# ctSkennerton/crass

Measured on AMD Instinct MI355X. Metric: reads/sec through DR search+recruit, 150bp synthetic, 1/2/4/8 MI355X, higher is better.
Workload: dtype u8; 1 GPU; 100000000 synthetic 150 bp reads, 50 seeded DRs, 1 % CRISPR reads (BASELINE.json configs[2]); pass1 + merge + pass2; total_reads=100000000, reads_per_gpu=100000000, read_len=150, n_dr=50, parallelism=read-shards x1, launcher=single context, pass1_found=563794, pass2_found=436000, patterns=13320, ac_states=0, filter_survivors=1705594, fast_filter=1, lds_automaton=2, merge_fallbacks=0

## Files before the change

### crass_amd/csrc/dev_common.h

```cpp
#pragma once
#include "engine_internal.h"

namespace crass {

#define WAVE 64

static __device__ __forceinline__ void wave_sync()
{
    __builtin_amdgcn_fence(__ATOMIC_RELEASE, "wavefront");
    __builtin_amdgcn_wave_barrier();
    __builtin_amdgcn_fence(__ATOMIC_ACQUIRE, "wavefront");
}

static __device__ __forceinline__ uint32_t uni(uint32_t x) { return (uint32_t)__builtin_amdgcn_readfirstlane((int)x); }
static __device__ __forceinline__ int uni(int x) { return __builtin_amdgcn_readfirstlane(x); }
static __device__ __forceinline__ uint64_t uni64(uint64_t x) { return ((uint64_t)uni((uint32_t)(x >> 32)) << 32) | (uint64_t)uni((uint32_t)x); }

static __device__ __forceinline__ uint64_t rd_word_off(const DevReads &R, uint64_t r)
{
    return R.stride_words ? r * (uint64_t)R.stride_words : R.word_off[r];
}
static __device__ __forceinline__ uint32_t rd_len(const DevReads &R, uint64_t r)
{
    return R.uniform_len ? R.uniform_len : R.lengths[r];
}
static __device__ __forceinline__ bool rd_is_exc(const DevReads &R, uint64_t r)
{
    return (R.exc_mask[r >> 5] >> (r & 31)) & 1u;
}
static __device__ __forceinline__ uint64_t rd_hint_off(const DevReads &R, uint64_t r)
{
    return R.uniform_len ? r * (uint64_t)((R.uniform_len + 63u) >> 6) : R.pos_hint_off[r];
}
static __device__ __forceinline__ uint64_t rd_header_id(const DevReads &R, uint64_t r)
{
    return R.header_id ? R.header_id[r] : r;
}

typedef unsigned short u16x2 __attribute__((ext_vector_type(2)));
static __device__ __forceinline__ uint32_t pk_min_u16(uint32_t a, uint32_t b)
{
    u16x2 r = __builtin_elementwise_min(__builtin_bit_cast(u16x2, a), __builtin_bit_cast(u16x2, b));
    return __builtin_bit_cast(uint32_t, r);
}

}
```

### crass_amd/csrc/engine.cpp

```cpp
#include "engine_ctx.h"

#include <cstdio>
#include <new>
#include <string>

void crass_hip_ctx::widen_p1() const
{
    P1Dense &D = dense;
    if (D.wide_ready) return;
    (void)wait_bulk();
    const uint64_t n = D.n;
    const uint32_t ss_cap = D.pack_ss_cap, stride = dr_stride;
    const uint8_t *hb = D.h_blob.p;
    const uint16_t *b_replen = (const uint16_t *)(hb + D.lay.replen), *b_ss = (const uint16_t *)(hb + D.lay.ss);
    const uint8_t *b_nss = hb + D.lay.nss, *b_ss8 = hb + D.lay.ss;
    D.w_replen.resize(n); D.w_nss.resize(n); D.w_ss_off.resize(n); D.w_ss.resize(n * (size_t)ss_cap);
    D.w_dr_len.resize(n); D.w_dr.resize(n * (size_t)stride);
    if (D.dr_fallback) (void)hipStreamSynchronize(copy_stream);
    else (void)wait_dx();
    const size_t per_task = 16384;
    host_parallel_for((size_t)((n + per_task - 1) / per_task), 16, [&](size_t t) {
        const uint64_t k0 = t * per_task, k1 = std::min<uint64_t>(n, k0 + per_task);
        for (uint64_t k = k0; k < k1; k++) { D.w_replen[k] = b_replen[k]; D.w_nss[k] = b_nss[k]; D.w_ss_off[k] = k * (uint64_t)ss_cap; }
        if (D.lay.ss_elem == 1) for (uint64_t i = k0 * ss_cap; i < k1 * (uint64_t)ss_cap; i++) D.w_ss[i] = b_ss8[i];
// ... 152 lines not shown
{
    if (!c || level < 0 || level > 2) return CRASS_ERR_INVALID_ARG;
    c->timing_level = level;
    return CRASS_OK;
}

int crass_hip_set_host_view(crass_hip_ctx *c, int light)
{
    if (!c || light < 0 || light > 1) return CRASS_ERR_INVALID_ARG;
    quiesce_worker(c);
    c->host_view_light = light != 0;
    if (c->host_view_light) c->dm.M.x_on = 0;
    return CRASS_OK;
}

int crass_hip_set_timing_focus(crass_hip_ctx *c, unsigned kernels)
{
    if (!c || kernels > 7u) return CRASS_ERR_INVALID_ARG;
    c->timing_focus = kernels;
    return CRASS_OK;
}

void crass_hip_destroy(crass_hip_ctx *c)
{
    if (!c) return;
    (void)hipSetDevice(c->device);
    quiesce_worker(c);
    c->worker.stop();
    if (c->stream) (void)hipStreamSynchronize(c->stream);
    if (c->copy_stream) (void)hipStreamSynchronize(c->copy_stream);
    if (c->hint_stream) (void)hipStreamSynchronize(c->hint_stream);
    (void)sdma_wait(c->dma);
    (void)c->wait_dx();
    ingest_free_all(c);
    if (getenv("CRASS_POLL_REPORT")) fprintf(stderr, "[crass_hip] stage-flag polls that ran out of their budget: %u (of %u flags)\n", c->n_poll_timeouts.load(), c->flag_seq);
    c->lb_status.release(); c->lb_ticket.release(); c->h_lb_fail.release(); c->h_flags.release();
    if (c->xchg.ev_counts) (void)hipEventDestroy(c->xchg.ev_counts);
    c->dm.release(); c->h_qblob.release(); c->xchg.send.release(); c->xchg.xinfo.release(); c->xchg.h_xinfo.release();
    c->dd_map.release(); c->dd_dx_chars.release(); c->dd_dx_len.release(); c->dd_dx_hash.release();
    c->h_dmap.release(); c->h_dx_chars.release(); c->h_dx_len.release(); c->h_dx_hash.release();
    if (c->ev_gathered) (void)hipEventDestroy(c->ev_gathered);
    if (c->ev_sink_copies) (void)hipEventDestroy(c->ev_sink_copies);
    for (int q = 0; q < crass_hip_ctx::kHintParts; q++) if (c->ev_hint[q]) (void)hipEventDestroy(c->ev_hint[q]);
    if (c->ev_hint_go) (void)hipEventDestroy(c->ev_hint_go);
    if (c->hint_stream) (void)hipStreamDestroy(c->hint_stream);
    sdma_destroy(c->dma); c->dma = nullptr;
    for (auto &d : c->dma_sink) { sdma_destroy(d); d = nullptr; }
    for (auto &d : c->dma_dx) { sdma_destroy(d); d = nullptr; }
    if (c->ev_premerge) (void)hipEventDestroy(c->ev_premerge);
    if (c->copy_stream) (void)hipStreamDestroy(c->copy_stream);
    c->r_packed.release(); c->r_word_off.release(); c->r_lengths.release(); c->r_header_id.release();
    c->r_exc_mask.release(); c->r_exc_read.release(); c->r_exc_off.release(); c->r_exc_bytes.release();
    c->d_mask.release(); c->d_word_prefix.release(); c->d_block_sums.release(); c->d_idx.release(); c->d_count.release();
    c->d_found.release(); c->d_hit_info.release(); c->d_surv.release(); c->d_dr.release(); c->d_ss_pool.release();
    c->d_ss_used.release(); c->d_rec.release(); c->d_exc_hit.release(); c->d_extra.release(); c->d_extra_bad.release(); c->h_extra_bad.release();
    c->g_surv.release(); c->g_dr.release(); c->g_ss.release(); c->g_fidx.release(); c->h_count.release(); c->h_surv.release(); c->h_dr.release(); c->h_ss.release(); c->h_idx.release(); c->h_rec.release();
    c->a_go4w.release(); c->a_go16.release(); c->a_go32.release(); c->a_out.release(); c->a_go4.release(); c->dense.release(); c->d_fidx.release(); c->d_pos_hint.release(); c->d_pos_hint_off.release(); c->d_pos_hint_blk.release(); c->d_punt.release(); c->d_redo.release(); c->dd_keys.release(); c->dd_first.release(); c->dd_slot.release(); c->dd_rep.release(); c->dd_hash.release(); c->h_rep.release(); c->h_hash.release(); c->a_anchor.release(); c->d_slot_info.release(); c->d_slot_pid.release(); c->a_out_pid.release(); c->a_pat_token.release();
    for (auto &e : c->ev) if (e) (void)hipEventDestroy(e);
    if (c->stream) (void)hipStreamDestroy(c->stream);
    delete c;
}

int validate_reads(const crass_reads *r)
{
    if (!r) return CRASS_ERR_INVALID_ARG;
    if (r->n_reads && !r->packed) return CRASS_ERR_INVALID_ARG;
    if (!r->stride_words && r->n_reads && !r->word_off) return CRASS_ERR_INVALID_ARG;
    if (!r->uniform_len && r->n_reads && !r->lengths) return CRASS_ERR_INVALID_ARG;
    if (r->n_exceptions && (!r->exc_read || !r->exc_off || !r->exc_bytes)) return CRASS_ERR_INVALID_ARG;
    if (r->uniform_len > CRASS_HIP_MAX_READ_LEN) return CRASS_ERR_UNSUPPORTED;
    return CRASS_OK;
}

int alloc_scratch(crass_hip_ctx *c)
{
    const uint64_t n = c->R.n_reads;
    const uint64_t n_words = std::max<uint64_t>((n + 63) / 64, 1024);
    HIPCHK(c, c->d_mask.ensure(n_words + 1));
    HIPCHK(c, c->d_word_prefix.ensure(n_words + 1));
    HIPCHK(c, c->d_block_sums.ensure((n_words + 255) / 256 + 2));
    HIPCHK(c, c->d_idx.ensure(n + 1));
    HIPCHK(c, c->d_count.ensure(8));
    HIPCHK(c, c->d_found.ensure(n + 1));
    HIPCHK(c, c->d_hit_info.ensure(n + 1));
    HIPCHK(c, c->d_ss_used.ensure(4));
    HIPCHK(c, c->h_count.ensure(32));
    HIPCHK(c, hipMemsetAsync(c->d_found.p, 0, n + 1, c->stream));
    return CRASS_OK;
}

static int setup_pos_hints(crass_hip_ctx *c, const uint32_t *lengths, uint32_t uniform_len, uint64_t n)
{
    c->n_pos_hint_words = 0;
    c->R.pos_hint = nullptr; c->R.pos_hint_off = nullptr; c->R.wave_walk = 0; c->R.hint_all = 0;
    const DevParams &P = c->dp;
    const bool lane_filter = c->R.stride_words >= 4 && c->R.stride_words <= 16;
    c->hint_filter = c->max_len <= c->env.long_min && !lane_filter && !c->env.no_hint_filter;
    c->hint_filter_any = false;
    const bool shifts_ok = P.lowDR + P.lowSp >= 17 && P.highDR + P.highSp <= 127 && P.highDR + P.highSp >= P.lowDR + P.lowSp;
    const bool lattice_hints = P.window == 8 && P.skips == 8 && shifts_ok;
    const bool any_filter = c->hint_filter && !lattice_hints && shifts_ok && P.window >= 6 && P.window <= 9 && P.skips >= 1;
    if ((c->max_len <= c->env.long_min && !c->hint_filter) || n == 0 || !(lattice_hints || any_filter)) return CRASS_OK;
    if (c->env.no_pos_hints) return CRASS_OK;
    std::vector<uint64_t> off(n + 1);
    uint64_t at = 0;
    for (uint64_t i = 0; i < n; i++) { off[i] = at; at += ((uint64_t)(lengths ? lengths[i] : uniform_len) + 63) / 64; }
    off[n] = at;
    HIPCHK(c, c->d_pos_hint_off.ensure(n + 1)); HIPCHK(c, c->d_pos_hint.ensure(at + 1));
    HIPCHK(c, hipMemcpy(c->d_pos_hint_off.p, off.data(), (n + 1) * 8, hipMemcpyHostToDevice));
    c->n_pos_hint_words = at;
    c->hint_filter_any = any_filter;
    c->R.pos_hint = c->d_pos_hint.p; c->R.pos_hint_off = c->d_pos_hint_off.p;
    c->R.hint_all = any_filter ? 1u : 0u;
    c->R.wave_walk = c->max_len > std::min<uint32_t>(c->env.long_min, c->env.wave_walk_min) ? 1u : 0u;
    c->pos_hint_blk = false;
    { const char *hp = getenv("CRASS_HINT_PARTS");
      const int want = hp ? atoi(hp) : 2;
      const bool big = hp ? (n >= 64 && at >= 2048) : (n >= 4096 && at >= (1u << 20));
      c->hint_parts = (big && !c->hint_filter) ? std::min(std::max(want, 1), (int)crass_hip_ctx::kHintParts) : 1; }
    if (c->hint_parts > 1 && !c->hint_stream) {
        int prio_lo = 0, prio_hi = 0;
        (void)hipDeviceGetStreamPriorityRange(&prio_lo, &prio_hi);
        HIPCHK(c, hipStreamCreateWithPriority(&c->hint_stream, hipStreamNonBlocking, getenv("CRASS_HINT_SAME_PRIORITY") ? 0 : prio_lo));
        for (int q = 0; q < crass_hip_ctx::kHintParts; q++) HIPCHK(c, hipEventCreateWithFlags(&c->ev_hint[q], hipEventDisableTiming));
        HIPCHK(c, hipEventCreateWithFlags(&c->ev_hint_go, hipEventDisableTiming));
    }
    for (int q = 0; q <= c->hint_parts; q++) {
        const uint64_t r = q == c->hint_parts ? n : n * (uint64_t)q / (uint64_t)c->hint_parts;
        c->hint_read_split[q] = r;
        c->hint_word_split[q] = q == c->hint_parts ? at : ((off[r] + 255) & ~255ull);
    }
    if (lengths && n <= 0xFFFFFFFFull) {
        std::vector<uint32_t> blk((at + 255) / 256 + 1, 0);
        uint64_t r = 0;
        for (uint64_t b = 0; b * 256 < at; b++) {
            while (r + 1 < n && off[r + 1] <= b * 256) r++;
            blk[b] = (uint32_t)r;
// ... 201 lines not shown
```

### crass_amd/csrc/engine_ctx.h

```cpp
#pragma once
#include "../../include/crass_hip.h"
#include "engine_internal.h"
#include "merge.h"
#include "fastx_launch.h"

#include <algorithm>
#include <atomic>
#include <chrono>
#include <condition_variable>
#include <cstdint>
#include <cstdlib>
#include <cstring>
#include <functional>
#include <memory>
#include <mutex>
#include <thread>
#include <utility>
#include <vector>

#pragma GCC visibility push(hidden)
namespace crass {

inline double now_ms()
{
// ... 164 lines not shown
    std::vector<uint8_t> f_flags;
    DevBuf<unsigned long long> n_table; DevBuf<uint64_t> n_rec_pos, n_ids, n_ctl; DevBuf<uint32_t> n_long;
    PinBuf<uint64_t> n_h_ctl;
    StageTimer<3> tm_names;
    float last_hid_ms[3] = {0, 0, 0};
    DevBuf<unsigned long long> nt_table; DevBuf<uint64_t> nt_rec_pos;
    bool have_names = false, nt_on_arena = false;
    const uint8_t *nt_bytes = nullptr; uint64_t nt_n_bytes = 0, nt_n_reads = 0, nt_mask = 0;
    DevBuf<uint8_t> nq_names; DevBuf<uint64_t> nq_off, nq_out; DevBuf<uint32_t> nq_long;
    DevBuf<uint32_t> nq_ctl, no_len, no_flag; DevBuf<uint64_t> no_tiles, no_idx, no_off;
    PinBuf<uint64_t> nq_h_ctl, no_h;
    uint64_t last_find_found = 0;
    StageTimer<2> tm_find;
    float last_names_ms[2] = {0, 0};
    LineFetch hl, ql;
    DevBuf<uint8_t> fa_arena; uint64_t fa_bytes = 0; bool have_arena = false;
    PinBuf<uint64_t> fa_h_base; PinBuf<int32_t> fa_h_format;
    struct ShardStaged { uint32_t file; uint64_t a, b, off; };
    DevBuf<uint8_t> sh_stage, sh_tail; DevBuf<FxProbe> sh_part; PinBuf<FxProbe> sh_h_part;
    std::vector<ShardStaged> sh_staged;
    std::vector<uint64_t> sh_base;
    uint64_t sh_n_reads = 0; bool sh_scanned = false, sh_loaded = false;
    StageTimer<2> tm_probe;
    float last_probe_ms = 0;
};

}
#pragma GCC visibility pop

using namespace crass;

struct EnvSwitches {
    bool no_lookback = false, no_pos_hints = false, merge_profile = false, no_lane_kernel = false;
    bool host_merge = false, no_speculation = false, exc_separate = false, dm_inject_fail = false, dm_init_late = false;
    bool no_presize = false;
    bool dd_full_table = false;
    bool no_device_view = false;
    bool force_device_view = false;
    bool no_dense_light = false;
    bool no_warm_launch = false;
    uint32_t view_group_cap = 32768;
    uint32_t view_sort_max = 2048;
    uint64_t test_bounds[4] = {0, 0, 0, 0};
    uint32_t row_cap = 256, dm_group_cap = 16384, surv_debug = 0;
    int stage_timing = -1;
    uint64_t pool_cap_bytes = 0;
    bool no_hint_filter = false;
    uint32_t wave_walk_min = 800;
    uint32_t long_min = 2048;
    uint64_t text_chunk_bytes = 64ull << 20;
    bool inflate_hbm_window = true;
    uint32_t hid_hash_bits = 64;
    bool lane_find_serial = false;
    uint32_t probe_blocks = 0;
    void read()
    {
        auto on = [](const char *n) { return getenv(n) != nullptr; };
        no_lookback = on("CRASS_NO_LOOKBACK"); no_pos_hints = on("CRASS_NO_POS_HINTS");
        merge_profile = on("CRASS_MERGE_PROFILE"); no_lane_kernel = on("CRASS_NO_LANE_KERNEL"); host_merge = on("CRASS_HOST_MERGE");
        no_speculation = on("CRASS_NO_SPECULATION"); exc_separate = on("CRASS_EXC_SEPARATE"); dm_init_late = on("CRASS_DM_INIT_LATE");
        dm_inject_fail = on("CRASS_DM_INJECT_FAIL"); no_presize = on("CRASS_NO_PRESIZE"); no_device_view = on("CRASS_NO_DEVICE_VIEW"); dd_full_table = on("CRASS_DD_FULL_TABLE"); force_device_view = on("CRASS_DEVICE_VIEW");
        view_group_cap = 32768; if (const char *e = getenv("CRASS_VIEW_GROUP_CAP")) view_group_cap = (uint32_t)std::max(1, atoi(e));
        view_sort_max = 2048; if (const char *e = getenv("CRASS_VIEW_SORT_MAX")) view_sort_max = (uint32_t)std::min(2048, std::max(64, atoi(e)));
        row_cap = 256; if (const char *e = getenv("CRASS_ROW_CAP")) row_cap = (uint32_t)std::max(1, atoi(e));
        dm_group_cap = 16384; if (const char *e = getenv("CRASS_DM_GROUP_CAP")) dm_group_cap = (uint32_t)std::max(1, atoi(e));
        surv_debug = 0; if (const char *e = getenv("CRASS_SURV_DEBUG")) surv_debug = (uint32_t)atoi(e);
        stage_timing = -1; if (const char *e = getenv("CRASS_STAGE_TIMING")) stage_timing = std::min(2, std::max(0, atoi(e)));
        for (auto &b : test_bounds) b = 0;
        if (const char *e = getenv("CRASS_TEST_BOUNDS")) { int k = 0; for (const char *q = e; *q && k < 4; k++) { test_bounds[k] = (uint64_t)atoll(q); while (*q && *q != ',') q++; if (*q == ',') q++; } }
        no_hint_filter = on("CRASS_NO_HINT_FILTER");
        wave_walk_min = 800; if (const char *e = getenv("CRASS_WAVE_WALK_MIN")) wave_walk_min = (uint32_t)std::max(0, atoi(e));
        long_min = 2048; if (const char *e = getenv("CRASS_LONG_MIN")) long_min = (uint32_t)std::max(0, atoi(e));
        no_warm_launch = getenv("CRASS_NO_WARM_LAUNCH") != nullptr;
        no_dense_light = getenv("CRASS_NO_DENSE_LIGHT") != nullptr;
        text_chunk_bytes = 64ull << 20; if (const char *e = getenv("CRASS_TEXT_CHUNK_BYTES")) text_chunk_bytes = (uint64_t)std::max(1ll, atoll(e));
        inflate_hbm_window = true; if (const char *e = getenv("CRASS_INFLATE_WINDOW")) inflate_hbm_window = strcmp(e, "lds") != 0;
        hid_hash_bits = 64; if (const char *e = getenv("CRASS_HID_TEST_HASH_BITS")) hid_hash_bits = (uint32_t)std::min(64, std::max(0, atoi(e)));
        lane_find_serial = false; if (const char *e = getenv("CRASS_LANE_FIND_SERIAL")) lane_find_serial = atoi(e) != 0;
        probe_blocks = 0; if (const char *e = getenv("CRASS_PROBE_BLOCKS")) probe_blocks = (uint32_t)std::max(0, atoi(e));
        pool_cap_bytes = 0; if (const char *e = getenv("CRASS_POOL_CAP_MB")) pool_cap_bytes = (uint64_t)std::max(1ll, atoll(e)) << 20;
    }
};

struct crass_hip_ctx {
    crass_params prm{};
    EnvSwitches env;
    DevParams dp{};
    int device = 0;
    hipStream_t stream = nullptr;
    mutable int last_hip = 0;

    DevReads R{};
    bool have_reads = false;
    uint64_t read_base = 0;
    uint32_t max_len = 0;
    bool uniform = false;
    DevBuf<uint32_t> r_packed; DevBuf<uint64_t> r_word_off; DevBuf<uint32_t> r_lengths; DevBuf<uint64_t> r_header_id;
    DevBuf<uint32_t> r_exc_mask; DevBuf<uint64_t> r_exc_read; DevBuf<uint64_t> r_exc_off; DevBuf<uint8_t> r_exc_bytes;
    std::vector<uint64_t> h_exc_read;
    std::vector<uint32_t> h_lengths;
    Ingest in;

    DevBuf<uint64_t> d_mask; DevBuf<uint32_t> d_word_prefix; DevBuf<uint32_t> d_block_sums;
    DevBuf<uint64_t> d_idx; DevBuf<uint32_t> d_count; DevBuf<uint8_t> d_found; DevBuf<uint32_t> d_hit_info;
    bool hints_valid = false;
    DevBuf<SurvOut> d_surv; DevBuf<char> d_dr; DevBuf<uint32_t> d_ss_pool; DevBuf<uint32_t> d_ss_used;
    DevBuf<RecruitOut> d_rec; DevBuf<uint32_t> d_exc_hit; DevBuf<uint64_t> d_extra;
    DevBuf<uint32_t> d_extra_bad; PinBuf<uint32_t> h_extra_bad;
    PinBuf<uint32_t> h_count; PinBuf<SurvOut> h_surv; PinBuf<char> h_dr; PinBuf<uint32_t> h_ss; PinBuf<uint64_t> h_idx;
    DevBuf<SurvOut> g_surv; DevBuf<char> g_dr; DevBuf<uint32_t> g_ss;
    PinBuf<RecruitOut> h_rec;
    DevBuf<uint16_t> a_go16; DevBuf<uint32_t> a_go32; DevBuf<uint16_t> a_out; DevBuf<uint16_t> a_go4;
    DevAutomaton A{};
    HostAutomaton H;
    bool full_automaton_uploaded = false;
    DevBuf<uint32_t> a_go4w;
    DevBuf<uint32_t> a_anchor; DevBuf<uint32_t> d_slot_info; DevBuf<uint32_t> d_slot_pid; DevBuf<uint32_t> a_out_pid; DevBuf<uint32_t> a_pat_token;
    bool have_pat_token = false;
    DevAnchors K{};
    bool have_anchors = false;
    bool have_patterns = false;
    uint32_t n_installed_patterns = 0;

    bool have_pass1 = false;
    struct P1List {
        std::vector<uint64_t> read; std::vector<uint8_t> low; std::vector<uint32_t> replen, nss;
        std::vector<uint64_t> ss_off; std::vector<uint32_t, NoInitAlloc<uint32_t>> ss; std::vector<uint16_t> dr_len; std::vector<char, NoInitAlloc<char>> dr;
        void clear() { read.clear(); low.clear(); replen.clear(); nss.clear(); ss_off.clear(); ss.clear(); dr_len.clear(); dr.clear(); }
        void reserve(size_t n, uint32_t stride) { read.reserve(n); low.reserve(n); replen.reserve(n); nss.reserve(n); ss_off.reserve(n); ss.reserve(n * 6); dr_len.reserve(n); dr.reserve(n * stride); }
        size_t size() const { return read.size(); }
    } cand;
    mutable struct P1Dense {
        DevBuf<uint16_t> d_dr_len; DevBuf<char> d_dr;
        uint64_t n = 0;
        bool active = false;
        PinBuf<uint8_t> h_blob; DevBuf<uint8_t> d_blob;
        P1Blob lay{};
        uint32_t pack_ss_cap = 0;
        bool wide_ready = false;
        std::vector<uint32_t> w_replen, w_nss; std::vector<uint32_t, NoInitAlloc<uint32_t>> w_ss; std::vector<uint64_t> w_ss_off; std::vector<uint16_t> w_dr_len;
        std::vector<char, NoInitAlloc<char>> w_dr;
        PinBuf<char> h_dr_fb; PinBuf<uint16_t> h_dr_len_fb; bool dr_fallback = false;
        void release()
        {
            h_blob.release(); d_blob.release(); h_dr_fb.release(); h_dr_len_fb.release(); d_dr_len.release(); d_dr.release();
        }
    } dense;
    DevBuf<uint64_t> d_fidx;
    DevBuf<uint64_t> g_fidx;
    DevBuf<uint64_t> d_pos_hint, d_pos_hint_off; uint64_t n_pos_hint_words = 0;
    DevBuf<uint32_t> d_punt;
    DevBuf<uint32_t> d_redo;
    SdmaCopy *dma_sink[4] = {nullptr, nullptr, nullptr, nullptr};
    DevBuf<uint32_t> d_pos_hint_blk; bool pos_hint_blk = false;
    DevBuf<unsigned long long> dd_keys; DevBuf<uint32_t> dd_first, dd_slot, dd_rep; DevBuf<uint64_t> dd_hash;
    PinBuf<uint32_t> h_rep; PinBuf<uint64_t> h_hash;
    bool have_rep = false;
    DevBuf<uint32_t> dd_map; DevBuf<char> dd_dx_chars; DevBuf<uint16_t> dd_dx_len; DevBuf<uint64_t> dd_dx_hash;
// ... 282 lines not shown
```

### crass_amd/csrc/engine_internal.h

```cpp
#pragma once
#include <stdint.h>
#include <stddef.h>
#include <hip/hip_runtime.h>
#include "devmem.h"
#include "merge.h"

namespace crass {

struct DevReads {
    const uint32_t *packed;
    const uint64_t *word_off;
    const uint32_t *lengths;
    const uint64_t *header_id;
    const uint32_t *exc_mask;
    uint64_t n_reads;
    uint32_t stride_words;
    uint32_t uniform_len;
    const uint64_t *exc_read;
    const uint64_t *exc_off;
    const uint8_t  *exc_bytes;
    uint64_t n_exc;
    const uint64_t *pos_hint;
    const uint64_t *pos_hint_off;
    uint32_t wave_walk;
    uint32_t hint_all;
};

struct DevParams {
    uint32_t lowDR, highDR, lowSp, highSp, window, minRepeats;
    uint32_t skips;
    uint32_t debug_stop;
    uint32_t exc_survive;
    uint32_t find_serial;
    unsigned long long *prof;
};

struct SurvOut {
    uint32_t found;
    uint32_t n_ss;
    uint32_t repeat_len;
    uint32_t ss_off;
    uint16_t dr_len;
    uint8_t  low_lexi;
    uint8_t  err;
};

struct RecruitOut {
    uint32_t start, end;
    uint32_t token;
    uint16_t dr_len;
    uint8_t  low_lexi;
    uint8_t  pad;
};

struct DevAutomaton {
    const uint16_t *go16;
    const uint32_t *go32;
    const uint16_t *out_len;
    const uint32_t *out_pid;
    const uint16_t *go4;
    const uint32_t *go4w;
    uint32_t n_states;
    uint32_t n_sym1;
    uint8_t  sym[256];
    uint32_t acgt_ok;
    uint32_t max_pat_len;
};

static __host__ __device__ __forceinline__ uint32_t ak_bloom_word(uint32_t h) { return h >> 17; }
static __host__ __device__ __forceinline__ uint32_t ak_bloom_bits(uint32_t h) { return (1u << ((h >> 12) & 31u)) | (1u << ((h >> 7) & 31u)); }

struct DevAnchors {
    const uint32_t *table;
    uint32_t log_size;
    uint32_t mode;
    uint32_t m1, m2;
    uint32_t n_keys;
    uint32_t with_exc;
};

struct DevMergeState {
    uint32_t n_survivors;
    uint32_t n_patterns;
    uint32_t n_keys;
    uint32_t log_size;
    uint32_t fail;
    uint32_t k0;
    uint32_t all_t;
    uint32_t unused_a, unused_b;
    uint32_t tab_mode;
    uint32_t n_badk;
    uint32_t pad[5];
};

static constexpr uint32_t kDmHotStripes = 16, kDmHotCounters = 5, kDmHotWords = kDmHotCounters * kDmHotStripes * 32;
enum { kHotSurvivors = 0, kHotKeys = 1, kHotK0 = 2, kHotEntCursor = 3, kHotRdCursor = 4 };
__host__ __device__ inline uint32_t dm_hot(uint32_t counter, uint32_t block) { return (counter * kDmHotStripes + (block & (kDmHotStripes - 1u))) * 32u; }

// ... 102 lines not shown
    if (tid < kDmHotStripes) {
        M.hot[dm_hot(kHotSurvivors, (uint32_t)tid)] = 0u; M.hot[dm_hot(kHotKeys, (uint32_t)tid)] = 0u; M.hot[dm_hot(kHotK0, (uint32_t)tid)] = 0xFFFFFFFFu;
        M.hot[dm_hot(kHotEntCursor, (uint32_t)tid)] = 0u; M.hot[dm_hot(kHotRdCursor, (uint32_t)tid)] = 0u;
    }
    if (tid == 0) {
        DevMergeState s{};
        s.k0 = 0xFFFFFFFFu;
        s.fail = M.inject_fail ? 16u : 0u;
        *M.st = s;
    }
}

static __device__ __forceinline__ void stage_flag_store(uint32_t *flag, uint32_t val)
{
    __hip_atomic_store(flag, val, __ATOMIC_RELEASE, __HIP_MEMORY_SCOPE_SYSTEM);
}
hipError_t launch_xg_fill(const char *dx_chars, const uint16_t *dx_len, const uint32_t *d_nd, uint32_t stride, uint64_t cap_rows,
                          uint32_t slot_bytes, uint8_t *send, hipStream_t st, const uint32_t *p1_counts = nullptr, uint64_t surv_bound = 0,
                          uint32_t *h_flag = nullptr, uint32_t flag_val = 0);
hipError_t launch_xg_unpack(const uint8_t *recv, uint32_t world, uint32_t rank, uint32_t stride, uint64_t cap_rows, uint32_t slot_bytes,
                            char *g_chars, uint16_t *g_len, uint32_t *xinfo, hipStream_t st, uint32_t *h_xinfo = nullptr,
                            uint32_t *zero2 = nullptr,
                            unsigned long long *dd_keys = nullptr, uint32_t *dd_first = nullptr, uint32_t dd_size = 0);
hipError_t launch_device_merge(const DevMerge &M, hipStream_t st, bool init_done = false, hipStream_t view_st = nullptr,
                               hipEvent_t ev_fork = nullptr, hipEvent_t ev_view = nullptr,
                               hipEvent_t ev_apply = nullptr);
hipError_t launch_anchor_filter_dev(const DevReads &R, const DevMerge &M, const uint8_t *found_flag, uint64_t *hitmask, hipStream_t st, uint32_t max_blocks = 0);
hipError_t launch_dm_verify(const DevReads &R, const DevMerge &M, const uint64_t *idx, const uint32_t *d_n, uint64_t n_max,
                            uint32_t *info_by_slot, uint32_t *pid_by_slot, hipStream_t st);
hipError_t warm_dmerge_module();

struct SurvLds {
    uint32_t seq_bytes;
    uint32_t ss_cap;
    uint32_t row_elems;
    uint32_t words_cap;
    uint32_t hint_words;
    uint32_t total_bytes;
    uint32_t seq_window;
    uint32_t ss_slot;
};

hipError_t launch_filter_general(const DevReads &R, const DevParams &P, uint64_t *hitmask,
                                 uint32_t max_len, hipStream_t st);
hipError_t launch_hint_positions(const DevReads &R, const DevParams &P, const uint64_t *hint_off, const uint32_t *blk_read, uint64_t n_words,
                                 uint64_t *hint_bits, hipStream_t st,
                                 uint64_t w_begin = 0, uint64_t w_end = ~0ull,
                                 uint64_t *hitmask = nullptr);
hipError_t launch_hint_filter_any(const DevReads &R, const DevParams &P, const uint64_t *hint_off, const uint32_t *blk_read, uint64_t n_words,
                                  uint64_t *hitmask, uint64_t *hint_bits, hipStream_t st);
hipError_t launch_long_light(const DevReads &R, const DevParams &P, const uint32_t *d_n, uint64_t n_max, SurvOut *out, uint64_t slot_base,
                             uint32_t max_len, hipStream_t st, uint32_t *punt_list, uint32_t *d_punt_n, const uint64_t *surv_idx = nullptr);
hipError_t launch_filter_fast(const DevReads &R, const DevParams &P, uint64_t *hitmask, uint32_t *seed_hint, hipStream_t st,
                              uint8_t *clear_found = nullptr, bool *cleared = nullptr);
#define CRASS_VGPR_FLOOR(N) asm volatile("" ::: "v" #N)

#ifdef __HIPCC__
template <int THREADS>
static __device__ __forceinline__ uint32_t block_reserve(uint32_t v, uint32_t *counter)
{
    __shared__ uint32_t br_tot[THREADS / 64];
    __shared__ uint32_t br_base;
    const int lane = threadIdx.x & 63, w = threadIdx.x >> 6;
    uint32_t incl = v;
#pragma unroll
    for (int off = 1; off < 64; off <<= 1) {
        const uint32_t u = (uint32_t)__shfl_up((int)incl, off);
        if (lane >= off) incl += u;
    }
    if (lane == 63) br_tot[w] = incl;
    __syncthreads();
    if (threadIdx.x == 0) {
        uint32_t tot = 0;
        for (int i = 0; i < THREADS / 64; i++) { const uint32_t x = br_tot[i]; br_tot[i] = tot; tot += x; }
        br_base = tot ? atomicAdd(counter, tot) : 0u;
    }
    __syncthreads();
    return br_base + br_tot[w] + incl - v;
}
#endif

struct Lookback {
    unsigned long long *status;
    uint32_t *ticket;
    uint32_t epoch;
    uint32_t *fail;
};
static inline uint32_t lookback_tile_words(uint64_t n_words) { return n_words >= 16384 ? 4096u : 256u; }

hipError_t launch_compact(const uint64_t *mask, uint64_t n_words, uint64_t n_bits, uint32_t *word_prefix,
                          uint32_t *block_sums, uint64_t *out_idx, uint64_t out_cap, uint32_t *d_count,
                          hipStream_t st, uint32_t *zero_a = nullptr, uint32_t n_a = 0, uint32_t *zero_b = nullptr, uint32_t n_b = 0,
                          const Lookback *lb = nullptr);
hipError_t launch_survivor(const DevReads &R, const DevParams &P, bool exceptions,
                           const uint64_t *surv_idx, const uint32_t *d_n_surv, uint64_t n_surv_max,
                           SurvOut *out, char *dr_chars, uint32_t dr_stride,
                           uint32_t *ss_pool, uint32_t ss_pool_cap, uint32_t *d_ss_used,
                           uint8_t *found_flag, const uint32_t *seed_hint, const SurvLds &lds, int grid, hipStream_t st,
                           int punt_only = 0,
                           uint64_t slot_base = 0, uint64_t slot_total = 0,
                           const uint32_t *punt_list = nullptr, const uint32_t *d_punt_n = nullptr,
                           uint32_t *redo_list = nullptr);
hipError_t launch_survivor_lanes(const DevReads &R, const DevParams &P, const uint64_t *surv_idx, const uint32_t *d_n_surv,
                                 uint64_t n_surv_max, SurvOut *out, char *dr_chars, uint32_t dr_stride, uint32_t *ss_pool,
                                 uint32_t ss_cap, uint8_t *found_flag, const uint32_t *seed_hint, hipStream_t st,
                                 const DevMerge *init_merge = nullptr, uint32_t max_len = 0, uint32_t *punt_cnt = nullptr);
hipError_t launch_recruit_general(const DevReads &R, const DevAutomaton &A, const uint8_t *found_flag,
                                  uint64_t *hitmask, uint32_t *hit_info, hipStream_t st);
hipError_t launch_recruit_lds(const DevReads &R, const DevAutomaton &A, const uint8_t *found_flag,
                              uint64_t *hitmask, uint32_t *hit_info, hipStream_t st);
hipError_t launch_anchor_filter(const DevReads &R, const DevAnchors &K, const uint8_t *found_flag,
                                uint64_t *hitmask, hipStream_t st, uint32_t max_blocks = 0);
hipError_t launch_recruit_list(const DevReads &R, const DevAutomaton &A, const uint64_t *idx, const uint32_t *d_n,
                               uint64_t n_max, uint32_t *info_by_slot, uint32_t *pid_by_slot, hipStream_t st);
hipError_t launch_recruit_exceptions(const DevReads &R, const DevAutomaton &A, const uint8_t *found_flag,
                                     uint32_t *exc_hit_info , hipStream_t st);
hipError_t launch_recruit_finish(const DevReads &R, const uint64_t *hit_idx, const uint32_t *d_n_hits,
                                 uint64_t n_hits_max, const uint32_t *hit_info, bool info_by_slot, bool exceptions,
                                 const uint32_t *pid_by_slot, const uint32_t *pat_token,
                                 RecruitOut *out, char *dr_chars, uint32_t dr_stride, hipStream_t st,
                                 const uint64_t *pat_mask = nullptr);
hipError_t launch_levenshtein_batch(const uint8_t *chars, const uint64_t *a_off, const uint32_t *a_len,
                                    const uint64_t *b_off, const uint32_t *b_len, uint64_t n_pairs,
                                    int32_t *dist, float *sim, uint32_t max_len, hipStream_t st);
hipError_t launch_mark_found(const uint64_t *idx, uint64_t n, const uint64_t *header_id, uint8_t *found_flag, hipStream_t st);
hipError_t launch_mark_found_skip(const uint64_t *idx, uint64_t n, uint64_t n_reads, const uint64_t *header_id, uint8_t *found_flag, uint32_t *bad,
                                  hipStream_t st);
hipError_t launch_copy_to_host(const void *d_src, void *h_dst, uint64_t bytes, hipStream_t st);
struct SdmaCopy;
SdmaCopy *sdma_create();
void sdma_destroy(SdmaCopy *s);
bool sdma_start(SdmaCopy *s, const void *d_src, void *h_dst, size_t bytes);
int sdma_wait(SdmaCopy *s);
bool sdma_pending(const SdmaCopy *s);
hipError_t launch_build_exc_mask(const uint64_t *exc_read, uint64_t n_exc, uint32_t *exc_mask, hipStream_t st);

hipError_t launch_found_compact(const SurvOut *out, const uint32_t *d_n, uint64_t n_max, uint32_t *d_err, unsigned long long *dd_keys,
                                uint32_t *dd_first, uint32_t dd_size, uint64_t *fidx, uint32_t *d_nf, const Lookback &lb, hipStream_t st);
hipError_t launch_select_found(const SurvOut *out, uint64_t n, uint64_t *mask, uint32_t *d_err, hipStream_t st);
hipError_t launch_gather_sparse(const uint64_t *fidx, const uint32_t *d_nf, uint64_t n_max, const SurvOut *out, const char *dr_chars, uint32_t dr_stride,
                                const uint32_t *ss_pool, SurvOut *g_out, uint64_t *g_slot, char *g_dr, uint32_t *g_ss, uint32_t g_ss_cap,
                                uint32_t *d_ss_total, hipStream_t st, uint16_t *g_dr_len = nullptr,
                                int ss16 = 0);
hipError_t launch_found_mask(const SurvOut *out, const uint32_t *d_n, uint64_t n, uint64_t *mask, uint32_t *d_err, hipStream_t st,
                             unsigned long long *dd_keys = nullptr, uint32_t *dd_first = nullptr, uint32_t dd_size = 0);
hipError_t launch_gather_found(const uint64_t *fidx, const uint32_t *d_nf, uint64_t n_max, const SurvOut *out,
                               const uint64_t *surv_idx, uint64_t read_base, const char *dr_chars, uint32_t dr_stride,
                               const uint32_t *ss_pool, uint32_t ss_cap, uint32_t ss_elem, uint8_t *blob,
                               uint16_t *g_dr_len, char *g_dr, hipStream_t st,
                               unsigned long long *dd_keys = nullptr, uint32_t *dd_first = nullptr, uint32_t dd_size = 0,
                               uint64_t *dd_hash = nullptr, uint32_t *dd_slot = nullptr, uint32_t *d_mismatch = nullptr);
static constexpr uint32_t kDdMaxProbes = 256;
struct P1Blob { uint64_t read, replen, nss, low, ss, total; uint32_t ss_elem; };
__host__ __device__ inline P1Blob p1_blob_layout(uint64_t nf, uint32_t ss_cap, uint32_t ss_elem = 2)
{
    P1Blob b;
    uint64_t at = 0;
    auto sec = [&](uint64_t bytes) { const uint64_t o = at; at += (bytes + 15u) & ~15ull; return o; };
// ... 37 lines not shown
```

### crass_amd/csrc/engine_pass1.cpp

```cpp
#include "engine_ctx.h"

#include <cstdio>

extern "C" {

static int hint_wait_all(crass_hip_ctx *c)
{
    if (!c->hint_pending) return CRASS_OK;
    HIPCHK(c, hipStreamWaitEvent(c->stream, c->ev_hint[c->hint_parts - 1], 0));
    c->hint_pending = false;
    return CRASS_OK;
}

static bool getenv_once_hl_host() { static const bool v = getenv("CRASS_HL_HOST_DEDUPE") != nullptr; return v; }
static bool getenv_once_copy_early() { static const bool on = getenv("CRASS_COPY_EARLY") != nullptr; return on; }

static void dump_surv_prof(crass_hip_ctx *c)
{
    if (!c->dp.prof) return;
    unsigned long long v[192];
    if (hipMemcpy(v, c->dp.prof, sizeof v, hipMemcpyDeviceToHost) != hipSuccess) return;
    (void)hipMemset(c->dp.prof, 0, sizeof v);
    { const unsigned long long big = ~0ull; (void)hipMemcpy(c->dp.prof + 188, &big, 8, hipMemcpyHostToDevice); }
    if (v[191]) fprintf(stderr, "[surv_prof] %llu waves; first start .. last start %.1f us, first start .. last end %.1f us\n", v[186], (double)(v[187] - v[188]) / 100.0, (double)(v[189] - v[188]) / 100.0);
// ... 36 lines not shown
                         const uint64_t *surv_idx_host)
{
    if (n_total == 0) return hint_wait_all(c);
    const SurvLds lds_full = survivor_lds_last_resort(c->max_len, c->dp);
    if (lds_full.total_bytes > 160 * 1024) return CRASS_ERR_UNSUPPORTED;
    const bool rows_bounded = lds_full.row_elems < survivor_lds_layout(c->max_len, c->dp).row_elems;
    const uint32_t row_cap = rows_bounded ? std::min(c->env.row_cap, std::max(c->dp.highDR, c->dp.highSp)) : c->env.row_cap;
    const bool long_full = getenv("CRASS_LONG_FULL_LAYOUT") != nullptr;
    const uint32_t win_env = getenv("CRASS_SEQ_WINDOW") ? (uint32_t)atoi(getenv("CRASS_SEQ_WINDOW")) : 0u;
    const bool windowed = !exc && (win_env || (c->max_len > c->env.long_min && !long_full));
    const SurvLds lds = windowed ? survivor_lds_layout(c->max_len, c->dp, row_cap, win_env ? win_env : 4608u, 256u)
                                 : survivor_lds_layout(c->max_len, c->dp, row_cap);
    const bool capped = lds.row_elems != lds_full.row_elems || lds.seq_window != 0 || lds.ss_cap != lds_full.ss_cap;
    const uint64_t chunk_cap = std::min<uint64_t>(n_total, 1u << 20);
    const uint64_t ss_per = std::min<uint64_t>(lds_full.ss_cap, 64);
    const uint64_t pool_cap = std::min<uint64_t>(std::max<uint64_t>(chunk_cap * ss_per, 1u << 16), 1ull << 28);
    HIPCHK(c, c->d_surv.ensure(chunk_cap));
    HIPCHK(c, c->d_dr.ensure(chunk_cap * c->dr_stride));
    HIPCHK(c, c->d_ss_pool.ensure(pool_cap));
    HIPCHK(c, c->h_surv.ensure(chunk_cap));
    HIPCHK(c, c->h_dr.ensure(chunk_cap * c->dr_stride));
    const bool ident_list = !exc && !surv_idx_host && c->R.n_exc == 0 && n_total <= chunk_cap;
    const uint32_t sh0 = c->dp.lowDR + c->dp.lowSp, sh1 = c->dp.highDR + c->dp.highSp;
    const bool light_any = !c->R.pos_hint && c->max_len > c->env.long_min && !(c->dp.window == 8 && c->dp.skips == 8) && c->dp.window >= 6 && c->dp.window <= 9 &&
                           sh0 >= 17 && sh1 <= 127 && sh1 >= sh0 && !c->env.no_pos_hints;
    const bool use_light = ident_list && ((c->R.pos_hint && c->dp.skips == 8 && c->dp.window == 8) || light_any) && c->dp.debug_stop == 0 && !getenv("CRASS_NO_LIGHT");
    const int grid = 256 * 64;
    const uint32_t stride = c->dr_stride;
    L.reserve(L.size() + n_total / 2 + 16, stride);
    for (uint64_t off = 0; off < n_total; off += chunk_cap) {
        const uint64_t nchunk = std::min(chunk_cap, n_total - off);
        HIPCHK(c, hipMemsetAsync(c->d_ss_used.p, 0, 4, c->stream));
        DevReads R = c->R;
        if (exc) {
            R.exc_read = c->R.exc_read + off; R.exc_off = c->R.exc_off + off; R.n_exc = nchunk;
        }
        if (use_light) {
            HIPCHK(c, c->d_punt.ensure(nchunk + 1)); HIPCHK(c, hipMemsetAsync(c->d_punt.p, 0, 4, c->stream));
            HIPCHK(c, c->d_redo.ensure(nchunk + 1)); HIPCHK(c, hipMemsetAsync(c->d_redo.p, 0, 4, c->stream));
        }
        if (!exc && off == 0) HIPCHK(c, c->stamp(8, 1));
        if (!exc && c->hint_pending && off == 0 && nchunk == n_total) {
            uint64_t s0 = 0;
            for (int q = 0; q < c->hint_parts; q++) {
                const uint64_t r1 = c->hint_read_split[q + 1];
                uint64_t s1 = q + 1 == c->hint_parts ? nchunk
                            : (surv_idx_host ? (uint64_t)(std::lower_bound(surv_idx_host, surv_idx_host + nchunk, r1) - surv_idx_host) : std::min<uint64_t>(r1, nchunk));
                if (q > 0) HIPCHK(c, hipStreamWaitEvent(c->stream, c->ev_hint[q], 0));
                if (s1 > s0 && use_light)
                    HIPCHK(c, launch_long_light(R, c->dp, c->d_count.p + 1, s1 - s0, c->d_surv.p + s0, s0, c->max_len, c->stream, c->d_punt.p + 1, c->d_punt.p));
                else if (s1 > s0)
                    HIPCHK(c, launch_survivor(R, c->dp, false, ident_list ? nullptr : c->d_idx.p + s0, c->d_count.p + 1, s1 - s0,
                                              c->d_surv.p + s0, c->d_dr.p + s0 * (size_t)stride, stride, c->d_ss_pool.p, (uint32_t)pool_cap, c->d_ss_used.p,
                                              c->d_found.p, c->hints_valid ? c->d_hit_info.p : nullptr, lds,
                                              (int)std::min<uint64_t>(grid, s1 - s0), c->stream, 0, s0, nchunk));
                s0 = s1;
            }
            c->hint_pending = false;
        } else if (use_light) {
            { const int hw = hint_wait_all(c); if (hw) return hw; }
            HIPCHK(c, launch_long_light(R, c->dp, c->d_count.p + 1, nchunk, c->d_surv.p, 0, c->max_len, c->stream, c->d_punt.p + 1, c->d_punt.p));
        } else {
            { const int hw = hint_wait_all(c); if (hw) return hw; }
            HIPCHK(c, launch_survivor(R, c->dp, exc, (exc || ident_list) ? nullptr : c->d_idx.p + off, c->d_count.p + (exc ? 0 : 1), nchunk,
                                      c->d_surv.p, c->d_dr.p, stride, c->d_ss_pool.p, (uint32_t)pool_cap, c->d_ss_used.p,
                                      c->d_found.p, (!exc && c->hints_valid) ? c->d_hit_info.p : nullptr, lds,
                                      (int)std::min<uint64_t>(grid, nchunk), c->stream));
        }
        if (use_light)
            HIPCHK(c, launch_survivor(R, c->dp, false, nullptr, c->d_count.p + 1, nchunk,
                                      c->d_surv.p, c->d_dr.p, stride, c->d_ss_pool.p, (uint32_t)pool_cap, c->d_ss_used.p,
                                      c->d_found.p, nullptr, lds, (int)std::min<uint64_t>(256 * 12, nchunk), c->stream, 7, 0, nchunk, c->d_punt.p + 1, c->d_punt.p,
                                      capped ? c->d_redo.p : nullptr));
        if (use_light && c->dp.prof) { HIPCHK(c, hipStreamSynchronize(c->stream)); dump_surv_prof(c); }
        if (capped && use_light)
            HIPCHK(c, launch_survivor(R, c->dp, false, nullptr, c->d_count.p + 1, nchunk,
                                      c->d_surv.p, c->d_dr.p, stride, c->d_ss_pool.p, (uint32_t)pool_cap, c->d_ss_used.p,
                                      c->d_found.p, nullptr, lds_full, (int)std::min<uint64_t>(256 * 2, nchunk), c->stream, 6, 0, nchunk, c->d_redo.p + 1, c->d_redo.p));
        else if (capped)
            HIPCHK(c, launch_survivor(R, c->dp, exc, (exc || ident_list) ? nullptr : c->d_idx.p + off, c->d_count.p + (exc ? 0 : 1), nchunk,
                                      c->d_surv.p, c->d_dr.p, stride, c->d_ss_pool.p, (uint32_t)pool_cap, c->d_ss_used.p,
                                      c->d_found.p, (!exc && c->hints_valid) ? c->d_hit_info.p : nullptr, lds_full,
                                      (int)std::min<uint64_t>(grid, nchunk), c->stream, 6));
        if (!exc && off == 0) HIPCHK(c, c->stamp(9, 1));
        const uint64_t n_words = (nchunk + 63) / 64;
        HIPCHK(c, c->d_fidx.ensure(nchunk)); HIPCHK(c, c->g_surv.ensure(nchunk)); HIPCHK(c, c->g_dr.ensure(nchunk * (size_t)stride + 16));
        HIPCHK(c, c->g_ss.ensure(pool_cap)); HIPCHK(c, c->g_fidx.ensure(nchunk));
        HIPCHK(c, c->d_mask.ensure(n_words + 1)); HIPCHK(c, c->d_word_prefix.ensure(n_words + 1)); HIPCHK(c, c->d_block_sums.ensure((n_words + 255) / 256 + 2));
        HIPCHK(c, hipMemsetAsync(c->d_count.p + 2, 0, 8, c->stream));
        HIPCHK(c, hipMemsetAsync(c->d_ss_used.p, 0, 4, c->stream));
        HIPCHK(c, launch_select_found(c->d_surv.p, nchunk, c->d_mask.p, c->d_count.p + 3, c->stream));
        HIPCHK(c, launch_compact(c->d_mask.p, n_words, nchunk, c->d_word_prefix.p, c->d_block_sums.p, c->d_fidx.p, nchunk, c->d_count.p + 2, c->stream));
        const bool ss16 = c->max_len < 65536;
        const bool hl_dedupe = !exc && off == 0 && nchunk == n_total && c->R.n_exc == 0 && !c->xchg.active && !c->env.host_merge &&
                               c->prm.lowDRsize >= (int)kDevMinDR && stride <= 64 && (stride & 15u) == 0 && nchunk < (1u << 24) && !getenv_once_hl_host();
        if (hl_dedupe) HIPCHK(c, c->g_dr_len.ensure(nchunk));
        HIPCHK(c, launch_gather_sparse(c->d_fidx.p, c->d_count.p + 2, nchunk, c->d_surv.p, c->d_dr.p, stride, c->d_ss_pool.p, c->g_surv.p,
                                       c->g_fidx.p, c->g_dr.p, c->g_ss.p, (uint32_t)pool_cap, c->d_ss_used.p, c->stream,
                                       hl_dedupe ? c->g_dr_len.p : nullptr, ss16 ? 1 : 0));
        HIPCHK(c, hipMemcpyAsync(c->h_count.p + 2, c->d_count.p + 2, 8, hipMemcpyDeviceToHost, c->stream));
        HIPCHK(c, hipMemcpyAsync(c->h_count.p + 6, c->d_ss_used.p, 4, hipMemcpyDeviceToHost, c->stream));
        const double tq0 = now_ms();
        HIPCHK(c, hipStreamSynchronize(c->stream));
        const double tq1 = now_ms();
        dump_surv_prof(c);
        if (c->h_count.p[3] == 2) return CRASS_ERR_SEARCH_FATAL;
        if (c->h_count.p[3]) return CRASS_ERR_OVERFLOW;
        const uint64_t nf = c->h_count.p[2];
        const uint32_t used = c->h_count.p[6];
        if (nf > nchunk || used > pool_cap) return CRASS_ERR_OVERFLOW;
        HIPCHK(c, c->h_ss.ensure(used + 1)); HIPCHK(c, c->h_idx.ensure(nf + 1));
        static const bool sink_eager = getenv("CRASS_SINK_EAGER") != nullptr;
        const bool lazy = !sink_eager && !exc && off == 0 && nchunk == n_total && c->R.n_exc == 0 && !surv_idx_host && &L == &c->cand && L.read.empty();
        if (nf) {
            hipStream_t cs = lazy ? c->copy_stream : c->stream;
            const void *srcs[4] = {c->g_surv.p, c->g_dr.p, c->g_fidx.p, c->g_ss.p};
            void *dsts[4] = {c->h_surv.p, c->h_dr.p, c->h_idx.p, c->h_ss.p};
            const size_t nbs[4] = {nf * sizeof(SurvOut), nf * (size_t)stride, nf * 8, used ? (size_t)used * (ss16 ? 2 : 4) : 0};
            static const bool sink_blit = getenv("CRASS_COPY_BLIT") != nullptr;
            for (int q = 0; q < 4; q++) {
                if (!nbs[q]) continue;
                if (lazy && !sink_blit) {
                    if (!c->dma_sink[q]) c->dma_sink[q] = sdma_create();
                    if (sdma_start(c->dma_sink[q], srcs[q], dsts[q], nbs[q])) continue;
                }
                HIPCHK(c, hipMemcpyAsync(dsts[q], srcs[q], nbs[q], hipMemcpyDeviceToHost, cs));
            }
            if (lazy) {
                if (!c->ev_sink_copies) HIPCHK(c, hipEventCreateWithFlags(&c->ev_sink_copies, hipEventDisableTiming));
                HIPCHK(c, hipEventRecord(c->ev_sink_copies, c->copy_stream));
                c->bulk_pending = true;
            }
            else HIPCHK(c, hipStreamSynchronize(c->stream));
        }
        bool hl_queued = false, hl_premerge = false;
// ... 197 lines not shown
                D.dr_fallback = true;
                HIPCHK(c, hipMemcpyAsync(c->h_rep.p, c->dd_rep.p, nf * 4, hipMemcpyDeviceToHost, c->copy_stream));
                HIPCHK(c, hipMemcpyAsync(c->h_hash.p, c->dd_hash.p, nf * 8, hipMemcpyDeviceToHost, c->copy_stream));
                c->bulk_pending = true;
                c->have_rep = true;
            }
        }
    } else D.lay.total = 0;
    D.n = nf;
    D.active = true;
    return CRASS_OK;
}

static int run_survivors_dense(crass_hip_ctx *c, uint64_t n_surv, const uint32_t *d_nsurv, bool *overflow, bool defer = false)
{
    *overflow = false;
    { const int hw = hint_wait_all(c); if (hw) return hw; }
    const SurvLds lds = survivor_lds_layout(c->max_len, c->dp);
    if (lds.total_bytes > 160 * 1024) return CRASS_ERR_UNSUPPORTED;
    const uint32_t stride = c->dr_stride;
    const uint64_t pool_cap = std::max<uint64_t>(n_surv * (uint64_t)lds.ss_cap, 1u << 16);
    if (n_surv == 0 || n_surv > kDenseMaxSurvivors || pool_cap >= (1ull << 31) || lds.ss_cap > 128 || (stride & 15)) return CRASS_ERR_STATE;
    crass_hip_ctx::P1Dense &D = c->dense;
    const bool speculative = (d_nsurv == c->d_count.p);
    const uint64_t n_alloc = speculative ? n_surv : std::max<uint64_t>(n_surv, survivor_bound(n_surv));
    const uint32_t ss_elem = c->max_len <= 256 ? 1u : 2u;
    const bool dedupe = n_surv < (1u << 24);
    const bool defer_ok = defer && dedupe && speculative && c->xchg.active;
    { const int as = ensure_dense_buffers(c, n_alloc, pool_cap, lds, dedupe); if (as) return as; }
    if (!speculative) {
        HIPCHK(c, hipMemsetAsync(c->d_count.p + 2, 0, 20, c->stream));
        HIPCHK(c, hipMemsetAsync(c->d_ss_used.p, 0, 4, c->stream));
    }
    c->dm_prepared_n = 0; c->dm_prepared_src = nullptr;
    const DevMerge *init_merge = nullptr;
    if (speculative && dedupe && c->prm.lowDRsize >= (int)kDevMinDR && stride <= 64 && !c->env.host_merge && !c->env.no_speculation && !c->env.dm_init_late) {
        const char *src = nullptr; const uint16_t *src_len = nullptr; uint64_t bound = 0;
        if (!c->xchg.active && c->dm_prev_local && c->dx_cap_hint) {
            HIPCHK(c, c->dd_dx_chars.ensure(n_alloc * stride + 16)); HIPCHK(c, c->dd_dx_len.ensure(n_alloc));
            src = c->dd_dx_chars.p; src_len = c->dd_dx_len.p; bound = c->dx_cap_hint;
        } else if (c->xchg.active && c->xchg.gx_cap_hint && c->xchg.gx_cap_hint <= c->xchg.world * c->xchg.cap) {
            const uint64_t n_max = c->xchg.world * c->xchg.cap;
            HIPCHK(c, c->dm.gx_chars.ensure((size_t)n_max * stride + 16)); HIPCHK(c, c->dm.gx_len.ensure(n_max));
            src = c->dm.gx_chars.p; src_len = c->dm.gx_len.p; bound = c->xchg.gx_cap_hint;
        }
        if (src) {
            const int ps = device_merge_prepare(c, src, src_len, bound, c->d_count.p + 4);
            if (ps) return ps;
            init_merge = &c->dm.M;
        }
    }
    HIPCHK(c, c->stamp(8, 1));
    static const bool no_hints_dbg = getenv("CRASS_SURV_NO_HINTS") != nullptr;
    const uint32_t *hints = (c->hints_valid && !no_hints_dbg) ? c->d_hit_info.p : nullptr;
    const bool no_lanes = c->env.no_lane_kernel;
    hipError_t le = no_lanes ? hipErrorNotSupported
                             : launch_survivor_lanes(c->R, c->dp, c->d_idx.p, d_nsurv, n_surv, c->d_surv.p, c->d_dr.p, stride,
                                                     c->d_ss_pool.p, lds.ss_cap, c->d_found.p, hints, c->stream, init_merge, c->max_len, c->d_count.p + 6);
    if (le != hipSuccess && le != hipErrorNotSupported) { c->last_hip = (int)le; return CRASS_ERR_HIP; }
    if (le == hipSuccess && init_merge) { c->dm_prepared_n = init_merge->n_tok; c->dm_prepared_src = init_merge->dx_chars; }
    bool light_done = false;
    if (le == hipErrorNotSupported && !no_lanes && c->dp.debug_stop == 0 && !c->env.no_dense_light && c->max_len <= 12288 && c->dp.window >= 6 && c->dp.window <= 9) {
        DevReads RL = c->R;
        const bool lattice = c->R.pos_hint && !c->R.hint_all && c->dp.skips == 8 && c->dp.window == 8;
        if (!lattice && !c->R.hint_all) RL.pos_hint = nullptr;
        HIPCHK(c, c->d_punt.ensure(n_surv + 1)); HIPCHK(c, hipMemsetAsync(c->d_punt.p, 0, 4, c->stream));
        const hipError_t ll = launch_long_light(RL, c->dp, d_nsurv, n_surv, c->d_surv.p, 0, c->max_len, c->stream, c->d_punt.p + 1, c->d_punt.p, c->d_idx.p);
        if (ll == hipSuccess) {
            light_done = true;
            HIPCHK(c, launch_survivor(c->R, c->dp, false, c->d_idx.p, d_nsurv, n_surv, c->d_surv.p, c->d_dr.p, stride,
                                      c->d_ss_pool.p, (uint32_t)pool_cap, c->d_ss_used.p, c->d_found.p, hints, lds,
                                      (int)std::min<uint64_t>(256 * 12, n_surv), c->stream, 7, 0, 0, c->d_punt.p + 1, c->d_punt.p));
        } else if (ll != hipErrorNotSupported) { c->last_hip = (int)ll; return CRASS_ERR_HIP; }
    }
    if (!light_done)
    HIPCHK(c, launch_survivor(c->R, c->dp, false, c->d_idx.p, d_nsurv, n_surv, c->d_surv.p, c->d_dr.p, stride,
                              c->d_ss_pool.p, (uint32_t)pool_cap, c->d_ss_used.p, c->d_found.p, hints, lds,
                              (int)std::min<uint64_t>(256 * 32, n_surv), c->stream, le == hipSuccess ? 4 : 0, 0, 0, nullptr,
                              le == hipSuccess ? c->d_count.p + 6 : nullptr));
    if (c->R.n_exc)
        HIPCHK(c, launch_survivor(c->R, c->dp, true, c->d_idx.p, d_nsurv, n_surv, c->d_surv.p, c->d_dr.p, stride,
                                  c->d_ss_pool.p, (uint32_t)pool_cap, c->d_ss_used.p, c->d_found.p, nullptr, lds,
                                  (int)std::min<uint64_t>(256 * 32, n_surv), c->stream, 5));
    HIPCHK(c, c->stamp(9, 1));
    const uint64_t n_words = (n_surv + 63) / 64;
    uint32_t tsize = 1024;
    if (dedupe) while (tsize < n_surv * 2) tsize <<= 1;
    if (dedupe && speculative && c->dx_cap_hint && !c->dd_full_table && !c->env.dd_full_table) {
        uint32_t small = c->env.test_bounds[1] ? 64u : 4096u;
        while (small < c->dx_cap_hint * 4ull && small < tsize) small <<= 1;
        tsize = std::min(tsize, small);
    }
    Lookback lbf;
    if (const Lookback *lb = c->next_lookback_elems(n_surv, &lbf)) {
        HIPCHK(c, launch_found_compact(c->d_surv.p, d_nsurv, n_surv, c->d_count.p + 3, dedupe ? c->dd_keys.p : nullptr,
                                       dedupe ? c->dd_first.p : nullptr, tsize, c->d_fidx.p, c->d_count.p + 2, *lb, c->stream));
    } else {
        HIPCHK(c, launch_found_mask(c->d_surv.p, d_nsurv, n_surv, c->d_mask.p, c->d_count.p + 3, c->stream,
                                    dedupe ? c->dd_keys.p : nullptr, dedupe ? c->dd_first.p : nullptr, tsize));
        HIPCHK(c, launch_compact(c->d_mask.p, n_words, n_surv, c->d_word_prefix.p, c->d_block_sums.p, c->d_fidx.p, n_surv, c->d_count.p + 2, c->stream));
    }
    HIPCHK(c, launch_gather_found(c->d_fidx.p, c->d_count.p + 2, n_surv, c->d_surv.p, c->d_idx.p, c->read_base, c->d_dr.p, stride,
                                  c->d_ss_pool.p, lds.ss_cap, ss_elem, D.d_blob.p, D.d_dr_len.p, D.d_dr.p, c->stream,
                                  dedupe ? c->dd_keys.p : nullptr, dedupe ? c->dd_first.p : nullptr, tsize, c->dd_hash.p, c->dd_slot.p,
                                  c->d_count.p + 5));
    c->have_rep = false;
    c->have_dev_tokens = false;
    if (dedupe) {
        Lookback lbd;
        const bool dxd = c->dx_via_dma;
        HIPCHK(c, launch_dx_tokens(D.d_dr.p, D.d_dr_len.p, c->dd_hash.p, stride, c->d_count.p + 2, (uint32_t)n_surv, c->dd_rep.p, c->dd_slot.p, c->dd_first.p, c->d_mask.p,
                                   c->d_word_prefix.p, c->d_block_sums.p, c->d_fidx.p, c->d_count.p + 4, c->d_count.p + 5, dxd ? c->dd_map.p : c->h_dmap.p,
                                   dxd ? nullptr : c->h_dx_chars.p, dxd ? nullptr : c->h_dx_len.p, dxd ? nullptr : c->h_dx_hash.p, c->dd_dx_chars.p, c->dd_dx_len.p, c->stream,
                                   c->d_count.p, defer_ok ? c->h_count.p + 16 : c->h_count.p, 8,
                                   c->next_lookback_tiles((n_surv + 1023) / 1024, &lbd)));
        if (c->xchg.active)
            HIPCHK(c, launch_xg_fill(c->dd_dx_chars.p, c->dd_dx_len.p, c->d_count.p + 4, stride, c->xchg.cap, c->xchg.slot, c->xchg.send.p, c->stream,
                                     defer_ok ? c->d_count.p : nullptr, n_surv,
                                     (defer_ok && c->poll_on) ? c->h_flags.p : nullptr, (defer_ok && c->poll_on) ? (c->want_p1 = ++c->flag_seq) : 0u));
    }
    if (!dedupe) HIPCHK(c, hipMemcpyAsync(c->h_count.p, c->d_count.p, 32, hipMemcpyDeviceToHost, c->stream));
    bool premerge_queued = false;
    c->premerge = 0;
    D.wide_ready = false; D.dr_fallback = false;
    D.pack_ss_cap = lds.ss_cap;
    const bool will_premerge = speculative && dedupe && !c->xchg.active && c->dm_prev_local && c->dx_cap_hint && c->prm.lowDRsize >= (int)kDevMinDR && stride <= 64 &&
                               !c->env.host_merge && !c->env.no_speculation;
    if (!c->poll_on && (will_premerge || defer_ok)) HIPCHK(c, hipEventRecord(c->ev_gathered, c->stream));
    if (will_premerge) {
        const bool prepared = c->dm_prepared_n == c->dx_cap_hint && c->dm_prepared_src == c->dd_dx_chars.p;
        const int ps = device_merge_enqueue(c, c->dd_dx_chars.p, c->dd_dx_len.p, c->dx_cap_hint, c->d_count.p + 4, prepared);
        if (ps) return ps;
        premerge_queued = true;
        if (!c->poll_on || !c->dma) HIPCHK(c, hipEventRecord(c->ev_premerge, c->stream));
    }
// ... 30 lines not shown
static int first_call_bounds_impl(crass_hip_ctx *c)
{
    c->surv_cap_hint = 0; c->hit_cap_hint = 0; c->dx_cap_hint = 0; c->dm_prev_local = false; c->premerge = 0;
    c->recruit_exact = false;
    const uint64_t n = c->R.n_reads;
    if (c->env.no_presize || c->env.no_speculation || n == 0 || c->max_len > c->env.long_min) return CRASS_OK;
    if (c->R.n_exc && c->env.exc_separate) return CRASS_OK;
    const DevParams &P = c->dp;
    const SurvLds lds = survivor_lds_layout(c->max_len, P);
    if (lds.total_bytes > 160 * 1024 || lds.ss_cap > 128 || (c->dr_stride & 15)) return CRASS_OK;
    const uint32_t min_len = P.lowDR + P.lowSp + P.window + 1;
    const double seeds = c->max_len > min_len ? (double)(c->max_len - min_len) / P.skips + 1.0 : 1.0;
    const double cand = (double)(P.highDR + P.highSp - P.lowDR - P.lowSp + 1);
    double rate = seeds * cand / (double)(1ull << (2 * P.window)) + 0.02;
    if (rate > 1.0) rate = 1.0;
    uint64_t surv = survivor_bound((uint64_t)((double)n * rate));
    if (surv > n + 65536) surv = survivor_bound(n * 2 / 3);
    if (c->env.test_bounds[0]) surv = std::max<uint64_t>(64, c->env.test_bounds[0]);
    const uint64_t pool_cap = std::max<uint64_t>(surv * (uint64_t)lds.ss_cap, 1u << 16);
    if (surv > kDenseMaxSurvivors || pool_cap >= (1ull << 31)) return CRASS_OK;
    size_t free_b = 0, total_b = 0;
    if (hipMemGetInfo(&free_b, &total_b) != hipSuccess) return CRASS_OK;
    const uint64_t per = 140ull + 3ull * c->dr_stride + 6ull * lds.ss_cap;
    if (surv * per > free_b / 4) return CRASS_OK;
    const bool dedupe = surv < (1u << 24);
    int s = ensure_dense_buffers(c, surv, pool_cap, lds, dedupe);
    if (s) return s;
    c->surv_cap_hint = surv;
    { const uint64_t nw = (n + 63) / 64; c->prealloc_lookback(std::max<uint64_t>((nw + lookback_tile_words(nw) - 1) / lookback_tile_words(nw), (surv + 1023) / 1024)); }
    if (dedupe && c->prm.lowDRsize >= (int)kDevMinDR && c->dr_stride <= 64 && !c->env.host_merge) {
        uint64_t dx = crass_hip_exchange_rows_for(n);
        if (c->env.test_bounds[1]) dx = std::max<uint64_t>(16, c->env.test_bounds[1]);
        s = device_merge_prepare(c, c->dd_dx_chars.p, c->dd_dx_len.p, dx, c->d_count.p + 4);
        if (s) return s;
        c->dx_cap_hint = (uint32_t)dx;
        c->dm_prev_local = true;
        try {
            auto touch = [](auto &v, size_t k) { v.resize(k); v.clear(); };
            MergeResult &m = c->merge;
            touch(m.cand_token, (size_t)(n / 128 + 4096));
            touch(m.tokens.strings.chars, (size_t)dx * 48); touch(m.tokens.strings.off, (size_t)dx + 2); m.tokens.strings.clear();
            touch(m.patterns.chars, (size_t)dx * 24); touch(m.patterns.off, (size_t)dx + 2); m.patterns.clear();
            touch(m.pat_group, (size_t)dx); touch(m.pat_token, (size_t)dx); touch(m.grp_tokens, (size_t)dx); touch(m.grp_off, (size_t)dx / 4 + 16);
        } catch (const std::bad_alloc &) { }
    }
    uint64_t hits = hit_bound(n / 64);
    if (c->env.test_bounds[2]) hits = std::max<uint64_t>(16, c->env.test_bounds[2]);
    s = ensure_recruit_buffers(c, hits, 0, true, true);
    if (s) return s;
    c->hit_cap_hint = hits;
    if (!c->env.no_warm_launch) {
        HIPCHK(c, hipMemsetAsync(c->d_count.p, 0, 32, c->stream));
        HIPCHK(c, launch_survivor(c->R, c->dp, false, c->d_idx.p, c->d_count.p + 1, surv, c->d_surv.p, c->d_dr.p, c->dr_stride,
                                  c->d_ss_pool.p, (uint32_t)pool_cap, c->d_ss_used.p, c->d_found.p, nullptr, lds,
                                  (int)std::min<uint64_t>(256 * 32, surv), c->stream, 4));
    }
    host_pool_warm();
    return CRASS_OK;
}

int first_call_bounds(crass_hip_ctx *c)
{
    const int s = first_call_bounds_impl(c);
    if (s == CRASS_ERR_OOM) {
        c->surv_cap_hint = 0; c->hit_cap_hint = 0; c->dx_cap_hint = 0; c->dm_prev_local = false; c->premerge = 0;
        c->last_hip = 0;
        c->dm.release();
        c->dm_prepared_n = 0; c->dm_prepared_src = nullptr;
        return CRASS_OK;
    }
    return s;
}

struct FilterRoute { bool fast = false, hint_filtered = false, found_cleared = false; };

static int launch_filter(crass_hip_ctx *c, uint64_t n_words, FilterRoute &fr)
{
    hipError_t fe = hipErrorNotSupported;
    static const bool found_memset = getenv("CRASS_FOUND_MEMSET") != nullptr;
    if (c->R.stride_words >= 4 && c->R.stride_words <= 16)
        fe = launch_filter_fast(c->R, c->dp, c->d_mask.p, c->d_hit_info.p, c->stream, found_memset ? nullptr : c->d_found.p, &fr.found_cleared);
    if (fe != hipSuccess) fr.found_cleared = false;
    const bool lattice_hints = c->hint_filter && c->R.pos_hint && !c->hint_filter_any;
    if (fe == hipSuccess) fr.fast = true;
    else if (fe == hipErrorNotSupported && (lattice_hints || (c->hint_filter_any && c->n_pos_hint_words))) {
        HIPCHK(c, hipMemsetAsync(c->d_mask.p, 0, n_words * 8, c->stream));
        const uint32_t *blk = c->pos_hint_blk ? c->d_pos_hint_blk.p : nullptr;
        const hipError_t he = lattice_hints ? launch_hint_positions(c->R, c->dp, c->d_pos_hint_off.p, blk, c->n_pos_hint_words, c->d_pos_hint.p, c->stream, 0, c->n_pos_hint_words, c->d_mask.p)
                                            : launch_hint_filter_any(c->R, c->dp, c->d_pos_hint_off.p, blk, c->n_pos_hint_words, c->d_mask.p, c->d_pos_hint.p, c->stream);
        c->hint_pending = false;
        if (he != hipSuccess) { c->last_hip = (int)he; return CRASS_ERR_HIP; }
        fr.hint_filtered = true;
    }
    else if (fe == hipErrorNotSupported) { HIPCHK(c, launch_filter_general(c->R, c->dp, c->d_mask.p, c->max_len, c->stream)); }
    else { c->last_hip = (int)fe; return CRASS_ERR_HIP; }
    return CRASS_OK;
}

static int launch_unfiltered(crass_hip_ctx *c, uint64_t n_words)
{
    HIPCHK(c, hipMemsetAsync(c->d_mask.p, 0xFF, n_words * 8, c->stream));
    if (!c->R.pos_hint) return CRASS_OK;
    const uint32_t *blk = c->pos_hint_blk ? c->d_pos_hint_blk.p : nullptr;
    if (c->hint_parts > 1) { HIPCHK(c, hipEventRecord(c->ev_hint_go, c->stream)); HIPCHK(c, hipStreamWaitEvent(c->hint_stream, c->ev_hint_go, 0)); }
    for (int q = 0; q < c->hint_parts; q++) {
        hipStream_t hs = q == 0 ? c->stream : c->hint_stream;
        hipError_t he = launch_hint_positions(c->R, c->dp, c->d_pos_hint_off.p, blk, c->n_pos_hint_words, c->d_pos_hint.p, hs,
                                              c->hint_word_split[q], c->hint_word_split[q + 1]);
        if (he != hipSuccess) { c->last_hip = (int)he; return CRASS_ERR_HIP; }
        if (q > 0) HIPCHK(c, hipEventRecord(c->ev_hint[q], c->hint_stream));
    }
    c->hint_pending = c->hint_parts > 1;
    return CRASS_OK;
}

int read_count(crass_hip_ctx *c)
{
    HIPCHK(c, hipMemcpyAsync(c->h_count.p, c->d_count.p, 4, hipMemcpyDeviceToHost, c->stream));
    HIPCHK(c, hipStreamSynchronize(c->stream));
    return CRASS_OK;
}

static int host_survivor_list(crass_hip_ctx *c, bool use_filter, uint64_t &n_surv, std::vector<uint64_t> &surv_idx)
{
    surv_idx.resize(n_surv);
    if (n_surv && use_filter) {
        HIPCHK(c, c->h_idx.ensure(n_surv));
        HIPCHK(c, hipMemcpyAsync(c->h_idx.p, c->d_idx.p, n_surv * 8, hipMemcpyDeviceToHost, c->stream));
        HIPCHK(c, hipStreamSynchronize(c->stream));
        memcpy(surv_idx.data(), c->h_idx.p, n_surv * 8);
    } else if (n_surv) {
        const uint64_t n = c->R.n_reads;
        size_t e = 0, w = 0;
        for (uint64_t r = 0; r < n; r++) {
            while (e < c->h_exc_read.size() && c->h_exc_read[e] < r) e++;
// ... 25 lines not shown
    return m;
}

static int fill_send_from_host(crass_hip_ctx *c)
{
    ensure_distinct(c);
    const uint64_t nd = c->dx_len.size();
    std::vector<uint8_t> buf(c->xchg.send_bytes(), 0);
    reinterpret_cast<uint64_t *>(buf.data())[0] = nd;
    reinterpret_cast<uint32_t *>(buf.data())[2] = c->dr_stride;
    reinterpret_cast<uint32_t *>(buf.data())[3] = (uint32_t)c->xchg.cap;
    for (uint64_t j = 0; j < nd && j < c->xchg.cap; j++) {
        uint8_t *row = buf.data() + (j + 1) * (size_t)c->xchg.slot;
        memcpy(row, c->dx_chars.data() + j * (size_t)c->dr_stride, c->dr_stride);
        const uint32_t l = c->dx_len[j];
        memcpy(row + c->dr_stride, &l, 4);
    }
    HIPCHK(c, hipMemcpy(c->xchg.send.p, buf.data(), buf.size(), hipMemcpyHostToDevice));
    return CRASS_OK;
}

static void publish_p1_counters(crass_hip_ctx *c, uint64_t n_surv, bool fast, bool hint_filtered, float ms_sink_host)
{
    c->cnt.ms_sink_host = ms_sink_host;
    c->cnt.n_filter_survivors = n_surv + (c->dp.exc_survive ? 0 : c->R.n_exc);
    c->cnt.n_pass1_found = c->n_cand();
    c->cnt.used_fast_filter = fast ? 1 : (hint_filtered ? 2 : 0);
    c->spans_p1 = true; c->span_survivors = n_surv != 0;
}

int crass_hip_seed_scan(crass_hip_ctx *c)
{
    if (!c) return CRASS_ERR_INVALID_ARG;
    if (!c->have_reads) return CRASS_ERR_STATE;
    (void)hipSetDevice(c->device);
    (void)c->wait_bulk();
    (void)c->wait_dx();
    c->bulk_status = CRASS_OK; c->dx_status = CRASS_OK;
    quiesce_worker(c);
    c->have_pass1 = c->have_merge = c->have_pass2 = false;
    c->dm.active = false;
    c->premerge_inflight = false;
    c->p1d.active = false;
    const bool defer_p1 = c->p1d.enabled && !c->p1d.force_sync && c->xchg.active;
    c->p1d.force_sync = false;
    if (c->dm.view_launched) { HIPCHK(c, hipStreamWaitEvent(c->stream, c->dm.ev_view, 0)); c->dm.view_launched = false; }
    const uint64_t n = c->R.n_reads;
    const uint64_t n_words = (n + 63) / 64;
    HIPCHK(c, c->stamp(0, 1));
    FilterRoute fr;
    const bool use_filter = c->max_len <= c->env.long_min;
    c->dp.exc_survive = (use_filter && c->R.n_exc > 0 && !c->env.exc_separate) ? 1u : 0u;
    if (const int fs = use_filter ? launch_filter(c, n_words, fr) : launch_unfiltered(c, n_words)) return fs;
    c->hints_valid = fr.fast;
    if (!fr.found_cleared) HIPCHK(c, hipMemsetAsync(c->d_found.p, 0, n + 1, c->stream));
    HIPCHK(c, c->stamp(1, 1));
    Lookback lbs;
    HIPCHK(c, launch_compact(c->d_mask.p, n_words, n, c->d_word_prefix.p, c->d_block_sums.p, c->d_idx.p, n, c->d_count.p, c->stream,
                             c->d_count.p + 2, 5, c->d_ss_used.p, 1, c->next_lookback(n_words, &lbs)));
    HIPCHK(c, c->stamp(2, 2));
    c->dense.active = false; c->have_rep = false; c->have_distinct = false;
    c->have_dev_tokens = false; c->hl_tokens = false;
    c->cand_fill = nullptr; c->cand_pending_n = 0;
    c->cand.clear();
    const double t_sink0 = now_ms();
    uint64_t n_surv = 0;
    int s = CRASS_ERR_STATE;
    const bool exc_ok = c->R.n_exc == 0 || c->dp.exc_survive;
    if (use_filter && exc_ok && c->surv_cap_hint && !c->env.no_speculation) {
        bool overflow = false;
        HIPCHK(c, c->stamp(3, 2));
        s = run_survivors_dense(c, c->surv_cap_hint, c->d_count.p, &overflow, defer_p1);
        if (s != CRASS_OK && s != CRASS_ERR_STATE) return s;
        if (s == CRASS_OK && c->p1d.active) {
            c->p1d.fast = fr.fast; c->p1d.hint_filtered = fr.hint_filtered;
            HIPCHK(c, c->stamp(4, 2));
            return CRASS_OK;
        }
        if (s == CRASS_OK) {
            n_surv = c->h_count.p[0];
            if (overflow) c->n_bound_overflows[0]++;
            if (overflow || n_surv == 0) {
                c->dense.active = false;
                s = CRASS_ERR_STATE;
                HIPCHK(c, hipMemsetAsync(c->d_found.p, 0, n + 1, c->stream));
            }
        } else {
            if (const int rs = read_count(c)) return rs;
            n_surv = c->h_count.p[0];
        }
    } else if (!use_filter && c->R.n_exc == 0) {
        n_surv = n;
    } else {
        if (const int rs = read_count(c)) return rs;
        n_surv = c->h_count.p[0];
    }
    const bool spec_done = (s == CRASS_OK);
    const bool try_dense = !spec_done && use_filter && exc_ok && n_surv > 0 && n_surv <= kDenseMaxSurvivors;
    if (!spec_done) {
        c->h_count.p[1] = 0xFFFFFFFFu;
        HIPCHK(c, hipMemcpyAsync(c->d_count.p + 1, c->h_count.p + 1, 4, hipMemcpyHostToDevice, c->stream));
        HIPCHK(c, c->stamp(3, 2));
        bool overflow = false;
        s = try_dense ? run_survivors_dense(c, n_surv, c->d_count.p + 1, &overflow) : CRASS_ERR_STATE;
        if (s != CRASS_OK && s != CRASS_ERR_STATE) return s;
    }
    if (use_filter && exc_ok) c->surv_cap_hint = survivor_bound(n_surv);
    if (s == CRASS_ERR_STATE) {
        const bool identity = !use_filter && c->R.n_exc == 0;
        std::vector<uint64_t> surv_idx;
        if (!identity) { const int ls = host_survivor_list(c, use_filter, n_surv, surv_idx); if (ls) return ls; }
        s = run_survivors(c, false, n_surv, c->cand, identity ? nullptr : surv_idx.data());
// ... 58 lines not shown
```

### crass_amd/csrc/kernels.hip

```cpp
#include "dev_common.h"
#include "comp_table.h"
#include "lane_find.h"
#include <type_traits>
#include <algorithm>

namespace crass {

static __constant__ CompTable c_comp = make_comp_table();

#define FG_WAVES 4

static __device__ __forceinline__ uint32_t lds_code(const uint32_t *w, uint32_t p, uint32_t mask)
{
    uint32_t wi = p >> 4, sh = (p & 15u) * 2u;
    uint64_t v = ((uint64_t)w[wi + 1] << 32) | w[wi];
    return (uint32_t)(v >> sh) & mask;
}

__global__ __launch_bounds__(FG_WAVES * WAVE) void k_filter_general(DevReads R, DevParams P, uint64_t *hitmask,
                                                                      uint32_t lds_words_per_wave)
{
    extern __shared__ __attribute__((aligned(16))) uint32_t fg_lds[];
    const int lane = threadIdx.x & 63;
    const int wave = threadIdx.x >> 6;
// ... 128 lines not shown
    }
    uint32_t miss = (t0 | (t0 >> 15)) & 0xFFFFu;
    if (SW > 8) miss |= (t1 | (t1 >> 15)) << 16;
    return ~miss & (n_seed >= 32 ? 0xFFFFFFFFu : ((1u << n_seed) - 1u));
}

template <int W, int D0, int D1, int LCT, int RPL>
__global__ __launch_bounds__(256) void k_filter_fast_impl(DevReads R, DevParams P, uint64_t *hitmask, uint32_t *seed_hint, uint8_t *clear_found)
{
    const uint64_t r_first = blockIdx.x * (uint64_t)(256 * RPL) + threadIdx.x;
    if (clear_found && r_first == 0) clear_found[R.n_reads] = 0;
    constexpr int WX = W + (D1 >> 4) + 2;
    const uint64_t r_last = R.n_reads - 1;
    uint32_t nxt[W];
    uint64_t nxt_exc;
    if constexpr (RPL > 1) ff_request_row<W>(R, P, r_first, r_last, nxt, nxt_exc);
    else ff_load_row<W>(R, P, r_first, nxt, nxt_exc);
#pragma unroll
    for (int it = 0; it < RPL; it++) {
    const uint64_t r = r_first + (uint64_t)it * 256u;
    const bool active = r < R.n_reads;
    if constexpr (RPL == 1) { if (clear_found && active) clear_found[r] = 0; }
    uint32_t w[WX];
#pragma unroll
    for (int i = 0; i < WX; i++) w[i] = i < W ? nxt[i] : 0u;
    const bool exc = (nxt_exc >> (r & 63)) & 1u;
    if (it + 1 < RPL) {
        ff_request_row<W>(R, P, r + 256u, r_last, nxt, nxt_exc);
        __builtin_amdgcn_sched_barrier(0);
    }
    const uint32_t L = active ? rd_len(R, r) : 0u;
    constexpr int SW = ((16 * W - 58) / 8 + 2) / 2;
    uint32_t acc[SW];
    ff_exact_scan<D0, D1, LCT>(w, acc, [&]() { if constexpr (RPL > 1) { if (clear_found) clear_found[active ? r : R.n_reads] = 0; } });
    bool hit = false;
    const int searchEnd = LCT > 0 ? (LCT - D0 - 8 - 1) : (int)(L - P.lowDR - P.lowSp - 8 - 1);
    if (active && !exc && searchEnd >= 0) {
        const uint32_t hint = ff_exact_hint<LCT>(acc, searchEnd / 8 + 1);
        hit = hint != 0;
        if (hit) seed_hint[r] = hint;
    }
    uint64_t m = __ballot(hit);
    if ((threadIdx.x & 63) == 0 && active) hitmask[r >> 6] = m;
    }
}

static __device__ __forceinline__ uint32_t pk_minimum3_f16(uint32_t a, uint32_t b, uint32_t c)
{
    uint32_t r;
    asm("v_pk_minimum3_f16 %0, %1, %2, %3" : "=v"(r) : "v"(a), "v"(b), "v"(c));
    return r;
}
template <int W, int D0, int D1, int LCT, int RPL>
__global__ __launch_bounds__(256) void k_filter_fast_pairs(DevReads R, DevParams P, uint64_t *hitmask, uint32_t *seed_hint, uint8_t *clear_found)
{
    static_assert(LCT > 0 && LCT - D0 - 9 >= 0 && RPL * 256 <= 65536, "uniform length with at least one seed");
    __shared__ uint32_t q_n;
    __shared__ uint16_t q[256 * RPL];
    __shared__ uint32_t tile_mask[2 * 4 * RPL];
    const uint64_t r_block = blockIdx.x * (uint64_t)(256 * RPL);
    const uint64_t r_first = r_block + threadIdx.x;
    const uint32_t lane = threadIdx.x & 63u;
    if (clear_found && r_first == 0) clear_found[R.n_reads] = 0;
    constexpr int WX = W + (D1 >> 4) + 2;
    constexpr int SW = ((16 * W - 58) / 8 + 2) / 2;
    constexpr int n_seed = (LCT - D0 - 9) / 8 + 1;
    constexpr uint32_t M14 = 0x3FFF3FFFu;
    const uint64_t r_last = R.n_reads - 1;
    uint32_t nxt[W];
    uint64_t nxt_exc;
    ff_request_row<W>(R, P, r_first, r_last, nxt, nxt_exc);
    if (threadIdx.x < 2 * 4 * RPL) tile_mask[threadIdx.x] = 0;
    if (threadIdx.x == 0) q_n = 0;
    __syncthreads();
#pragma unroll
    for (int it = 0; it < RPL; it++) {
        const uint64_t r = r_first + (uint64_t)it * 256u;
        const bool active = r < R.n_reads;
        uint32_t w[WX];
#pragma unroll
        for (int i = 0; i < WX; i++) w[i] = i < W ? nxt[i] : 0u;
        const bool exc = (nxt_exc >> (r & 63)) & 1u;
        if (it + 1 < RPL) {
            ff_request_row<W>(R, P, r + 256u, r_last, nxt, nxt_exc);
            __builtin_amdgcn_sched_barrier(0);
        }
        uint32_t acc[SW];
#pragma unroll
        for (int i = 0; i < SW; i++) acc[i] = 0x3C003C00u;
#pragma unroll
        for (int d = D0; d <= D1; d += 2) {
            if (d == D0 + 2 && clear_found) clear_found[active ? r : R.n_reads] = 0;
#pragma unroll
            for (int k = 0; k < SW; k++) {
                if (d > LCT - 9 - 16 * k) continue;
                const int q0 = d >> 4, sh0 = (d & 15) * 2;
                const uint32_t s0 = sh0 ? __builtin_amdgcn_alignbit(w[k + q0 + 1], w[k + q0], sh0) : w[k + q0];
                const uint32_t a = (s0 ^ w[k]) & M14;
                uint32_t b = a;
                if (d + 1 <= D1 && d + 1 <= LCT - 9 - 16 * k) {
                    const int q1 = (d + 1) >> 4, sh1 = ((d + 1) & 15) * 2;
                    const uint32_t s1 = sh1 ? __builtin_amdgcn_alignbit(w[k + q1 + 1], w[k + q1], sh1) : w[k + q1];
                    b = (s1 ^ w[k]) & M14;
                }
                acc[k] = pk_minimum3_f16(acc[k], a, b);
            }
        }
        uint32_t m = 0x3C003C00u;
#pragma unroll
        for (int k = 0; 2 * k < n_seed; k += 2) m = pk_minimum3_f16(m, acc[k], 2 * (k + 1) < n_seed ? acc[k + 1] : acc[k]);
        const bool pos = active && !exc && pk_nonzero_u16(m) != 0x00010001u;
        const uint64_t pm = __ballot(pos);
        if (pm) {
            uint32_t base = 0;
            if (lane == 0) base = atomicAdd(&q_n, (uint32_t)__popcll(pm));
            base = __builtin_amdgcn_readfirstlane(base);
            const uint32_t before = __builtin_amdgcn_mbcnt_hi((uint32_t)(pm >> 32), __builtin_amdgcn_mbcnt_lo((uint32_t)pm, 0u));
            if (pos) q[base + before] = (uint16_t)(it * 256 + threadIdx.x);
        }
    }
    __syncthreads();
    const uint32_t qn = q_n;
    for (uint32_t b0 = threadIdx.x & ~63u; b0 < qn; b0 += 256u) {
        const bool have = b0 + lane < qn;
        const uint32_t loc = have ? q[b0 + lane] : 0u;
        uint32_t w[WX];
#pragma unroll
        for (int i = 0; i < WX; i++) w[i] = 0u;
        if (have) ff_load_words<W>(R, r_block + loc, w);
        uint32_t acc[SW];
        ff_exact_scan<D0, D1, LCT>(w, acc);
        const uint32_t hint = ff_exact_hint<LCT>(acc, n_seed);
        if (have && hint != 0) {
            seed_hint[r_block + loc] = hint;
            atomicOr(&tile_mask[loc >> 5], 1u << (loc & 31u));
        }
    }
    __syncthreads();
    if (threadIdx.x < 4 * RPL) {
        const uint64_t r0 = r_block + threadIdx.x * 64u;
        if (r0 < R.n_reads) hitmask[r0 >> 6] = (uint64_t)tile_mask[2 * threadIdx.x] | ((uint64_t)tile_mask[2 * threadIdx.x + 1] << 32);
    }
}

template <int W>
__global__ __launch_bounds__(256) void k_filter_fast_range(DevReads R, DevParams P, uint64_t *hitmask, uint32_t *seed_hint)
{
    const uint64_t r = blockIdx.x * (uint64_t)256 + threadIdx.x;
    constexpr int WX = 2 * W + 2;
    uint32_t row[W];
    uint64_t exc_word;
    ff_load_row<W>(R, P, r, row, exc_word);
    const bool active = r < R.n_reads;
    uint32_t w[WX];
#pragma unroll
    for (int i = 0; i < WX; i++) w[i] = i < W ? row[i] : 0u;
    const bool exc = (exc_word >> (r & 63)) & 1u;
    const uint32_t L = active ? rd_len(R, r) : 0u;
    constexpr int SW = ((16 * W - 26) / 8 + 2) / 2;
    const int D0 = (int)(P.lowDR + P.lowSp), D1 = min((int)(P.highDR + P.highSp), 16 * W + 15);
    uint32_t acc[SW];
#pragma unroll
    for (int i = 0; i < SW; i++) acc[i] = 0xFFFFFFFFu;
    const int n_seed_max = (16 * W - D0 - 9) / 8 + 1;
#pragma unroll
    for (int q = 0; q <= W; q++) {
        if (16 * q + 15 < D0 || 16 * q > D1) continue;
        const int sb_lo = max(0, D0 - 16 * q), sb_hi = min(15, D1 - 16 * q);
        for (int sb = sb_lo; sb <= sb_hi; sb++) {
            const uint32_t sh = (uint32_t)(2 * sb);
#pragma unroll
            for (int k = 0; k < SW; k++) {
                if (2 * k >= n_seed_max) continue;
                const uint32_t lo = w[k + q], hi = w[k + q + 1];
                acc[k] = pk_min_u16(acc[k], __builtin_amdgcn_alignbit(hi, lo, sh) ^ w[k]);
            }
        }
    }
    bool hit = false;
    const int searchEnd = (int)(L - P.lowDR - P.lowSp - 8 - 1);
    if (active && !exc && searchEnd >= 0) {
        const int n_seed = searchEnd / 8 + 1;
        uint32_t t0 = 0, t1 = 0;
#pragma unroll
        for (int k = 0; k < SW; k++) {
            const uint32_t f = pk_nonzero_u16(acc[k]);
            if (k < 8) t0 |= f << (2 * k); else t1 |= f << (2 * (k - 8));
        }
        uint32_t miss = (t0 | (t0 >> 15)) & 0xFFFFu;
        if (SW > 8) miss |= (t1 | (t1 >> 15)) << 16;
        const uint32_t hint = ~miss & (n_seed >= 32 ? 0xFFFFFFFFu : ((1u << n_seed) - 1u));
        hit = hint != 0;
        if (hit) seed_hint[r] = hint;
    }
// ... 24 lines not shown
#pragma unroll
    for (int q = 0; q <= W; q++) {
        if (16 * q + 15 < D0 || 16 * q > D1) continue;
        const int sb_lo = max(0, D0 - 16 * q), sb_hi = min(15, D1 - 16 * q);
        for (int sb = sb_lo; sb <= sb_hi; sb++) {
            const uint32_t sh = (uint32_t)(2 * sb);
            uint32_t z[W + 1];
#pragma unroll
            for (int k = 0; k <= W; k++) {
                const uint32_t x = __builtin_amdgcn_alignbit(w[k + q + 1], w[k + q], sh) ^ w[k];
                z[k] = x | (x >> 1);
            }
#pragma unroll
            for (int k = 0; k < W; k++) z[k] |= __builtin_amdgcn_alignbit(z[k + 1], z[k], (uint32_t)(2 * s1));
            if (s2 > 0) {
                z[W] |= z[W] >> (2 * s1);
#pragma unroll
                for (int k = 0; k < W; k++) z[k] |= __builtin_amdgcn_alignbit(z[k + 1], z[k], (uint32_t)(2 * s2));
            }
            if (s3 > 0) {
                z[W] |= z[W] >> (2 * s2);
#pragma unroll
                for (int k = 0; k < W; k++) z[k] |= __builtin_amdgcn_alignbit(z[k + 1], z[k], (uint32_t)(2 * s3));
            }
            if (s4 > 0) {
                z[W] |= z[W] >> (2 * s3);
#pragma unroll
                for (int k = 0; k < W; k++) z[k] |= __builtin_amdgcn_alignbit(z[k + 1], z[k], (uint32_t)(2 * s4));
            }
#pragma unroll
            for (int k = 0; k < W; k++) nz[k] &= z[k];
        }
    }
    bool hit = false;
    const int searchEnd = (int)(L - P.lowDR - P.lowSp - P.window - 1);
    if (active && !exc && searchEnd >= 0) {
        const uint32_t skips = P.skips;
        uint32_t hint = 0, more = 0;
        uint32_t j = 0;
        for (uint32_t i = 0; j <= (uint32_t)searchEnd; i++, j += skips) {
            uint32_t word = 0;
#pragma unroll
            for (int k = 0; k < W; k++) word = (j >> 4) == (uint32_t)k ? nz[k] : word;
            const uint32_t m = ((word >> (2u * (j & 15u))) & 1u) ^ 1u;
            if (i < 32u) hint |= m << i; else more |= m;
        }
        hit = (hint | more) != 0;
        if (hit) seed_hint[r] = more ? 0xFFFFFFFFu : hint;
    }
    const uint64_t m = __ballot(hit);
    if ((threadIdx.x & 63) == 0 && active) hitmask[r >> 6] = m;
}

hipError_t launch_filter_fast(const DevReads &R, const DevParams &P, uint64_t *hitmask, uint32_t *seed_hint, hipStream_t st, uint8_t *clear_found, bool *cleared)
{
    if (cleared) *cleared = false;
    if (!R.stride_words || R.n_reads == 0) return hipErrorNotSupported;
    if (P.window != 8 || P.skips != 8) {
        if (P.window < 6 || P.window > 9 || P.skips < 1 || P.lowDR + P.lowSp < 17 || P.highDR + P.highSp < P.lowDR + P.lowSp) return hipErrorNotSupported;
        const uint64_t nb = (R.n_reads + 255) / 256;
        if (nb > 0x7FFFFFFFull) return hipErrorNotSupported;
        switch (R.stride_words) {
#define FA_CASE(WW) case WW: CRASS_LAUNCH((k_filter_fast_any<WW>), dim3((unsigned)nb), dim3(256), 0, st, R, P, hitmask, seed_hint); break;
            FA_CASE(4) FA_CASE(5) FA_CASE(6) FA_CASE(7) FA_CASE(8) FA_CASE(9) FA_CASE(10)
            FA_CASE(11) FA_CASE(12) FA_CASE(13) FA_CASE(14) FA_CASE(15) FA_CASE(16)
#undef FA_CASE
            default: return hipErrorNotSupported;
        }
        return hipGetLastError();
    }
    if (P.lowDR + P.lowSp != 49 || P.highDR + P.highSp != 97) {
        if (P.lowDR + P.lowSp < 17 || P.highDR + P.highSp < P.lowDR + P.lowSp) return hipErrorNotSupported;
        const uint64_t nb = (R.n_reads + 255) / 256;
        if (nb > 0x7FFFFFFFull) return hipErrorNotSupported;
        switch (R.stride_words) {
#define FR_CASE(WW) case WW: CRASS_LAUNCH((k_filter_fast_range<WW>), dim3((unsigned)nb), dim3(256), 0, st, R, P, hitmask, seed_hint); break;
            FR_CASE(4) FR_CASE(5) FR_CASE(6) FR_CASE(7) FR_CASE(8) FR_CASE(9) FR_CASE(10)
            FR_CASE(11) FR_CASE(12) FR_CASE(13) FR_CASE(14) FR_CASE(15) FR_CASE(16)
#undef FR_CASE
            default: return hipErrorNotSupported;
        }
        return hipGetLastError();
    }
    uint64_t blocks = (R.n_reads + 255) / 256;
    if (blocks > 0x7FFFFFFFull) return hipErrorNotSupported;
    static const int rpl_env = getenv("CRASS_FF_RPL") ? atoi(getenv("CRASS_FF_RPL")) : 0;
    const int rpl = rpl_env ? rpl_env : (R.n_reads >= (1u << 22) ? 4 : 1);
    dim3 g((unsigned)blocks), b(256), g4((unsigned)((blocks + 3) / 4));
    static const bool ff_exact = getenv("CRASS_FF_EXACT") && atoi(getenv("CRASS_FF_EXACT")) != 0;
    if (cleared && clear_found) *cleared = true;
#define FF_LEN(LL, WW) if (R.uniform_len == LL && R.stride_words == WW) { \
        if (rpl >= 4 && !ff_exact) CRASS_LAUNCH((k_filter_fast_pairs<WW, 49, 97, LL, 4>), g4, b, 0, st, R, P, hitmask, seed_hint, clear_found); \
        else if (rpl >= 4) CRASS_LAUNCH((k_filter_fast_impl<WW, 49, 97, LL, 4>), g4, b, 0, st, R, P, hitmask, seed_hint, clear_found); \
        else CRASS_LAUNCH((k_filter_fast_impl<WW, 49, 97, LL, 1>), g, b, 0, st, R, P, hitmask, seed_hint, clear_found); \
        return hipGetLastError(); }
    FF_LEN(100, 7) FF_LEN(101, 7) FF_LEN(125, 8) FF_LEN(126, 8) FF_LEN(150, 10) FF_LEN(151, 10) FF_LEN(250, 16) FF_LEN(251, 16)
#undef FF_LEN
    switch (R.stride_words) {
#define FF_CASE(WW) case WW: CRASS_LAUNCH((k_filter_fast_impl<WW, 49, 97, 0, 1>), g, b, 0, st, R, P, hitmask, seed_hint, clear_found); break;
        FF_CASE(4) FF_CASE(5) FF_CASE(6) FF_CASE(7) FF_CASE(8) FF_CASE(9) FF_CASE(10)
        FF_CASE(11) FF_CASE(12) FF_CASE(13) FF_CASE(14) FF_CASE(15) FF_CASE(16)
#undef FF_CASE
        default: if (cleared) *cleared = false; return hipErrorNotSupported;
    }
    return hipGetLastError();
}

static __device__ __forceinline__ uint64_t hint_bits_class(const uint32_t (&w)[13], uint32_t rho)
{
    uint32_t v[12];
    const uint32_t rs = 2u * rho;
#pragma unroll
    for (int i = 0; i < 12; i++) v[i] = rs ? ((w[i] >> rs) | (w[i + 1] << (32u - rs))) : w[i];
    uint32_t acc[4] = {0xFFFFFFFFu, 0xFFFFFFFFu, 0xFFFFFFFFu, 0xFFFFFFFFu};
#pragma unroll
    for (int d = 49; d <= 97; d++) {
        const int q = d >> 4, sh = (d & 15) * 2;
#pragma unroll
        for (int k = 0; k < 4; k++) {
            const uint32_t lo = v[k + q], hi = v[k + q + 1];
            const uint32_t x = (sh ? ((lo >> sh) | (hi << (32 - sh))) : lo) ^ v[k];
            acc[k] = pk_min_u16(acc[k], x);
        }
    }
    const uint32_t m0 = pk_nonzero_u16(acc[0]), m1 = pk_nonzero_u16(acc[1]), m2 = pk_nonzero_u16(acc[2]), m3 = pk_nonzero_u16(acc[3]);
    const uint32_t lo = __builtin_amdgcn_perm(m1, m0, 0x06040200u) ^ 0x01010101u;
    const uint32_t hi = __builtin_amdgcn_perm(m3, m2, 0x06040200u) ^ 0x01010101u;
    return ((uint64_t)(hi << rho) << 32) | (uint64_t)(lo << rho);
}

static __device__ __forceinline__ uint64_t hint_bits_class_range(const uint32_t (&w)[13], uint32_t rho, int D0, int D1)
{
    uint32_t v[12];
    const uint32_t rs = 2u * rho;
#pragma unroll
    for (int i = 0; i < 12; i++) v[i] = rs ? ((w[i] >> rs) | (w[i + 1] << (32u - rs))) : w[i];
    uint32_t acc[4] = {0xFFFFFFFFu, 0xFFFFFFFFu, 0xFFFFFFFFu, 0xFFFFFFFFu};
#pragma unroll
    for (int q = 0; q < 8; q++) {
        if (16 * q + 15 < D0 || 16 * q > D1) continue;
        const int sb_lo = max(0, D0 - 16 * q), sb_hi = min(15, D1 - 16 * q);
        for (int sb = sb_lo; sb <= sb_hi; sb++) {
            const uint32_t sh = (uint32_t)(2 * sb);
#pragma unroll
            for (int k = 0; k < 4; k++) acc[k] = pk_min_u16(acc[k], __builtin_amdgcn_alignbit(v[k + q + 1], v[k + q], sh) ^ v[k]);
// ... 1116 lines not shown
        for (int i = 0; i < SV_PREFETCH_HINTS; i++) {
            const int wi = lane + i * WAVE;
            if (wi < nh) l_hint[wi] = pf.hw[i];
        }
        first = lane + SV_PREFETCH_HINTS * WAVE;
        if (nh <= SV_PREFETCH_HINTS * WAVE) return;
    }
    const uint64_t *ph = R.pos_hint + rd_hint_off(R, r);
    for (int wi = first; wi < nh; wi += WAVE) l_hint[wi] = ph[wi];
}

static __device__ void load_read_to_lds(const DevReads &R, uint64_t r, uint8_t *seq, uint32_t *words, int L, int lane,
                                        const ReadPrefetch *pf = nullptr)
{
    const uint32_t *g = R.packed + rd_word_off(R, r);
    const int nw = (L + 15) >> 4;
    const int ng = (nw + 4) >> 2;
    const bool have = pf && pf->r == r;
    uint4 *w4 = reinterpret_cast<uint4 *>(words);
    int first = lane;
    if (have) {
#pragma unroll
        for (int i = 0; i < SV_PREFETCH_VEC; i++) {
            const int gi = lane + i * WAVE;
            if (gi < ng) w4[gi] = pf->v[i];
        }
        first = lane + SV_PREFETCH_VEC * WAVE;
    }
    for (int gi = first; gi < ng; gi += WAVE) w4[gi] = sv_load_group(g, gi, nw);
    (void)seq;
}

#define PROF_READ_DONE(cat_, tot_) do { \
            wave_sync(); \
            if (lane == 0) { h.lprof[PF_TOTAL] = (tot_); h.lprof[PF_READS] = 1ull; } \
            wave_sync(); \
            unsigned long long *ws_ = h.lprof + PF_SLOTS + (cat_) * PF_SLOTS; \
            if (lane < PF_SLOTS && lane != PF_MAX) ws_[lane] += h.lprof[lane]; \
            if (lane == PF_MAX && (tot_) > ws_[PF_MAX]) ws_[PF_MAX] = (tot_); \
            if (lane == 0) { int b_ = 63 - __clzll((long long)((tot_) | 1ull)) - 8; b_ = b_ < 0 ? 0 : (b_ >= PF_BINS ? PF_BINS - 1 : b_); h.lprof[5 * PF_SLOTS + (cat_) * PF_BINS + b_] += 1ull; } \
            wave_sync(); } while (0)
#define PROF_WAVE_FLUSH() do { if (h.lprof) { wave_sync(); \
            if (lane == 0) { atomicAdd(P.prof + 190, (unsigned long long)__builtin_readcyclecounter() - wave_c0); atomicAdd(P.prof + 191, (unsigned long long)__builtin_amdgcn_s_memrealtime() - wave_r0); \
                             atomicMax(P.prof + 189, (unsigned long long)__builtin_amdgcn_s_memrealtime()); atomicAdd(P.prof + 186, 1ull); \
                             if (blockIdx.x < 16384) P.prof[193 + 2 * blockIdx.x] = (unsigned long long)__builtin_amdgcn_s_memrealtime(); } \
            for (int q_ = lane; q_ < 4 * PF_SLOTS + 4 * PF_BINS; q_ += WAVE) { \
                const unsigned long long v_ = h.lprof[PF_SLOTS + q_]; \
                if (v_) { if (q_ < 4 * PF_SLOTS && (q_ % PF_SLOTS) == PF_MAX) atomicMax(P.prof + q_, v_); else atomicAdd(P.prof + q_, v_); } } } } while (0)
template <bool EXC>
__global__ __launch_bounds__(WAVE) __attribute__((amdgpu_waves_per_eu(3, 3))) void k_survivor(DevReads R, DevParams P, const uint64_t *surv_idx,
                                                   const uint32_t *d_n_surv, uint64_t n_max, SurvOut *out,
                                                   char *dr_chars, uint32_t dr_stride, uint32_t *ss_pool,
                                                   uint32_t ss_pool_cap, uint32_t *d_ss_used,
                                                   uint8_t *found_flag, const uint32_t *seed_hint, SurvLds lds, int punt_only, uint64_t slot_base, uint64_t slot_total,
                                                   const uint32_t *punt_list, const uint32_t *d_punt_n, uint32_t *redo_list)
{
    extern __shared__ __attribute__((aligned(16))) uint8_t sv_lds[];
    const int lane = threadIdx.x;
    RH h;
    h.seq = sv_lds;
    h.seq_buf = sv_lds; h.seq_win = EXC ? 0 : (int)lds.seq_window;
    h.ss = reinterpret_cast<uint32_t *>(sv_lds + lds.seq_bytes);
    h.cap = (int)lds.ss_cap;
    h.rowA = reinterpret_cast<uint16_t *>(h.ss + lds.ss_cap);
    h.rowB = h.rowA + lds.row_elems;
    h.row_cap = (int)lds.row_elems;
    uint32_t *l_words = reinterpret_cast<uint32_t *>(h.rowB + lds.row_elems);
    h.words = EXC ? nullptr : l_words;
    h.sims = reinterpret_cast<float *>(l_words + lds.words_cap);
    uint64_t *l_hint = reinterpret_cast<uint64_t *>(h.sims + lds.ss_cap);
    h.cmask = (1u << (2 * P.window)) - 1u;
    h.lprof = P.prof ? reinterpret_cast<unsigned long long *>(sv_lds + ((lds.total_bytes + 7u) & ~7u)) : nullptr;
    if (h.lprof) { for (int q = lane; q < PF_LDS_WORDS; q += WAVE) h.lprof[q] = 0ull; wave_sync(); }
    const unsigned long long wave_c0 = h.lprof ? (unsigned long long)__builtin_readcyclecounter() : 0ull;
    const unsigned long long wave_r0 = h.lprof ? (unsigned long long)__builtin_amdgcn_s_memrealtime() : 0ull;
    if (h.lprof && lane == 0) { atomicMin(P.prof + 188, wave_r0); atomicMax(P.prof + 187, wave_r0); }
    if (h.lprof && lane == 0 && blockIdx.x < 16384) P.prof[192 + 2 * blockIdx.x] = wave_r0;
    uint64_t n_surv = (EXC && punt_only != 5) ? R.n_exc : (uint64_t)(*d_n_surv);
    if (n_surv > n_max) n_surv = n_max;
    if (!EXC && punt_only == 4 && !punt_list && d_punt_n && *d_punt_n == 0u) { PROF_WAVE_FLUSH(); return; }
    uint64_t punt_base = (uint64_t)blockIdx.x * WAVE, punt_mask = 0;
    uint64_t lp = blockIdx.x;
    const uint64_t n_list = punt_list ? (uint64_t)(*d_punt_n) : 0;
    ReadPrefetch pf;
    pf.r = ~0ull;
    uint64_t next_s = ~0ull, next_r = 0;
    for (uint64_t s = blockIdx.x;; ) {
        if (punt_only && punt_list) {
            if (lp >= n_list) { PROF_WAVE_FLUSH(); return; }
            s = uni(punt_list[lp]);
            lp += gridDim.x;
        } else if (punt_only) {
            while (punt_mask == 0) {
                if (punt_base >= n_surv) { PROF_WAVE_FLUSH(); return; }
                const uint64_t q = punt_base + lane;
                punt_mask = __ballot(q < n_surv && out[q].err == (uint8_t)punt_only);
                if (punt_mask == 0) punt_base += (uint64_t)gridDim.x * WAVE;
            }
            const int b = __ffsll((unsigned long long)punt_mask) - 1;
            punt_mask &= punt_mask - 1;
            s = punt_base + b;
            if (punt_mask == 0) punt_base += (uint64_t)gridDim.x * WAVE;
        } else if (s >= n_surv) { PROF_WAVE_FLUSH(); return; }
        uint64_t r;
        int L;
        wave_sync();
        const unsigned long long prof_t0 = h.lprof ? (unsigned long long)__builtin_readcyclecounter() : 0ull;
// ... 8 lines not shown
                e = lo;
            } else r = uni64(R.exc_read[s]);
            uint64_t o0 = uni64(R.exc_off[e]);
            L = (int)uni((uint32_t)(R.exc_off[e + 1] - o0));
            for (int i = lane; i < L; i += WAVE) h.seq[i] = R.exc_bytes[o0 + i];
        } else {
            r = (next_s == s) ? next_r : (surv_idx ? uni64(surv_idx[s]) : s + slot_base);
            if (!punt_only && R.n_exc && rd_is_exc(R, r)) {
                if (lane == 0) { SurvOut x; x.found = 0; x.n_ss = 0; x.repeat_len = 0; x.ss_off = 0; x.dr_len = 0; x.low_lexi = 0; x.err = 5; out[s] = x; }
                s += gridDim.x;
                continue;
            }
            L = (int)uni(rd_len(R, r));
            bool no_seed = false;
            if (R.pos_hint && !punt_only) {
                const int nh = (L + 63) >> 6;
                bool any = false;
                if (pf.r == r) {
#pragma unroll
                    for (int i = 0; i < SV_PREFETCH_HINTS; i++) any |= (lane + i * WAVE < nh) && pf.hw[i] != 0ull;
                    if (nh > SV_PREFETCH_HINTS * WAVE) any = true;
                } else {
                    const uint64_t *gh = R.pos_hint + rd_hint_off(R, r);
                    for (int wi = lane; wi < nh; wi += WAVE) any |= gh[wi] != 0ull;
                }
                no_seed = __ballot(any) == 0ull;
            }
            if (!no_seed) {
                load_read_to_lds(R, r, h.seq, l_words, L, lane, &pf);
                if (R.pos_hint) load_hints_to_lds(R, r, L, l_hint, lane, pf);
            }
            pf.r = ~0ull;
            if (!punt_only && s + gridDim.x < n_surv) {
                const uint64_t r2 = surv_idx ? uni64(surv_idx[s + gridDim.x]) : s + gridDim.x + slot_base;
                next_s = s + gridDim.x; next_r = r2;
                if (!R.n_exc || !rd_is_exc(R, r2)) prefetch_read(R, r2, lane, pf);
            } else if (punt_only && punt_list && lp < n_list) {
                const uint64_t s2 = uni(punt_list[lp]);
                const uint64_t r2 = surv_idx ? uni64(surv_idx[s2]) : s2 + slot_base;
                next_s = s2; next_r = r2;
                prefetch_read(R, r2, lane, pf);
            }
            if (no_seed) {
                if (lane == 0) { SurvOut x; x.found = 0; x.n_ss = 0; x.repeat_len = 0; x.ss_off = 0; x.dr_len = 0; x.low_lexi = 0; x.err = 0; out[s] = x; }
                if (h.lprof) { const unsigned long long tot = (unsigned long long)__builtin_readcyclecounter() - prof_t0; PROF_READ_DONE(0, tot); }
                s += gridDim.x;
                continue;
            }
        }
        wave_sync();
        if (h.lprof && lane == 0) h.lprof[PF_STAGE] = (unsigned long long)__builtin_readcyclecounter() - prof_t0;
        h.L = L; h.nss = 0; h.replen = 0; h.err = 0;
        h.asc_lo = 0; h.asc_hi = 0; h.asc_pad = (int)(P.highDR + P.highSp) + 32; h.seq = h.seq_buf;
        const uint32_t hint = (!EXC && seed_hint) ? seed_hint[r] : 0xFFFFFFFFu;
        uint64_t *ph = (!EXC && R.pos_hint) ? l_hint : nullptr;
        uint32_t *cls_from = reinterpret_cast<uint32_t *>(l_hint + lds.hint_words - 4);
        if (ph && lane < 8) cls_from[lane] = (lane == 0 || R.hint_all) ? 0u : 0xFFFFFFFFu;
        wave_sync();
        const uint32_t j_start = (!EXC && punt_only == 7) ? uni(out[s].repeat_len) : 0u;
        int f = (P.debug_stop == 1) ? 0 : search_core(h, P, hint, lane, ph, ph ? cls_from : nullptr, j_start);
        const unsigned long long prof_t1 = h.lprof ? (unsigned long long)__builtin_readcyclecounter() : 0ull;
        SurvOut o;
        o.found = 0; o.n_ss = 0; o.repeat_len = 0; o.ss_off = 0; o.dr_len = 0; o.low_lexi = 0; o.err = 0;
        if (f == -3 || (f == -2 && lds.ss_cap < lds.ss_slot)) o.err = 6;
        else if (f < 0) o.err = (f == -2) ? 2 : 1;
        if (f == 1 && P.debug_stop != 4) {
            int low = 0;
            int dlen = dr_low_lexi(h, dr_chars + s * (uint64_t)dr_stride, (int)dr_stride, low, lane);
            if (dlen < 0 || dlen > (int)dr_stride) o.err = 1;
            else {
                uint32_t off = 0;
                if ((slot_total ? slot_total : n_surv) * lds.ss_slot <= ss_pool_cap) off = (uint32_t)(s + slot_base) * lds.ss_slot;
                else {
                    if (lane == 0) off = atomicAdd(d_ss_used, (uint32_t)h.nss);
                    off = (uint32_t)__shfl((int)off, 0);
                }
                if ((uint64_t)off + (uint64_t)h.nss > ss_pool_cap) o.err = 3;
                else {
                    for (int k = lane; k < h.nss; k += WAVE) ss_pool[off + k] = h.ss[k];
                    o.found = 1; o.n_ss = (uint32_t)h.nss; o.repeat_len = (uint32_t)h.replen;
                    o.ss_off = off; o.dr_len = (uint16_t)dlen; o.low_lexi = (uint8_t)low;
                    if (lane == 0) found_flag[rd_header_id(R, r)] = 1;
                }
            }
        }
        if (lane == 0) out[s] = o;
        if (redo_list && o.err == 6 && lane == 0) redo_list[1u + atomicAdd(redo_list, 1u)] = (uint32_t)s;
        if (h.lprof && lane == 0) h.lprof[PF_OUT] = (unsigned long long)__builtin_readcyclecounter() - prof_t1;
        if (h.lprof) {
            const unsigned long long tot = (unsigned long long)__builtin_readcyclecounter() - prof_t0;
            const int cat = o.err ? 3 : (o.found ? 2 : 1);
            PROF_READ_DONE(cat, tot);
            if (lane == 0) atomicMax(P.prof + 185, (tot << 24) | (unsigned long long)((s + slot_base) & 0xFFFFFFull));
        }
        if (!punt_only) s += gridDim.x;
    }
}

#define LL_HW 3
#define LL_VEC 3
struct LightPrefetch { uint4 v[LL_VEC]; uint64_t hw[LL_HW]; };

static __device__ __forceinline__ void ll_prefetch(const DevReads &R, uint64_t r, int lane, LightPrefetch &pf)
{
    const uint32_t *g = R.packed + rd_word_off(R, r);
    const int L = (int)uni(rd_len(R, r));
    const int nw = (L + 15) >> 4, nh = (L + 63) >> 6;
// ... 873 lines not shown
            uint32_t endSearch = j + o.highDR + o.highSp + o.window;
            if (endSearch >= seq_length) endSearch = seq_length - 1;
            if (endSearch < beginSearch) endSearch = beginSearch;
            if (beginSearch > seq_length) { error = true; continue; }
            int pos = ln_find(h, (int)beginSearch, (int)endSearch, (int)j, (int)o.window, o.find_serial);
            if (o.debug_stop == 2) pos = -1;
            if (pos >= 0) {
                ln_add(h, j, j + o.window - 1);
                ln_add(h, (uint32_t)pos, (uint32_t)pos + o.window - 1);
                if (!h.punt) ln_scan_right(h, (int)j, o.window, o.lowSp, 24, o.find_serial);
                if (h.punt) { finished = true; result = 0; continue; }
            }
            if ((uint32_t)(h.nss / 2) >= o.minRepeats) {
                uint32_t actual_repeat_length = ln_extend(h, (int)o.window, (int)o.lowSp);
                if (o.debug_stop != 3 && (actual_repeat_length >= o.lowDR) && (actual_repeat_length <= o.highDR)) { ready = true; continue; }
                j = ln_ss(h, h.nss - 1) - 1;
                on_lattice = false;
            }
            h.nss = 0;
            j = j + skips;
        }
        if (!finished && error) { finished = true; result = -1; }
        if (!finished && out_of_seeds) { finished = true; result = 0; }
        if (!__syncthreads_or((int)(!finished))) break;
        QcPending pd;
        pd.kind = 0;
        int qc = 0;
        if (!finished) qc = qc_pool_begin(h, (int)o.lowSp, (int)o.highSp, o.debug_stop, pool, pd);
        __syncthreads();
        {
            const uint32_t n32 = pool.cnt[0], n64 = pool.cnt[1];
            for (uint32_t t = threadIdx.x; t < n32; t += blockDim.x) qc_run_task<uint32_t>(pool, t);
            for (uint32_t t = blockDim.x - 1u - threadIdx.x; t < n64; t += blockDim.x) qc_run_task<uint64_t>(pool, pool.cap - 1u - t);
        }
        __syncthreads();
        if (threadIdx.x == 0) { pool.cnt[0] = 0u; pool.cnt[1] = 0u; }
        if (!finished) {
            if (qc == 2) qc = qc_pool_end(pool, pd);
            if (h.punt) { finished = true; result = 0; }
            else if (qc < 0) { finished = true; result = -1; }
            else if (qc) { finished = true; result = 1; }
            else {
                j = ln_ss(h, h.nss - 1) - 1;
                on_lattice = false;
                h.nss = 0;
                j = j + skips;
            }
        }
    }
    return result;
}

#define SL_WAVES 4
static __device__ __forceinline__ uint64_t ln_hint64(const DevReads &R, const uint32_t *seed_hint, uint64_t r, int L, uint32_t skips)
{
    if (seed_hint) return 0xFFFFFFFF00000000ull | (uint64_t)seed_hint[r];
    if (!R.pos_hint) return ~0ull;
    const uint64_t *ph = R.pos_hint + rd_hint_off(R, r);
    const int nh = (L + 63) >> 6;
    if (R.hint_all) {
        uint64_t hint = 0;
        for (uint32_t i = 0, p = 0; i < 64u && (int)p < L; i++, p += skips) hint |= ((ph[p >> 6] >> (p & 63u)) & 1ull) << i;
        return hint;
    }
    uint64_t hint = 0;
    for (int k = 0; k < 8 && k < nh; k++)
        hint |= (((ph[k] & 0x0101010101010101ull) * 0x0102040810204080ull) >> 56) << (8 * k);
    return hint;
}
__global__ __launch_bounds__(WAVE * SL_WAVES) void k_survivor_lanes(DevReads R, DevParams P, const uint64_t *surv_idx, const uint32_t *d_n_surv,
                                                         uint64_t n_max, SurvOut *out, char *dr_chars, uint32_t dr_stride,
                                                         uint32_t *ss_pool, uint32_t ss_cap, uint8_t *found_flag,
                                                         const uint32_t *seed_hint, uint32_t words_per_read, DevMerge IM, int do_init, int regroup,
                                                         uint32_t *punt_cnt)
{
    extern __shared__ __attribute__((aligned(16))) uint32_t sl_lds[];
    __shared__ uint16_t sl_perm[WAVE * SL_WAVES];
    __shared__ uint32_t sl_cnt[SL_WAVES];
    __shared__ uint32_t sl_hint[WAVE * SL_WAVES];
    const int lane = threadIdx.x & (WAVE - 1), wv = threadIdx.x >> 6;
    if (do_init) dm_init_slice(IM, blockIdx.x * (uint64_t)blockDim.x + threadIdx.x, (uint64_t)gridDim.x * blockDim.x);
    uint64_t n_surv = *d_n_surv;
    if (n_surv > n_max) n_surv = n_max;
    uint64_t s = blockIdx.x * (uint64_t)blockDim.x + threadIdx.x;
    if (regroup) {
        bool heavy = false;
        if (s < n_surv) {
            const uint64_t r0 = surv_idx[s];
            const uint32_t h0 = seed_hint ? seed_hint[r0] : 0u;
            sl_hint[threadIdx.x] = h0;
            heavy = !rd_is_exc(R, r0) && (seed_hint ? __popc(h0) : __popcll(ln_hint64(R, nullptr, r0, (int)rd_len(R, r0), P.skips))) >= 2;
        }
        const uint64_t hb = __ballot(heavy);
        if (lane == 0) sl_cnt[wv] = (uint32_t)__popcll(hb);
        __syncthreads();
        uint32_t heavy_before = 0, heavy_total = 0;
#pragma unroll
        for (int k = 0; k < SL_WAVES; k++) { const uint32_t c = sl_cnt[k]; heavy_total += c; if (k < wv) heavy_before += c; }
        const uint32_t below = (uint32_t)__popcll(hb & ((1ull << lane) - 1ull));
        const uint32_t pos = heavy ? heavy_before + below
                                   : heavy_total + ((uint32_t)wv * WAVE - heavy_before) + ((uint32_t)lane - below);
        sl_perm[pos] = (uint16_t)threadIdx.x;
        __syncthreads();
        s = blockIdx.x * (uint64_t)blockDim.x + sl_perm[threadIdx.x];
    }
    const bool hint_in_lds = regroup && seed_hint;
    const size_t wave_words = (size_t)(words_per_read + 5) * WAVE + ((size_t)ss_cap * WAVE + 1) / 2;
    uint32_t *wbase = sl_lds + (size_t)wv * wave_words;
    uint32_t *lw = wbase + lane;
    uint16_t *lss = reinterpret_cast<uint16_t *>(wbase + (size_t)(words_per_read + 5) * WAVE) + lane;
    static_assert(WAVE * SL_WAVES <= 256, "QcTask keeps the owner's thread index in 8 bits");
    __shared__ QcTask sl_task[2 * WAVE * SL_WAVES];
    __shared__ uint8_t sl_res[2 * WAVE * SL_WAVES];
    __shared__ uint32_t sl_qcnt[2];
    if (threadIdx.x < 2) sl_qcnt[threadIdx.x] = 0u;
    QcPool pool;
    pool.task = sl_task; pool.res = sl_res; pool.cnt = sl_qcnt; pool.rows = sl_lds; pool.wave_words = (uint32_t)wave_words; pool.cap = 2 * WAVE * SL_WAVES;
    bool active = s < n_surv;
    const uint64_t r = active ? surv_idx[s] : 0;
    if (active && rd_is_exc(R, r)) {
        SurvOut o;
        o.found = 0; o.n_ss = 0; o.repeat_len = 0; o.ss_off = 0; o.dr_len = 0; o.low_lexi = 0; o.err = 5;
        out[s] = o;
        active = false;
    }
    const int L = active ? (int)rd_len(R, r) : 0;
    const uint32_t *g = R.packed + (active ? rd_word_off(R, r) : 0);
    const int nw = (L + 15) >> 4;
    {
        int i = 0;
        for (; i + 4 <= nw; i += 4) {
            const ff_u32x4 v = *reinterpret_cast<const ff_u32x4 *>(g + i);
            lw[i * WAVE] = v.x; lw[(i + 1) * WAVE] = v.y; lw[(i + 2) * WAVE] = v.z; lw[(i + 3) * WAVE] = v.w;
        }
        for (; i < nw; i++) lw[i * WAVE] = g[i];
        for (; i < (int)words_per_read + 5; i++) lw[i * WAVE] = 0u;
    }
    LaneRead h;
    h.w = lw; h.ss = lss; h.L = L; h.nss = 0; h.cap = (int)ss_cap; h.replen = 0; h.punt = 0;
    h.cmask = (1u << (2 * P.window)) - 1u;
    const uint64_t hint = !active ? 0ull : hint_in_lds ? (0xFFFFFFFF00000000ull | (uint64_t)sl_hint[(uint32_t)(s - blockIdx.x * (uint64_t)blockDim.x)]) : ln_hint64(R, seed_hint, r, L, P.skips);
    int f = (P.debug_stop == 1) ? 0 : ln_search_core(h, P, hint, active, pool);
    if (!active) return;
    if (P.debug_stop == 4 && f == 1) f = 0;
    SurvOut o;
    o.found = 0; o.n_ss = 0; o.repeat_len = 0; o.ss_off = 0; o.dr_len = 0; o.low_lexi = 0; o.err = 0;
    if (h.punt) { o.err = 4; if (punt_cnt) atomicAdd(punt_cnt, 1u); }
    else if (f < 0) o.err = 1;
    else if (f == 1) {
        const int num_repeats = h.nss / 2;
        int pick;
        if (num_repeats == 1) pick = 0;
        else if (num_repeats == 2) {
            if (ln_ss(h, 0) == 0) pick = 2;
            else if (ln_ss(h, h.nss - 1) == (uint32_t)L) pick = 0;
            else pick = ((int)(ln_ss(h, 1) - ln_ss(h, 0)) > (int)(ln_ss(h, 3) - ln_ss(h, 2))) ? 0 : 2;
        } else pick = 2;
        uint32_t dlen = 0;
        const uint32_t st = ln_ss(h, pick);
        if (!substr_len(L, st, ln_ss(h, pick + 1) - st + 1, dlen) || dlen > dr_stride) o.err = 1;
        else {
            int less = 0;
            char *dr = dr_chars + s * (uint64_t)dr_stride;
            const uint32_t off = (uint32_t)s * ss_cap;
            if (dlen <= 64 && (dr_stride & 15u) == 0) {
                uint64_t v0, v1;
                ln_load128(h, (int)st, v0, v1);
                const uint64_t m0 = dlen >= 32 ? ~0ull : ((1ull << (2 * dlen)) - 1ull);
                const uint64_t m1 = dlen >= 64 ? ~0ull : (dlen > 32 ? ((1ull << (2 * (dlen - 32))) - 1ull) : 0ull);
                v0 &= m0; v1 &= m1;
                auto rev2 = [](uint64_t t) -> uint64_t { t = __brevll(t); return ((t >> 1) & 0x5555555555555555ull) | ((t & 0x5555555555555555ull) << 1); };
                const uint64_t c0 = rev2(~v1), c1 = rev2(~v0);
                const uint32_t drop = 128u - 2u * dlen;
                uint64_t r0, r1;
                if (drop == 0) { r0 = c0; r1 = c1; }
                else if (drop < 64) { r0 = (c0 >> drop) | (c1 << (64 - drop)); r1 = c1 >> drop; }
                else { r0 = c1 >> (drop - 64); r1 = 0; }
                r0 &= m0; r1 &= m1;
                const uint64_t d0 = v0 ^ r0, d1 = v1 ^ r1;
                if (d0 | d1) {
                    const uint64_t dv = d0 ? d0 : d1, av = d0 ? v0 : v1, bv = d0 ? r0 : r1;
                    const int p = (__ffsll((unsigned long long)dv) - 1) & ~1;
                    less = ((av >> p) & 3ull) < ((bv >> p) & 3ull);
                }
                const uint64_t s0 = less ? v0 : r0, s1 = less ? v1 : r1;
                uint4 *d4 = reinterpret_cast<uint4 *>(dr);
                for (uint32_t q = 0; q < dr_stride / 16; q++) {
                    const uint32_t bits = q < 2 ? (uint32_t)(s0 >> (32 * q)) : (q < 4 ? (uint32_t)(s1 >> (32 * (q - 2))) : 0u);
                    uint32_t wv[4];
#pragma unroll
                    for (int k = 0; k < 4; k++) {
                        const uint32_t b8 = (bits >> (8 * k)) & 0xFFu;
                        const uint32_t Ls = ((b8 & 0x55u) * 0x00041041u) & 0x01010101u, Hs = (((b8 >> 1) & 0x55u) * 0x00041041u) & 0x01010101u;
                        uint32_t asc = 0x41414141u + (Ls << 1) + Hs * 6u + (Ls & Hs) * 0x0Bu;
                        const int rem = (int)dlen - (int)(q * 16 + k * 4);
                        if (rem <= 0) asc = 0u; else if (rem < 4) asc &= (1u << (8 * rem)) - 1u;
                        wv[k] = asc;
                    }
                    uint4 o4; o4.x = wv[0]; o4.y = wv[1]; o4.z = wv[2]; o4.w = wv[3];
                    d4[q] = o4;
                }
                if (less) for (int k = 0; k < h.nss; k++) ss_pool[off + k] = ln_ss(h, k);
                else for (int k = 0; k < h.nss; k++) ss_pool[off + k] = (uint32_t)L - 1 - ln_ss(h, h.nss - 1 - k);
            } else {
            for (uint32_t i = 0; i < dlen; i++) {
                const uint32_t a = ln_base(h, (int)(st + i)), b = 3u - ln_base(h, (int)(st + dlen - 1 - i));
                if (a != b) { less = a < b; break; }
            }
            if (less) {
                for (uint32_t i = 0; i < dr_stride; i++) dr[i] = (i < dlen) ? "ACGT"[ln_base(h, (int)(st + i))] : (char)0;
                for (int k = 0; k < h.nss; k++) ss_pool[off + k] = ln_ss(h, k);
            } else {
                for (uint32_t i = 0; i < dr_stride; i++) dr[i] = (i < dlen) ? "ACGT"[3u - ln_base(h, (int)(st + dlen - 1 - i))] : (char)0;
                for (int k = 0; k < h.nss; k++) ss_pool[off + k] = (uint32_t)L - 1 - ln_ss(h, h.nss - 1 - k);
            }
            }
            o.found = 1; o.n_ss = (uint32_t)h.nss; o.repeat_len = (uint32_t)h.replen; o.ss_off = off;
            o.dr_len = (uint16_t)dlen; o.low_lexi = (uint8_t)less;
            found_flag[rd_header_id(R, r)] = 1;
        }
    }
    out[s] = o;
}

hipError_t launch_survivor_lanes(const DevReads &R, const DevParams &P, const uint64_t *surv_idx, const uint32_t *d_n_surv,
                                 uint64_t n_surv_max, SurvOut *out, char *dr_chars, uint32_t dr_stride, uint32_t *ss_pool,
                                 uint32_t ss_cap, uint8_t *found_flag, const uint32_t *seed_hint, hipStream_t st, const DevMerge *init_merge,
                                 uint32_t max_len, uint32_t *punt_cnt)
{
    if (n_surv_max == 0) return init_merge ? hipErrorNotSupported : hipSuccess;
    const uint32_t wpr = R.stride_words ? R.stride_words : (max_len + 15) / 16;
    if (!wpr || wpr > 32 || ss_cap > 64) return hipErrorNotSupported;
    const size_t wave_words = (size_t)(wpr + 5) * WAVE + ((size_t)ss_cap * WAVE + 1) / 2;
    const size_t lds = wave_words * 4 * SL_WAVES;
    static const bool no_regroup = getenv("CRASS_SURV_NO_REGROUP") != nullptr;
    const unsigned bt = WAVE * SL_WAVES;
    if (lds > 64 * 1024) {
        const hipError_t e = hipFuncSetAttribute(reinterpret_cast<const void *>(&k_survivor_lanes), hipFuncAttributeMaxDynamicSharedMemorySize, (int)lds);
        if (e != hipSuccess) return e;
    }
    CRASS_LAUNCH(k_survivor_lanes, dim3((unsigned)((n_surv_max + bt - 1) / bt)), dim3(bt), lds, st, R, P, surv_idx, d_n_surv,
                       n_surv_max, out, dr_chars, dr_stride, ss_pool, ss_cap, found_flag, seed_hint, wpr, init_merge ? *init_merge : DevMerge{},
                       init_merge ? 1 : 0, ((seed_hint || R.pos_hint) && !no_regroup) ? 1 : 0, punt_cnt);
    return hipGetLastError();
}

SurvLds survivor_lds_layout(uint32_t max_len, const DevParams &P, uint32_t row_len_cap, uint32_t seq_window_bytes, uint32_t ss_entries_cap)
{
    SurvLds l;
    l.seq_bytes = ((max_len + 16 + 16) + 15u) & ~15u;
    l.seq_window = 0;
    if (seq_window_bytes && ((seq_window_bytes + 15u) & ~15u) + 32u < l.seq_bytes) { l.seq_bytes = ((seq_window_bytes + 15u) & ~15u) + 32u; l.seq_window = l.seq_bytes - 32u; }
    uint32_t reps = max_len / (P.window + P.lowSp) + 4;
    l.ss_cap = ((2 * reps) + 3u) & ~3u;
    l.ss_slot = l.ss_cap;
    if (ss_entries_cap && ((ss_entries_cap + 3u) & ~3u) < l.ss_cap) l.ss_cap = (ss_entries_cap + 3u) & ~3u;
    l.row_elems = ((std::min(max_len, row_len_cap) + 8) + 7u) & ~7u;
    l.words_cap = (((max_len + 15) / 16 + 2) + 3u) & ~3u;
    l.hint_words = (((max_len + 63) / 64 + 2 + 1u) & ~1u) + 4u;
    l.total_bytes = l.seq_bytes + l.ss_cap * 4 + 2 * l.row_elems * 2 + l.words_cap * 4 + l.ss_cap * 4 + l.hint_words * 8;
    return l;
}

SurvLds survivor_lds_last_resort(uint32_t max_len, const DevParams &P)
{
    const SurvLds l = survivor_lds_layout(max_len, P);
    if (l.total_bytes <= 160 * 1024) return l;
    return survivor_lds_layout(max_len, P, std::max(P.highDR, P.highSp));
}

hipError_t launch_survivor(const DevReads &R, const DevParams &P, bool exceptions, const uint64_t *surv_idx,
                           const uint32_t *d_n_surv, uint64_t n_surv_max, SurvOut *out, char *dr_chars,
                           uint32_t dr_stride, uint32_t *ss_pool, uint32_t ss_pool_cap, uint32_t *d_ss_used,
                           uint8_t *found_flag, const uint32_t *seed_hint, const SurvLds &lds, int grid, hipStream_t st,
                           int punt_only, uint64_t slot_base, uint64_t slot_total, const uint32_t *punt_list, const uint32_t *d_punt_n, uint32_t *redo_list)
{
    if (n_surv_max == 0) return hipSuccess;
    hipError_t e;
    const uint32_t lds_bytes = ((lds.total_bytes + 7u) & ~7u) + (P.prof ? PF_LDS_WORDS * 8u : 0u);
    if (exceptions) {
        e = hipFuncSetAttribute(reinterpret_cast<const void *>(&k_survivor<true>), hipFuncAttributeMaxDynamicSharedMemorySize, (int)lds_bytes);
        if (e != hipSuccess) return e;
        CRASS_LAUNCH(k_survivor<true>, dim3(grid), dim3(WAVE), lds_bytes, st, R, P, surv_idx, d_n_surv, n_surv_max,
                           out, dr_chars, dr_stride, ss_pool, ss_pool_cap, d_ss_used, found_flag, seed_hint, lds, punt_only, slot_base, slot_total, punt_list, d_punt_n, redo_list);
    } else {
        e = hipFuncSetAttribute(reinterpret_cast<const void *>(&k_survivor<false>), hipFuncAttributeMaxDynamicSharedMemorySize, (int)lds_bytes);
        if (e != hipSuccess) return e;
        static const bool occ_dbg = getenv("CRASS_OCC_DEBUG") != nullptr;
        if (occ_dbg) {
            int nb = -1;
            (void)hipOccupancyMaxActiveBlocksPerMultiprocessor(&nb, reinterpret_cast<const void *>(&k_survivor<false>), WAVE, lds_bytes);
            fprintf(stderr, "[occ] k_survivor<false>: %d blocks per CU with %u bytes of LDS, grid %d, punt %d\n", nb, lds_bytes, grid, punt_only);
        }
        CRASS_LAUNCH(k_survivor<false>, dim3(grid), dim3(WAVE), lds_bytes, st, R, P, surv_idx, d_n_surv, n_surv_max,
                           out, dr_chars, dr_stride, ss_pool, ss_pool_cap, d_ss_used, found_flag, seed_hint, lds, punt_only, slot_base, slot_total, punt_list, d_punt_n, redo_list);
    }
    return hipGetLastError();
}

__global__ __launch_bounds__(256) void k_lev_batch_lanes(const uint8_t *chars, const uint64_t *a_off, const uint32_t *a_len,
                                                          const uint64_t *b_off, const uint32_t *b_len, uint64_t n_pairs,
                                                          int32_t *dist, float *sim)
{
    uint64_t k = blockIdx.x * (uint64_t)blockDim.x + threadIdx.x;
    if (k >= n_pairs) return;
    const uint8_t *s = chars + a_off[k], *t = chars + b_off[k];
    const int n = (int)a_len[k], m = (int)b_len[k];
    int d = lane_lev_bp(s, n, t, m);
    dist[k] = d;
    if (sim && d >= 0) {
        float max_length = (float)(n > m ? n : m);
        sim[k] = (n < 3 || m < 3) ? 0.0f : (float)(1.0 - (double)((float)d / max_length));
    }
}

__global__ __launch_bounds__(WAVE) void k_lev_batch(const uint8_t *chars, const uint64_t *a_off, const uint32_t *a_len,
                                                     const uint64_t *b_off, const uint32_t *b_len, uint64_t n_pairs,
                                                     int32_t *dist, float *sim, uint32_t row_elems, uint32_t str_bytes)
{
    extern __shared__ __attribute__((aligned(16))) uint8_t lv_lds[];
    uint8_t *sa = lv_lds;
    uint8_t *sb = lv_lds + str_bytes;
    uint16_t *rowA = reinterpret_cast<uint16_t *>(lv_lds + 2 * (size_t)str_bytes);
    uint16_t *rowB = rowA + row_elems;
    const int lane = threadIdx.x;
    for (uint64_t k = blockIdx.x; k < n_pairs; k += gridDim.x) {
        int n = (int)a_len[k], m = (int)b_len[k];
        if (dist[k] != -1) continue;
        wave_sync();
        for (int i = lane; i < n; i += WAVE) sa[i] = chars[a_off[k] + i];
        for (int i = lane; i < m; i += WAVE) sb[i] = chars[b_off[k] + i];
        wave_sync();
        int d = wave_lev(sa, n, sb, m, rowA, rowB, lane);
        float s = 0.0f;
        if (sim) s = wave_similarity(sa, n, sb, m, rowA, rowB, lane);
        if (lane == 0) { dist[k] = d; if (sim) sim[k] = s; }
    }
}

hipError_t launch_levenshtein_batch(const uint8_t *chars, const uint64_t *a_off, const uint32_t *a_len,
                                    const uint64_t *b_off, const uint32_t *b_len, uint64_t n_pairs,
                                    int32_t *dist, float *sim, uint32_t max_len, hipStream_t st)
{
    if (n_pairs == 0) return hipSuccess;
    uint32_t str_bytes = (max_len + 16 + 15u) & ~15u;
    uint32_t row_elems = ((max_len + 8) + 7u) & ~7u;
    size_t lds = 2 * (size_t)str_bytes + 2 * (size_t)row_elems * 2;
    hipError_t e = hipFuncSetAttribute(reinterpret_cast<const void *>(&k_lev_batch), hipFuncAttributeMaxDynamicSharedMemorySize, (int)lds);
// ... 9 lines not shown
```

### crass_amd/csrc/sinks.hip

```cpp
#include "dev_common.h"
#include <algorithm>

namespace crass {

__global__ void k_build_exc_mask(const uint64_t *exc_read, uint64_t n_exc, uint32_t *exc_mask)
{
    uint64_t i = blockIdx.x * (uint64_t)blockDim.x + threadIdx.x;
    if (i < n_exc) {
        uint64_t r = exc_read[i];
        atomicOr(&exc_mask[r >> 5], 1u << (r & 31));
    }
}

__global__ void k_mark_found(const uint64_t *idx, uint64_t n, const uint64_t *header_id, uint8_t *found_flag)
{
    const uint64_t i = blockIdx.x * (uint64_t)blockDim.x + threadIdx.x;
    if (i < n) { const uint64_t r = idx[i]; found_flag[header_id ? header_id[r] : r] = 1; }
}
hipError_t launch_mark_found(const uint64_t *idx, uint64_t n, const uint64_t *header_id, uint8_t *found_flag, hipStream_t st)
{
    if (!n) return hipSuccess;
    CRASS_LAUNCH(k_mark_found, dim3((unsigned)((n + 255) / 256)), dim3(256), 0, st, idx, n, header_id, found_flag);
    return hipGetLastError();
}
// ... 46 lines not shown
{
    __shared__ uint32_t sh[256];
    uint64_t wi = blockIdx.x * 256ull + threadIdx.x;
    uint32_t c = 0;
    if (wi < n_words) {
        uint64_t m = mask[wi];
        uint64_t rem = n_bits - wi * 64;
        if (rem < 64) m &= (1ull << rem) - 1ull;
        c = (uint32_t)__popcll(m);
    }
    sh[threadIdx.x] = c;
    __syncthreads();
    for (int off = 1; off < 256; off <<= 1) {
        uint32_t v = (threadIdx.x >= (unsigned)off) ? sh[threadIdx.x - off] : 0;
        __syncthreads();
        sh[threadIdx.x] += v;
        __syncthreads();
    }
    if (wi < n_words) word_prefix[wi] = sh[threadIdx.x] - c;
    if (threadIdx.x == 255) block_sums[blockIdx.x] = sh[255];
}

__global__ __launch_bounds__(1024) void k_block_scan(uint32_t *block_sums, uint32_t n_blocks, uint32_t *d_count, uint32_t *zero_a, uint32_t n_a, uint32_t *zero_b, uint32_t n_b)
{
    if (threadIdx.x < n_a) zero_a[threadIdx.x] = 0u;
    if (threadIdx.x < n_b) zero_b[threadIdx.x] = 0u;

    __shared__ uint32_t sh[1024];
    __shared__ uint32_t carry;
    if (threadIdx.x == 0) carry = 0;
    __syncthreads();
    for (uint32_t base = 0; base < n_blocks; base += 1024) {
        uint32_t i = base + threadIdx.x;
        uint32_t c = (i < n_blocks) ? block_sums[i] : 0;
        sh[threadIdx.x] = c;
        __syncthreads();
        for (int off = 1; off < 1024; off <<= 1) {
            uint32_t v = (threadIdx.x >= (unsigned)off) ? sh[threadIdx.x - off] : 0;
            __syncthreads();
            sh[threadIdx.x] += v;
            __syncthreads();
        }
        uint32_t excl = sh[threadIdx.x] - c + carry;
        if (i < n_blocks) block_sums[i] = excl;
        __syncthreads();
        if (threadIdx.x == 1023) carry += sh[1023];
        __syncthreads();
    }
    if (threadIdx.x == 0) *d_count = carry;
}

__global__ __launch_bounds__(256) void k_mask_scatter(const uint64_t *mask, uint64_t n_words, uint64_t n_bits,
                                                       const uint32_t *word_prefix, const uint32_t *block_sums,
                                                       uint64_t *out_idx, uint64_t out_cap)
{
    uint64_t wi = blockIdx.x * 256ull + threadIdx.x;
    if (wi >= n_words) return;
    uint64_t m = mask[wi];
    uint64_t rem = n_bits - wi * 64;
    if (rem < 64) m &= (1ull << rem) - 1ull;
    uint64_t o = (uint64_t)block_sums[blockIdx.x] + word_prefix[wi];
    while (m) {
        int b = __ffsll((unsigned long long)m) - 1;
        m &= m - 1;
        if (o < out_cap) out_idx[o] = wi * 64 + b;
        o++;
    }
}

static __device__ __forceinline__ unsigned long long lb_pack(uint32_t epoch, uint32_t flag, uint32_t value)
{
    return ((unsigned long long)epoch << 34) | ((unsigned long long)flag << 32) | value;
}
static __device__ uint32_t lb_exclusive_prefix(const Lookback &lb, uint32_t tile, uint32_t total)
{
    __shared__ uint32_t excl_sh;
    if (threadIdx.x < 64) {
        const int lane = (int)threadIdx.x;
        if (lane == 0)
            __hip_atomic_store(&lb.status[tile], lb_pack(lb.epoch, tile == 0 ? 2u : 1u, total), __ATOMIC_RELAXED, __HIP_MEMORY_SCOPE_AGENT);
        uint32_t excl = 0;
        int t = (int)tile - 1;
        while (t >= 0) {
            const int idx = t - lane;
            uint32_t flag = 2u, val = 0u;
            if (idx >= 0) {
                flag = 0u;
                for (uint32_t spins = 0; spins < (1u << 24); spins++) {
                    const unsigned long long w = __hip_atomic_load(&lb.status[idx], __ATOMIC_RELAXED, __HIP_MEMORY_SCOPE_AGENT);
                    if ((uint32_t)(w >> 34) == lb.epoch && ((w >> 32) & 3ull) != 0ull) { flag = (uint32_t)(w >> 32) & 3u; val = (uint32_t)w; break; }
                    __builtin_amdgcn_s_sleep(1);
                }
                if (flag == 0u) { *lb.fail = 1u; flag = 2u; }
            }
            const unsigned long long pm = __ballot(flag == 2u);
            const int stop = pm ? __ffsll(pm) - 1 : 64;
            uint32_t v = lane <= stop ? val : 0u;
#pragma unroll
            for (int off = 32; off > 0; off >>= 1) v += (uint32_t)__shfl_xor((int)v, off);
            excl += v;
            if (pm) break;
            t -= 64;
        }
        if (lane == 0) {
            if (tile != 0) __hip_atomic_store(&lb.status[tile], lb_pack(lb.epoch, 2u, excl + total), __ATOMIC_RELAXED, __HIP_MEMORY_SCOPE_AGENT);
            excl_sh = excl;
        }
    }
    __syncthreads();
    return excl_sh;
}
static __device__ uint32_t lb_tile_id(const Lookback &lb, uint32_t n_act)
{
    __shared__ uint32_t tile_sh;
    if (threadIdx.x == 0) {
        const uint32_t t = atomicAdd(lb.ticket, 1u);
        if (t + 1u >= n_act) __hip_atomic_store(lb.ticket, 0u, __ATOMIC_RELAXED, __HIP_MEMORY_SCOPE_AGENT);
        tile_sh = t;
    }
    __syncthreads();
    return tile_sh;
}
template <int T>
static __device__ uint32_t block_scan_t(uint32_t v, uint32_t *total)
{
    __shared__ uint32_t wsum[T / 64];
    const int lane = threadIdx.x & 63, wv = threadIdx.x >> 6;
    uint32_t incl = v;
#pragma unroll
    for (int off = 1; off < 64; off <<= 1) {
        const uint32_t y = (uint32_t)__shfl_up((int)incl, off);
        if (lane >= off) incl += y;
    }
    if (lane == 63) wsum[wv] = incl;
    __syncthreads();
    uint32_t base = 0, all = 0;
#pragma unroll
    for (int k = 0; k < T / 64; k++) { const uint32_t s = wsum[k]; if (k < wv) base += s; all += s; }
    *total = all;
    return base + incl - v;
}

template <int T, int W>
__global__ __launch_bounds__(T) void k_mask_compact_lb(const uint64_t *mask, uint64_t n_words, uint64_t n_bits, uint32_t *word_prefix,
                                                        uint32_t *block_sums, uint64_t *out_idx, uint64_t out_cap, uint32_t *d_count,
                                                        uint32_t *zero_a, uint32_t n_a, uint32_t *zero_b, uint32_t n_b, Lookback lb,
                                                        uint32_t n_tiles)
{
    const uint32_t tile = lb_tile_id(lb, n_tiles);
    if (tile == 0) {
        if (threadIdx.x < n_a) zero_a[threadIdx.x] = 0u;
        if (threadIdx.x < n_b) zero_b[threadIdx.x] = 0u;
    }
    const uint64_t w0 = ((uint64_t)tile * T + threadIdx.x) * W;
    uint64_t m[W];
    uint32_t cnt = 0;
#pragma unroll
    for (int q = 0; q < W; q++) {
        const uint64_t wi = w0 + q;
        m[q] = 0;
        if (wi < n_words) {
            m[q] = mask[wi];
            const uint64_t rem = n_bits - wi * 64;
            if (rem < 64) m[q] &= (1ull << rem) - 1ull;
        }
        cnt += (uint32_t)__popcll(m[q]);
    }
    uint32_t total;
    const uint32_t in_tile = block_scan_t<T>(cnt, &total);
    const uint32_t excl = lb_exclusive_prefix(lb, tile, total);
    if (tile == n_tiles - 1 && threadIdx.x == 0) *d_count = excl + total;
    uint64_t o = (uint64_t)excl + in_tile;
#pragma unroll
    for (int q = 0; q < W; q++) {
        const uint64_t wi = w0 + q;
        if (wi >= n_words) break;
        if (word_prefix) {
            word_prefix[wi] = (uint32_t)o;
            if ((wi & 255u) == 0) block_sums[wi >> 8] = 0u;
        }
        uint64_t mm = m[q];
        while (mm) {
            const int b = __ffsll((unsigned long long)mm) - 1;
            mm &= mm - 1;
            if (o < out_cap) out_idx[o] = wi * 64 + b;
            o++;
        }
    }
}

static constexpr uint32_t kLbElemsPerTile = 4096;
static __device__ uint32_t lb_rank4(const Lookback &lb, uint32_t tile, uint32_t cnt, uint32_t *upto)
{
    uint32_t all;
    const uint32_t in_tile = block_scan_t<1024>(cnt, &all);
    const uint32_t excl = lb_exclusive_prefix(lb, tile, all);
    *upto = excl + all;
    return excl + in_tile;
}

hipError_t launch_compact(const uint64_t *mask, uint64_t n_words, uint64_t n_bits, uint32_t *word_prefix,
                          uint32_t *block_sums, uint64_t *out_idx, uint64_t out_cap, uint32_t *d_count, hipStream_t st,
                          uint32_t *zero_a, uint32_t n_a, uint32_t *zero_b, uint32_t n_b, const Lookback *lb)
{
    if (lb && n_words) {
        const uint32_t tw = lookback_tile_words(n_words);
        const uint32_t n_tiles = (uint32_t)((n_words + tw - 1) / tw);
        if (tw == 256)
            CRASS_LAUNCH((k_mask_compact_lb<256, 1>), dim3(n_tiles), dim3(256), 0, st, mask, n_words, n_bits, word_prefix, block_sums, out_idx, out_cap,
                               d_count, zero_a, n_a, zero_b, n_b, *lb, n_tiles);
        else
            CRASS_LAUNCH((k_mask_compact_lb<1024, 4>), dim3(n_tiles), dim3(1024), 0, st, mask, n_words, n_bits, word_prefix, block_sums, out_idx, out_cap,
                               d_count, zero_a, n_a, zero_b, n_b, *lb, n_tiles);
        return hipGetLastError();
    }
    if (n_words == 0) {
        if (n_a) (void)hipMemsetAsync(zero_a, 0, 4 * (size_t)n_a, st);
        if (n_b) (void)hipMemsetAsync(zero_b, 0, 4 * (size_t)n_b, st);
        return hipMemsetAsync(d_count, 0, 4, st);
    }
    unsigned nb = (unsigned)((n_words + 255) / 256);
    CRASS_LAUNCH(k_mask_count, dim3(nb), dim3(256), 0, st, mask, n_words, n_bits, word_prefix, block_sums);
    CRASS_LAUNCH(k_block_scan, dim3(1), dim3(1024), 0, st, block_sums, nb, d_count, zero_a, n_a, zero_b, n_b);
    CRASS_LAUNCH(k_mask_scatter, dim3(nb), dim3(256), 0, st, mask, n_words, n_bits, word_prefix, block_sums, out_idx, out_cap);
    return hipGetLastError();
}

__global__ __launch_bounds__(256) void k_found_mask(const SurvOut *out, const uint32_t *d_n, uint64_t n, uint64_t *mask, uint32_t *d_err,
                                                     unsigned long long *dd_keys, uint32_t *dd_first, uint32_t dd_size)
{
    const uint64_t s = blockIdx.x * (uint64_t)blockDim.x + threadIdx.x;
    for (uint64_t i = s; i < dd_size; i += (uint64_t)gridDim.x * blockDim.x) { dd_keys[i] = 0ull; dd_first[i] = 0xFFFFFFFFu; }
    bool f = false;
    if (s < n && s < (uint64_t)*d_n) {
        const SurvOut o = out[s];
        f = o.found != 0;
        if (o.err) atomicMax(d_err, (uint32_t)o.err);
    }
    const uint64_t m = __ballot(f);
    if ((threadIdx.x & 63) == 0 && s < n) mask[s >> 6] = m;
}

static __device__ uint64_t dr_hash64(const char *p, uint32_t n)
{
    uint64_t h = 0x9E3779B97F4A7C15ull ^ ((uint64_t)n * 0xD6E8FEB86659FD93ull);
    while (n >= 8) {
        uint64_t v = 0;
        for (int i = 0; i < 8; i++) v |= (uint64_t)(uint8_t)p[i] << (8 * i);
        h = (h ^ v) * 0xFF51AFD7ED558CCDull; h ^= h >> 32; p += 8; n -= 8;
    }
    if (n) {
        uint64_t v = 0;
        for (uint32_t i = 0; i < n; i++) v |= (uint64_t)(uint8_t)p[i] << (8 * i);
        h = (h ^ v) * 0xC4CEB9FE1A85EC53ull; h ^= h >> 29;
    }
    return h ^ (h >> 31);
}

#define GF_BLOCK 1024
#define GF_SLOTS 2048
__global__ __launch_bounds__(GF_BLOCK) void k_gather_found(const uint64_t *fidx, const uint32_t *d_nf, uint64_t n_max,
                                                            const SurvOut *out, const uint64_t *surv_idx, uint64_t read_base,
                                                            const char *dr_chars, uint32_t dr_stride, const uint32_t *ss_pool,
                                                            uint32_t ss_cap, uint32_t ss_elem, uint8_t *blob, uint16_t *g_dr_len, char *g_dr,
                                                            unsigned long long *dd_keys, uint32_t *dd_first, uint32_t dd_mask,
                                                            uint64_t *dd_hash, uint32_t *dd_slot, uint32_t *d_mismatch)
{
    __shared__ unsigned long long lkey[GF_SLOTS];
    __shared__ uint32_t lmin[GF_SLOTS], lslot[GF_SLOTS];
    const uint64_t k = blockIdx.x * (uint64_t)GF_BLOCK + threadIdx.x;
    uint64_t n = *d_nf;
    if (n > n_max) n = n_max;
    if (blockIdx.x * (uint64_t)GF_BLOCK >= n) return;
    if (dd_keys) {
        for (uint32_t i = threadIdx.x; i < GF_SLOTS; i += GF_BLOCK) { lkey[i] = 0ull; lmin[i] = 0xFFFFFFFFu; }
        __syncthreads();
    }
// ... 471 lines not shown
```

Baseline: 30.03 billion reads/s.

## Pack seed hints per filter block and compact them into survivor slot order

The fast filter now writes seed hints densely per block of survivors instead of scattering them by read index. The compaction kernels then copy each survivor's hint into a slot-indexed array, so the survivor kernels read hints contiguously by slot rather than gathering from a read-indexed table. This adds a hint buffer sized to the read count and extra work in compaction. It also ties the filter block size to the compaction's hint block size, which is enforced by static asserts.

After: 30.01 billion reads/s (median of 2 runs). No clear change (-0.1%).

```diff
diff --git a/crass_amd/csrc/dev_common.h b/crass_amd/csrc/dev_common.h
--- a/crass_amd/csrc/dev_common.h
+++ b/crass_amd/csrc/dev_common.h
@@ -28,6 +28,10 @@
 {
     return (R.exc_mask[r >> 5] >> (r & 31)) & 1u;
 }
+static __device__ __forceinline__ uint32_t seed_hint_of(const SeedHints &h, uint64_t r, uint64_t s)
+{
+    return h.by_slot ? h.by_slot[s] : (h.by_read ? h.by_read[r] : 0xFFFFFFFFu);
+}
 static __device__ __forceinline__ uint64_t rd_hint_off(const DevReads &R, uint64_t r)
 {
     return R.uniform_len ? r * (uint64_t)((R.uniform_len + 63u) >> 6) : R.pos_hint_off[r];
diff --git a/crass_amd/csrc/engine.cpp b/crass_amd/csrc/engine.cpp
--- a/crass_amd/csrc/engine.cpp
+++ b/crass_amd/csrc/engine.cpp
@@ -228,7 +228,7 @@
     c->r_packed.release(); c->r_word_off.release(); c->r_lengths.release(); c->r_header_id.release();
     c->r_exc_mask.release(); c->r_exc_read.release(); c->r_exc_off.release(); c->r_exc_bytes.release();
     c->d_mask.release(); c->d_word_prefix.release(); c->d_block_sums.release(); c->d_idx.release(); c->d_count.release();
-    c->d_found.release(); c->d_hit_info.release(); c->d_surv.release(); c->d_dr.release(); c->d_ss_pool.release();
+    c->d_found.release(); c->d_hit_info.release(); c->d_surv_hint.release(); c->d_surv.release(); c->d_dr.release(); c->d_ss_pool.release();
     c->d_ss_used.release(); c->d_rec.release(); c->d_exc_hit.release(); c->d_extra.release(); c->d_extra_bad.release(); c->h_extra_bad.release();
     c->g_surv.release(); c->g_dr.release(); c->g_ss.release(); c->g_fidx.release(); c->h_count.release(); c->h_surv.release(); c->h_dr.release(); c->h_ss.release(); c->h_idx.release(); c->h_rec.release();
     c->a_go4w.release(); c->a_go16.release(); c->a_go32.release(); c->a_out.release(); c->a_go4.release(); c->dense.release(); c->d_fidx.release(); c->d_pos_hint.release(); c->d_pos_hint_off.release(); c->d_pos_hint_blk.release(); c->d_punt.release(); c->d_redo.release(); c->dd_keys.release(); c->dd_first.release(); c->dd_slot.release(); c->dd_rep.release(); c->dd_hash.release(); c->h_rep.release(); c->h_hash.release(); c->a_anchor.release(); c->d_slot_info.release(); c->d_slot_pid.release(); c->a_out_pid.release(); c->a_pat_token.release();
@@ -259,6 +259,7 @@
     HIPCHK(c, c->d_count.ensure(8));
     HIPCHK(c, c->d_found.ensure(n + 1));
     HIPCHK(c, c->d_hit_info.ensure(n + 1));
+    if (c->hints_can_pack()) HIPCHK(c, c->d_surv_hint.ensure(n + 1));
     HIPCHK(c, c->d_ss_used.ensure(4));
     HIPCHK(c, c->h_count.ensure(32));
     HIPCHK(c, hipMemsetAsync(c->d_found.p, 0, n + 1, c->stream));
diff --git a/crass_amd/csrc/engine_ctx.h b/crass_amd/csrc/engine_ctx.h
--- a/crass_amd/csrc/engine_ctx.h
+++ b/crass_amd/csrc/engine_ctx.h
@@ -240,6 +240,7 @@
     bool inflate_hbm_window = true;
     uint32_t hid_hash_bits = 64;
     bool lane_find_serial = false;
+    bool hints_by_read = false;
     uint32_t probe_blocks = 0;
     void read()
     {
@@ -265,6 +266,7 @@
         inflate_hbm_window = true; if (const char *e = getenv("CRASS_INFLATE_WINDOW")) inflate_hbm_window = strcmp(e, "lds") != 0;
         hid_hash_bits = 64; if (const char *e = getenv("CRASS_HID_TEST_HASH_BITS")) hid_hash_bits = (uint32_t)std::min(64, std::max(0, atoi(e)));
         lane_find_serial = false; if (const char *e = getenv("CRASS_LANE_FIND_SERIAL")) lane_find_serial = atoi(e) != 0;
+        hints_by_read = false; if (const char *e = getenv("CRASS_HINTS_BY_READ")) hints_by_read = atoi(e) != 0;
         probe_blocks = 0; if (const char *e = getenv("CRASS_PROBE_BLOCKS")) probe_blocks = (uint32_t)std::max(0, atoi(e));
         pool_cap_bytes = 0; if (const char *e = getenv("CRASS_POOL_CAP_MB")) pool_cap_bytes = (uint64_t)std::max(1ll, atoll(e)) << 20;
     }
@@ -292,6 +294,16 @@
     DevBuf<uint64_t> d_mask; DevBuf<uint32_t> d_word_prefix; DevBuf<uint32_t> d_block_sums;
     DevBuf<uint64_t> d_idx; DevBuf<uint32_t> d_count; DevBuf<uint8_t> d_found; DevBuf<uint32_t> d_hit_info;
     bool hints_valid = false;
+    bool hints_packed = false;
+    DevBuf<uint32_t> d_surv_hint;
+    SeedHints pass1_hints(uint64_t off = 0) const
+    {
+        SeedHints h;
+        if (!hints_valid) return h;
+        if (hints_packed) h.by_slot = d_surv_hint.p + off; else h.by_read = d_hit_info.p;
+        return h;
+    }
+    bool hints_can_pack() const { return !env.hints_by_read && R.uniform_len && R.stride_words >= 4 && R.stride_words <= 16; }
     DevBuf<SurvOut> d_surv; DevBuf<char> d_dr; DevBuf<uint32_t> d_ss_pool; DevBuf<uint32_t> d_ss_used;
     DevBuf<RecruitOut> d_rec; DevBuf<uint32_t> d_exc_hit; DevBuf<uint64_t> d_extra;
     DevBuf<uint32_t> d_extra_bad; PinBuf<uint32_t> h_extra_bad;
diff --git a/crass_amd/csrc/engine_internal.h b/crass_amd/csrc/engine_internal.h
--- a/crass_amd/csrc/engine_internal.h
+++ b/crass_amd/csrc/engine_internal.h
@@ -44,6 +44,18 @@
     uint8_t  low_lexi;
     uint8_t  err;
 };
+
+struct SeedHints {
+    const uint32_t *by_read = nullptr;
+    const uint32_t *by_slot = nullptr;
+#if defined(__HIPCC__) || defined(__CUDACC__)
+    __host__ __device__
+#endif
+    bool any() const { return by_read || by_slot; }
+    SeedHints from_slot(uint64_t off) const { SeedHints h = *this; if (h.by_slot) h.by_slot += off; return h; }
+};
+static constexpr uint32_t kHintBlockReads = 1024;
+static constexpr uint32_t kHintBlockWords = kHintBlockReads / 64;
 
 struct RecruitOut {
     uint32_t start, end;
@@ -252,7 +264,7 @@
 hipError_t launch_long_light(const DevReads &R, const DevParams &P, const uint32_t *d_n, uint64_t n_max, SurvOut *out, uint64_t slot_base,
                              uint32_t max_len, hipStream_t st, uint32_t *punt_list, uint32_t *d_punt_n, const uint64_t *surv_idx = nullptr);
 hipError_t launch_filter_fast(const DevReads &R, const DevParams &P, uint64_t *hitmask, uint32_t *seed_hint, hipStream_t st,
-                              uint8_t *clear_found = nullptr, bool *cleared = nullptr);
+                              uint8_t *clear_found = nullptr, bool *cleared = nullptr, bool *packed = nullptr);
 #define CRASS_VGPR_FLOOR(N) asm volatile("" ::: "v" #N)
 
 #ifdef __HIPCC__
@@ -291,19 +303,20 @@
 hipError_t launch_compact(const uint64_t *mask, uint64_t n_words, uint64_t n_bits, uint32_t *word_prefix,
                           uint32_t *block_sums, uint64_t *out_idx, uint64_t out_cap, uint32_t *d_count,
                           hipStream_t st, uint32_t *zero_a = nullptr, uint32_t n_a = 0, uint32_t *zero_b = nullptr, uint32_t n_b = 0,
-                          const Lookback *lb = nullptr);
+                          const Lookback *lb = nullptr,
+                          const uint32_t *packed_hint = nullptr, uint32_t *slot_hint = nullptr);
 hipError_t launch_survivor(const DevReads &R, const DevParams &P, bool exceptions,
                            const uint64_t *surv_idx, const uint32_t *d_n_surv, uint64_t n_surv_max,
                            SurvOut *out, char *dr_chars, uint32_t dr_stride,
                            uint32_t *ss_pool, uint32_t ss_pool_cap, uint32_t *d_ss_used,
-                           uint8_t *found_flag, const uint32_t *seed_hint, const SurvLds &lds, int grid, hipStream_t st,
+                           uint8_t *found_flag, const SeedHints &hints, const SurvLds &lds, int grid, hipStream_t st,
                            int punt_only = 0,
                            uint64_t slot_base = 0, uint64_t slot_total = 0,
                            const uint32_t *punt_list = nullptr, const uint32_t *d_punt_n = nullptr,
                            uint32_t *redo_list = nullptr);
 hipError_t launch_survivor_lanes(const DevReads &R, const DevParams &P, const uint64_t *surv_idx, const uint32_t *d_n_surv,
                                  uint64_t n_surv_max, SurvOut *out, char *dr_chars, uint32_t dr_stride, uint32_t *ss_pool,
-                                 uint32_t ss_cap, uint8_t *found_flag, const uint32_t *seed_hint, hipStream_t st,
+                                 uint32_t ss_cap, uint8_t *found_flag, const SeedHints &hints, hipStream_t st,
                                  const DevMerge *init_merge = nullptr, uint32_t max_len = 0, uint32_t *punt_cnt = nullptr);
 hipError_t launch_recruit_general(const DevReads &R, const DevAutomaton &A, const uint8_t *found_flag,
                                   uint64_t *hitmask, uint32_t *hit_info, hipStream_t st);
diff --git a/crass_amd/csrc/engine_pass1.cpp b/crass_amd/csrc/engine_pass1.cpp
--- a/crass_amd/csrc/engine_pass1.cpp
+++ b/crass_amd/csrc/engine_pass1.cpp
@@ -112,7 +112,7 @@
                 else if (s1 > s0)
                     HIPCHK(c, launch_survivor(R, c->dp, false, ident_list ? nullptr : c->d_idx.p + s0, c->d_count.p + 1, s1 - s0,
                                               c->d_surv.p + s0, c->d_dr.p + s0 * (size_t)stride, stride, c->d_ss_pool.p, (uint32_t)pool_cap, c->d_ss_used.p,
-                                              c->d_found.p, c->hints_valid ? c->d_hit_info.p : nullptr, lds,
+                                              c->d_found.p, c->pass1_hints(s0), lds,
                                               (int)std::min<uint64_t>(grid, s1 - s0), c->stream, 0, s0, nchunk));
                 s0 = s1;
             }
@@ -124,23 +124,23 @@
             { const int hw = hint_wait_all(c); if (hw) return hw; }
             HIPCHK(c, launch_survivor(R, c->dp, exc, (exc || ident_list) ? nullptr : c->d_idx.p + off, c->d_count.p + (exc ? 0 : 1), nchunk,
                                       c->d_surv.p, c->d_dr.p, stride, c->d_ss_pool.p, (uint32_t)pool_cap, c->d_ss_used.p,
-                                      c->d_found.p, (!exc && c->hints_valid) ? c->d_hit_info.p : nullptr, lds,
+                                      c->d_found.p, (!exc && !ident_list) ? c->pass1_hints(off) : SeedHints{}, lds,
                                       (int)std::min<uint64_t>(grid, nchunk), c->stream));
         }
         if (use_light)
             HIPCHK(c, launch_survivor(R, c->dp, false, nullptr, c->d_count.p + 1, nchunk,
                                       c->d_surv.p, c->d_dr.p, stride, c->d_ss_pool.p, (uint32_t)pool_cap, c->d_ss_used.p,
-                                      c->d_found.p, nullptr, lds, (int)std::min<uint64_t>(256 * 12, nchunk), c->stream, 7, 0, nchunk, c->d_punt.p + 1, c->d_punt.p,
+                                      c->d_found.p, SeedHints{}, lds, (int)std::min<uint64_t>(256 * 12, nchunk), c->stream, 7, 0, nchunk, c->d_punt.p + 1, c->d_punt.p,
                                       capped ? c->d_redo.p : nullptr));
         if (use_light && c->dp.prof) { HIPCHK(c, hipStreamSynchronize(c->stream)); dump_surv_prof(c); }
         if (capped && use_light)
             HIPCHK(c, launch_survivor(R, c->dp, false, nullptr, c->d_count.p + 1, nchunk,
                                       c->d_surv.p, c->d_dr.p, stride, c->d_ss_pool.p, (uint32_t)pool_cap, c->d_ss_used.p,
-                                      c->d_found.p, nullptr, lds_full, (int)std::min<uint64_t>(256 * 2, nchunk), c->stream, 6, 0, nchunk, c->d_redo.p + 1, c->d_redo.p));
+                                      c->d_found.p, SeedHints{}, lds_full, (int)std::min<uint64_t>(256 * 2, nchunk), c->stream, 6, 0, nchunk, c->d_redo.p + 1, c->d_redo.p));
         else if (capped)
             HIPCHK(c, launch_survivor(R, c->dp, exc, (exc || ident_list) ? nullptr : c->d_idx.p + off, c->d_count.p + (exc ? 0 : 1), nchunk,
                                       c->d_surv.p, c->d_dr.p, stride, c->d_ss_pool.p, (uint32_t)pool_cap, c->d_ss_used.p,
-                                      c->d_found.p, (!exc && c->hints_valid) ? c->d_hit_info.p : nullptr, lds_full,
+                                      c->d_found.p, (!exc && !ident_list) ? c->pass1_hints(off) : SeedHints{}, lds_full,
                                       (int)std::min<uint64_t>(grid, nchunk), c->stream, 6));
         if (!exc && off == 0) HIPCHK(c, c->stamp(9, 1));
         const uint64_t n_words = (nchunk + 63) / 64;
@@ -444,7 +444,7 @@
     }
     HIPCHK(c, c->stamp(8, 1));
     static const bool no_hints_dbg = getenv("CRASS_SURV_NO_HINTS") != nullptr;
-    const uint32_t *hints = (c->hints_valid && !no_hints_dbg) ? c->d_hit_info.p : nullptr;
+    const SeedHints hints = no_hints_dbg ? SeedHints{} : c->pass1_hints();
     const bool no_lanes = c->env.no_lane_kernel;
     hipError_t le = no_lanes ? hipErrorNotSupported
                              : launch_survivor_lanes(c->R, c->dp, c->d_idx.p, d_nsurv, n_surv, c->d_surv.p, c->d_dr.p, stride,
@@ -472,7 +472,7 @@
                               le == hipSuccess ? c->d_count.p + 6 : nullptr));
     if (c->R.n_exc)
         HIPCHK(c, launch_survivor(c->R, c->dp, true, c->d_idx.p, d_nsurv, n_surv, c->d_surv.p, c->d_dr.p, stride,
-                                  c->d_ss_pool.p, (uint32_t)pool_cap, c->d_ss_used.p, c->d_found.p, nullptr, lds,
+                                  c->d_ss_pool.p, (uint32_t)pool_cap, c->d_ss_used.p, c->d_found.p, SeedHints{}, lds,
                                   (int)std::min<uint64_t>(256 * 32, n_surv), c->stream, 5));
     HIPCHK(c, c->stamp(9, 1));
     const uint64_t n_words = (n_surv + 63) / 64;
@@ -609,7 +609,7 @@
     if (!c->env.no_warm_launch) {
         HIPCHK(c, hipMemsetAsync(c->d_count.p, 0, 32, c->stream));
         HIPCHK(c, launch_survivor(c->R, c->dp, false, c->d_idx.p, c->d_count.p + 1, surv, c->d_surv.p, c->d_dr.p, c->dr_stride,
-                                  c->d_ss_pool.p, (uint32_t)pool_cap, c->d_ss_used.p, c->d_found.p, nullptr, lds,
+                                  c->d_ss_pool.p, (uint32_t)pool_cap, c->d_ss_used.p, c->d_found.p, SeedHints{}, lds,
                                   (int)std::min<uint64_t>(256 * 32, surv), c->stream, 4));
     }
     host_pool_warm();
@@ -629,15 +629,18 @@
     return s;
 }
 
-struct FilterRoute { bool fast = false, hint_filtered = false, found_cleared = false; };
+struct FilterRoute { bool fast = false, hint_filtered = false, found_cleared = false, packed = false; };
 
 static int launch_filter(crass_hip_ctx *c, uint64_t n_words, FilterRoute &fr)
 {
     hipError_t fe = hipErrorNotSupported;
     static const bool found_memset = getenv("CRASS_FOUND_MEMSET") != nullptr;
-    if (c->R.stride_words >= 4 && c->R.stride_words <= 16)
-        fe = launch_filter_fast(c->R, c->dp, c->d_mask.p, c->d_hit_info.p, c->stream, found_memset ? nullptr : c->d_found.p, &fr.found_cleared);
-    if (fe != hipSuccess) fr.found_cleared = false;
+    if (c->R.stride_words >= 4 && c->R.stride_words <= 16) {
+        fr.packed = c->hints_can_pack();
+        if (fr.packed) HIPCHK(c, c->d_surv_hint.ensure(c->R.n_reads + 1));
+        fe = launch_filter_fast(c->R, c->dp, c->d_mask.p, c->d_hit_info.p, c->stream, found_memset ? nullptr : c->d_found.p, &fr.found_cleared, &fr.packed);
+    }
+    if (fe != hipSuccess) { fr.found_cleared = false; fr.packed = false; }
     const bool lattice_hints = c->hint_filter && c->R.pos_hint && !c->hint_filter_any;
     if (fe == hipSuccess) fr.fast = true;
     else if (fe == hipErrorNotSupported && (lattice_hints || (c->hint_filter_any && c->n_pos_hint_words))) {
@@ -769,12 +772,13 @@
     const bool use_filter = c->max_len <= c->env.long_min;
     c->dp.exc_survive = (use_filter && c->R.n_exc > 0 && !c->env.exc_separate) ? 1u : 0u;
     if (const int fs = use_filter ? launch_filter(c, n_words, fr) : launch_unfiltered(c, n_words)) return fs;
-    c->hints_valid = fr.fast;
+    c->hints_valid = fr.fast; c->hints_packed = fr.fast && fr.packed;
     if (!fr.found_cleared) HIPCHK(c, hipMemsetAsync(c->d_found.p, 0, n + 1, c->stream));
     HIPCHK(c, c->stamp(1, 1));
     Lookback lbs;
     HIPCHK(c, launch_compact(c->d_mask.p, n_words, n, c->d_word_prefix.p, c->d_block_sums.p, c->d_idx.p, n, c->d_count.p, c->stream,
-                             c->d_count.p + 2, 5, c->d_ss_used.p, 1, c->next_lookback(n_words, &lbs)));
+                             c->d_count.p + 2, 5, c->d_ss_used.p, 1, c->next_lookback(n_words, &lbs),
+                             c->hints_packed ? c->d_hit_info.p : nullptr, c->hints_packed ? c->d_surv_hint.p : nullptr));
     HIPCHK(c, c->stamp(2, 2));
     c->dense.active = false; c->have_rep = false; c->have_distinct = false;
     c->have_dev_tokens = false; c->hl_tokens = false;
diff --git a/crass_amd/csrc/kernels.hip b/crass_amd/csrc/kernels.hip
--- a/crass_amd/csrc/kernels.hip
+++ b/crass_amd/csrc/kernels.hip
@@ -204,11 +204,13 @@
     return r;
 }
 template <int W, int D0, int D1, int LCT, int RPL>
-__global__ __launch_bounds__(256) void k_filter_fast_pairs(DevReads R, DevParams P, uint64_t *hitmask, uint32_t *seed_hint, uint8_t *clear_found)
+__global__ __launch_bounds__(256) void k_filter_fast_pairs(DevReads R, DevParams P, uint64_t *hitmask, uint32_t *seed_hint, uint8_t *clear_found, int pack)
 {
     static_assert(LCT > 0 && LCT - D0 - 9 >= 0 && RPL * 256 <= 65536, "uniform length with at least one seed");
+    static_assert(256 * RPL == (int)kHintBlockReads, "the compaction takes a block of packed hints to be this kernel's block");
     __shared__ uint32_t q_n;
     __shared__ uint16_t q[256 * RPL];
+    __shared__ uint32_t q_hint[256 * RPL];
     __shared__ uint32_t tile_mask[2 * 4 * RPL];
     const uint64_t r_block = blockIdx.x * (uint64_t)(256 * RPL);
     const uint64_t r_first = r_block + threadIdx.x;
@@ -283,8 +285,9 @@
         uint32_t acc[SW];
         ff_exact_scan<D0, D1, LCT>(w, acc);
         const uint32_t hint = ff_exact_hint<LCT>(acc, n_seed);
+        if (have && pack) q_hint[b0 + lane] = hint;
         if (have && hint != 0) {
-            seed_hint[r_block + loc] = hint;
+            if (!pack) seed_hint[r_block + loc] = hint;
             atomicOr(&tile_mask[loc >> 5], 1u << (loc & 31u));
         }
     }
@@ -292,6 +295,23 @@
     if (threadIdx.x < 4 * RPL) {
         const uint64_t r0 = r_block + threadIdx.x * 64u;
         if (r0 < R.n_reads) hitmask[r0 >> 6] = (uint64_t)tile_mask[2 * threadIdx.x] | ((uint64_t)tile_mask[2 * threadIdx.x + 1] << 32);
+    }
+    if (!pack || (threadIdx.x & ~63u) >= qn) return;
+    static_assert(2 * 4 * RPL == 32, "one mask half per lane of half a wave");
+    const uint32_t half = tile_mask[lane & 31u];
+    uint32_t incl = (uint32_t)__popc(half);
+#pragma unroll
+    for (int off = 1; off < 32; off <<= 1) {
+        const uint32_t y = (uint32_t)__shfl_up((int)incl, off, 32);
+        if ((lane & 31u) >= (uint32_t)off) incl += y;
+    }
+    const uint32_t excl = incl - (uint32_t)__popc(half);
+    for (uint32_t b0 = threadIdx.x & ~63u; b0 < qn; b0 += 256u) {
+        const bool have = b0 + lane < qn;
+        const uint32_t hint = have ? q_hint[b0 + lane] : 0u;
+        const uint32_t loc = have ? q[b0 + lane] : 0u;
+        const uint32_t rank = (uint32_t)__shfl((int)excl, (int)(loc >> 5)) + (uint32_t)__popc((uint32_t)__shfl((int)half, (int)(loc >> 5)) & ((1u << (loc & 31u)) - 1u));
+        if (hint != 0) seed_hint[r_block + rank] = hint;
     }
 }
 
@@ -422,9 +442,11 @@
     if ((threadIdx.x & 63) == 0 && active) hitmask[r >> 6] = m;
 }
 
-hipError_t launch_filter_fast(const DevReads &R, const DevParams &P, uint64_t *hitmask, uint32_t *seed_hint, hipStream_t st, uint8_t *clear_found, bool *cleared)
+hipError_t launch_filter_fast(const DevReads &R, const DevParams &P, uint64_t *hitmask, uint32_t *seed_hint, hipStream_t st, uint8_t *clear_found, bool *cleared, bool *packed)
 {
     if (cleared) *cleared = false;
+    const bool may_pack = packed && *packed;
+    if (packed) *packed = false;
     if (!R.stride_words || R.n_reads == 0) return hipErrorNotSupported;
     if (P.window != 8 || P.skips != 8) {
         if (P.window < 6 || P.window > 9 || P.skips < 1 || P.lowDR + P.lowSp < 17 || P.highDR + P.highSp < P.lowDR + P.lowSp) return hipErrorNotSupported;
@@ -460,7 +482,7 @@
     static const bool ff_exact = getenv("CRASS_FF_EXACT") && atoi(getenv("CRASS_FF_EXACT")) != 0;
     if (cleared && clear_found) *cleared = true;
 #define FF_LEN(LL, WW) if (R.uniform_len == LL && R.stride_words == WW) { \
-        if (rpl >= 4 && !ff_exact) CRASS_LAUNCH((k_filter_fast_pairs<WW, 49, 97, LL, 4>), g4, b, 0, st, R, P, hitmask, seed_hint, clear_found); \
+        if (rpl >= 4 && !ff_exact) { CRASS_LAUNCH((k_filter_fast_pairs<WW, 49, 97, LL, 4>), g4, b, 0, st, R, P, hitmask, seed_hint, clear_found, may_pack ? 1 : 0); if (packed) *packed = may_pack; } \
         else if (rpl >= 4) CRASS_LAUNCH((k_filter_fast_impl<WW, 49, 97, LL, 4>), g4, b, 0, st, R, P, hitmask, seed_hint, clear_found); \
         else CRASS_LAUNCH((k_filter_fast_impl<WW, 49, 97, LL, 1>), g, b, 0, st, R, P, hitmask, seed_hint, clear_found); \
         return hipGetLastError(); }
@@ -1683,7 +1705,7 @@
                                                    const uint32_t *d_n_surv, uint64_t n_max, SurvOut *out,
                                                    char *dr_chars, uint32_t dr_stride, uint32_t *ss_pool,
                                                    uint32_t ss_pool_cap, uint32_t *d_ss_used,
-                                                   uint8_t *found_flag, const uint32_t *seed_hint, SurvLds lds, int punt_only, uint64_t slot_base, uint64_t slot_total,
+                                                   uint8_t *found_flag, SeedHints hints, SurvLds lds, int punt_only, uint64_t slot_base, uint64_t slot_total,
                                                    const uint32_t *punt_list, const uint32_t *d_punt_n, uint32_t *redo_list)
 {
     extern __shared__ __attribute__((aligned(16))) uint8_t sv_lds[];
@@ -1798,7 +1820,7 @@
         if (h.lprof && lane == 0) h.lprof[PF_STAGE] = (unsigned long long)__builtin_readcyclecounter() - prof_t0;
         h.L = L; h.nss = 0; h.replen = 0; h.err = 0;
         h.asc_lo = 0; h.asc_hi = 0; h.asc_pad = (int)(P.highDR + P.highSp) + 32; h.seq = h.seq_buf;
-        const uint32_t hint = (!EXC && seed_hint) ? seed_hint[r] : 0xFFFFFFFFu;
+        const uint32_t hint = EXC ? 0xFFFFFFFFu : seed_hint_of(hints, r, s);
         uint64_t *ph = (!EXC && R.pos_hint) ? l_hint : nullptr;
         uint32_t *cls_from = reinterpret_cast<uint32_t *>(l_hint + lds.hint_words - 4);
         if (ph && lane < 8) cls_from[lane] = (lane == 0 || R.hint_all) ? 0u : 0xFFFFFFFFu;
@@ -2778,6 +2800,7 @@
 }
 
 #define SL_WAVES 4
+#define SL_SLOT_WORDS 16
 static __device__ __forceinline__ uint64_t ln_hint64(const DevReads &R, const uint32_t *seed_hint, uint64_t r, int L, uint32_t skips)
 {
     if (seed_hint) return 0xFFFFFFFF00000000ull | (uint64_t)seed_hint[r];
@@ -2797,19 +2820,64 @@
 __global__ __launch_bounds__(WAVE * SL_WAVES) void k_survivor_lanes(DevReads R, DevParams P, const uint64_t *surv_idx, const uint32_t *d_n_surv,
                                                          uint64_t n_max, SurvOut *out, char *dr_chars, uint32_t dr_stride,
                                                          uint32_t *ss_pool, uint32_t ss_cap, uint8_t *found_flag,
-                                                         const uint32_t *seed_hint, uint32_t words_per_read, DevMerge IM, int do_init, int regroup,
+                                                         SeedHints hints, uint32_t words_per_read, DevMerge IM, int do_init, int regroup,
                                                          uint32_t *punt_cnt)
 {
     extern __shared__ __attribute__((aligned(16))) uint32_t sl_lds[];
     __shared__ uint16_t sl_perm[WAVE * SL_WAVES];
     __shared__ uint32_t sl_cnt[SL_WAVES];
     __shared__ uint32_t sl_hint[WAVE * SL_WAVES];
+    __shared__ uint64_t sl_read[WAVE * SL_WAVES];
     const int lane = threadIdx.x & (WAVE - 1), wv = threadIdx.x >> 6;
+    const uint32_t *seed_hint = hints.by_read;
     if (do_init) dm_init_slice(IM, blockIdx.x * (uint64_t)blockDim.x + threadIdx.x, (uint64_t)gridDim.x * blockDim.x);
     uint64_t n_surv = *d_n_surv;
     if (n_surv > n_max) n_surv = n_max;
     uint64_t s = blockIdx.x * (uint64_t)blockDim.x + threadIdx.x;
-    if (regroup) {
+    const size_t wave_words = (size_t)(words_per_read + 5) * WAVE + ((size_t)ss_cap * WAVE + 1) / 2;
+    bool slot_exc = false;
+    uint64_t slot_r = 0;
+    uint32_t slot_hint = 0;
+    if (hints.by_slot) {
+        const bool have = s < n_surv;
+        const uint64_t r0 = have ? surv_idx[s] : 0;
+        const uint32_t h0 = have ? hints.by_slot[s] : 0u;
+        const bool exc0 = have && R.n_exc && rd_is_exc(R, r0);
+        const int nw0 = (have && !exc0) ? (int)((rd_len(R, r0) + 15) >> 4) : 0;
+        const uint32_t *g0 = R.packed + (nw0 ? rd_word_off(R, r0) : 0);
+        uint32_t row[SL_SLOT_WORDS];
+#pragma unroll
+        for (int i = 0; i < SL_SLOT_WORDS; i += 4) {
+            if (i + 4 <= nw0) {
+                const ff_u32x4 v = *reinterpret_cast<const ff_u32x4 *>(g0 + i);
+                row[i] = v.x; row[i + 1] = v.y; row[i + 2] = v.z; row[i + 3] = v.w;
+            } else {
+#pragma unroll
+                for (int k = 0; k < 4; k++) row[i + k] = i + k < nw0 ? g0[i + k] : 0u;
+            }
+        }
+        const bool heavy = regroup && nw0 && __popc(h0) >= 2;
+        const uint64_t hb = __ballot(heavy);
+        if (lane == 0) sl_cnt[wv] = (uint32_t)__popcll(hb);
+        __syncthreads();
+        uint32_t heavy_before = 0, heavy_total = 0;
+#pragma unroll
+        for (int k = 0; k < SL_WAVES; k++) { const uint32_t c = sl_cnt[k]; heavy_total += c; if (k < wv) heavy_before += c; }
+        const uint32_t below = (uint32_t)__popcll(hb & ((1ull << lane) - 1ull));
+        const uint32_t pos = heavy ? heavy_before + below
+                                   : heavy_total + ((uint32_t)wv * WAVE - heavy_before) + ((uint32_t)lane - below);
+        uint32_t *col = sl_lds + (size_t)(pos >> 6) * wave_words + (pos & (WAVE - 1));
+#pragma unroll
+        for (int i = 0; i < SL_SLOT_WORDS; i++) if (i < (int)words_per_read + 5) col[i * WAVE] = row[i];
+        for (int i = SL_SLOT_WORDS; i < (int)words_per_read + 5; i++) col[i * WAVE] = 0u;
+        sl_read[pos] = r0; sl_hint[pos] = h0;
+        sl_perm[pos] = (uint16_t)(threadIdx.x | (exc0 ? 0x8000u : 0u));
+        __syncthreads();
+        const uint32_t from = sl_perm[threadIdx.x];
+        s = blockIdx.x * (uint64_t)blockDim.x + (from & 0x7FFFu);
+        slot_exc = (from >> 15) != 0;
+        slot_r = sl_read[threadIdx.x]; slot_hint = sl_hint[threadIdx.x];
+    } else if (regroup) {
         bool heavy = false;
         if (s < n_surv) {
             const uint64_t r0 = surv_idx[s];
@@ -2831,7 +2899,6 @@
         s = blockIdx.x * (uint64_t)blockDim.x + sl_perm[threadIdx.x];
     }
     const bool hint_in_lds = regroup && seed_hint;
-    const size_t wave_words = (size_t)(words_per_read + 5) * WAVE + ((size_t)ss_cap * WAVE + 1) / 2;
     uint32_t *wbase = sl_lds + (size_t)wv * wave_words;
     uint32_t *lw = wbase + lane;
     uint16_t *lss = reinterpret_cast<uint16_t *>(wbase + (size_t)(words_per_read + 5) * WAVE) + lane;
@@ -2843,8 +2910,8 @@
     QcPool pool;
     pool.task = sl_task; pool.res = sl_res; pool.cnt = sl_qcnt; pool.rows = sl_lds; pool.wave_words = (uint32_t)wave_words; pool.cap = 2 * WAVE * SL_WAVES;
     bool active = s < n_surv;
-    const uint64_t r = active ? surv_idx[s] : 0;
-    if (active && rd_is_exc(R, r)) {
+    const uint64_t r = hints.by_slot ? slot_r : (active ? surv_idx[s] : 0);
+    if (active && (hints.by_slot ? slot_exc : rd_is_exc(R, r))) {
         SurvOut o;
         o.found = 0; o.n_ss = 0; o.repeat_len = 0; o.ss_off = 0; o.dr_len = 0; o.low_lexi = 0; o.err = 5;
         out[s] = o;
@@ -2853,7 +2920,7 @@
     const int L = active ? (int)rd_len(R, r) : 0;
     const uint32_t *g = R.packed + (active ? rd_word_off(R, r) : 0);
     const int nw = (L + 15) >> 4;
-    {
+    if (!hints.by_slot) {
         int i = 0;
         for (; i + 4 <= nw; i += 4) {
             const ff_u32x4 v = *reinterpret_cast<const ff_u32x4 *>(g + i);
@@ -2865,7 +2932,7 @@
     LaneRead h;
     h.w = lw; h.ss = lss; h.L = L; h.nss = 0; h.cap = (int)ss_cap; h.replen = 0; h.punt = 0;
     h.cmask = (1u << (2 * P.window)) - 1u;
-    const uint64_t hint = !active ? 0ull : hint_in_lds ? (0xFFFFFFFF00000000ull | (uint64_t)sl_hint[(uint32_t)(s - blockIdx.x * (uint64_t)blockDim.x)]) : ln_hint64(R, seed_hint, r, L, P.skips);
+    const uint64_t hint = !active ? 0ull : hints.by_slot ? (0xFFFFFFFF00000000ull | (uint64_t)slot_hint) : hint_in_lds ? (0xFFFFFFFF00000000ull | (uint64_t)sl_hint[(uint32_t)(s - blockIdx.x * (uint64_t)blockDim.x)]) : ln_hint64(R, seed_hint, r, L, P.skips);
     int f = (P.debug_stop == 1) ? 0 : ln_search_core(h, P, hint, active, pool);
     if (!active) return;
     if (P.debug_stop == 4 && f == 1) f = 0;
@@ -2951,12 +3018,13 @@
 
 hipError_t launch_survivor_lanes(const DevReads &R, const DevParams &P, const uint64_t *surv_idx, const uint32_t *d_n_surv,
                                  uint64_t n_surv_max, SurvOut *out, char *dr_chars, uint32_t dr_stride, uint32_t *ss_pool,
-                                 uint32_t ss_cap, uint8_t *found_flag, const uint32_t *seed_hint, hipStream_t st, const DevMerge *init_merge,
+                                 uint32_t ss_cap, uint8_t *found_flag, const SeedHints &hints, hipStream_t st, const DevMerge *init_merge,
                                  uint32_t max_len, uint32_t *punt_cnt)
 {
     if (n_surv_max == 0) return init_merge ? hipErrorNotSupported : hipSuccess;
     const uint32_t wpr = R.stride_words ? R.stride_words : (max_len + 15) / 16;
     if (!wpr || wpr > 32 || ss_cap > 64) return hipErrorNotSupported;
+    if (hints.by_slot && wpr > SL_SLOT_WORDS) return hipErrorNotSupported;
     const size_t wave_words = (size_t)(wpr + 5) * WAVE + ((size_t)ss_cap * WAVE + 1) / 2;
     const size_t lds = wave_words * 4 * SL_WAVES;
     static const bool no_regroup = getenv("CRASS_SURV_NO_REGROUP") != nullptr;
@@ -2966,8 +3034,8 @@
         if (e != hipSuccess) return e;
     }
     CRASS_LAUNCH(k_survivor_lanes, dim3((unsigned)((n_surv_max + bt - 1) / bt)), dim3(bt), lds, st, R, P, surv_idx, d_n_surv,
-                       n_surv_max, out, dr_chars, dr_stride, ss_pool, ss_cap, found_flag, seed_hint, wpr, init_merge ? *init_merge : DevMerge{},
-                       init_merge ? 1 : 0, ((seed_hint || R.pos_hint) && !no_regroup) ? 1 : 0, punt_cnt);
+                       n_surv_max, out, dr_chars, dr_stride, ss_pool, ss_cap, found_flag, hints, wpr, init_merge ? *init_merge : DevMerge{},
+                       init_merge ? 1 : 0, ((hints.any() || R.pos_hint) && !no_regroup) ? 1 : 0, punt_cnt);
     return hipGetLastError();
 }
 
@@ -2998,7 +3066,7 @@
 hipError_t launch_survivor(const DevReads &R, const DevParams &P, bool exceptions, const uint64_t *surv_idx,
                            const uint32_t *d_n_surv, uint64_t n_surv_max, SurvOut *out, char *dr_chars,
                            uint32_t dr_stride, uint32_t *ss_pool, uint32_t ss_pool_cap, uint32_t *d_ss_used,
-                           uint8_t *found_flag, const uint32_t *seed_hint, const SurvLds &lds, int grid, hipStream_t st,
+                           uint8_t *found_flag, const SeedHints &hints, const SurvLds &lds, int grid, hipStream_t st,
                            int punt_only, uint64_t slot_base, uint64_t slot_total, const uint32_t *punt_list, const uint32_t *d_punt_n, uint32_t *redo_list)
 {
     if (n_surv_max == 0) return hipSuccess;
@@ -3008,7 +3076,7 @@
         e = hipFuncSetAttribute(reinterpret_cast<const void *>(&k_survivor<true>), hipFuncAttributeMaxDynamicSharedMemorySize, (int)lds_bytes);
         if (e != hipSuccess) return e;
         CRASS_LAUNCH(k_survivor<true>, dim3(grid), dim3(WAVE), lds_bytes, st, R, P, surv_idx, d_n_surv, n_surv_max,
-                           out, dr_chars, dr_stride, ss_pool, ss_pool_cap, d_ss_used, found_flag, seed_hint, lds, punt_only, slot_base, slot_total, punt_list, d_punt_n, redo_list);
+                           out, dr_chars, dr_stride, ss_pool, ss_pool_cap, d_ss_used, found_flag, hints, lds, punt_only, slot_base, slot_total, punt_list, d_punt_n, redo_list);
     } else {
         e = hipFuncSetAttribute(reinterpret_cast<const void *>(&k_survivor<false>), hipFuncAttributeMaxDynamicSharedMemorySize, (int)lds_bytes);
         if (e != hipSuccess) return e;
@@ -3019,7 +3087,7 @@
             fprintf(stderr, "[occ] k_survivor<false>: %d blocks per CU with %u bytes of LDS, grid %d, punt %d\n", nb, lds_bytes, grid, punt_only);
         }
         CRASS_LAUNCH(k_survivor<false>, dim3(grid), dim3(WAVE), lds_bytes, st, R, P, surv_idx, d_n_surv, n_surv_max,
-                           out, dr_chars, dr_stride, ss_pool, ss_pool_cap, d_ss_used, found_flag, seed_hint, lds, punt_only, slot_base, slot_total, punt_list, d_punt_n, redo_list);
+                           out, dr_chars, dr_stride, ss_pool, ss_pool_cap, d_ss_used, found_flag, hints, lds, punt_only, slot_base, slot_total, punt_list, d_punt_n, redo_list);
     }
     return hipGetLastError();
 }
diff --git a/crass_amd/csrc/sinks.hip b/crass_amd/csrc/sinks.hip
--- a/crass_amd/csrc/sinks.hip
+++ b/crass_amd/csrc/sinks.hip
@@ -122,7 +122,7 @@
 
 __global__ __launch_bounds__(256) void k_mask_scatter(const uint64_t *mask, uint64_t n_words, uint64_t n_bits,
                                                        const uint32_t *word_prefix, const uint32_t *block_sums,
-                                                       uint64_t *out_idx, uint64_t out_cap)
+                                                       uint64_t *out_idx, uint64_t out_cap, const uint32_t *packed_hint, uint32_t *slot_hint)
 {
     uint64_t wi = blockIdx.x * 256ull + threadIdx.x;
     if (wi >= n_words) return;
@@ -130,10 +130,15 @@
     uint64_t rem = n_bits - wi * 64;
     if (rem < 64) m &= (1ull << rem) - 1ull;
     uint64_t o = (uint64_t)block_sums[blockIdx.x] + word_prefix[wi];
+    const uint64_t hb = packed_hint ? (wi & ~(uint64_t)(kHintBlockWords - 1)) : 0;
+    const uint64_t o_blk = packed_hint ? (uint64_t)block_sums[blockIdx.x] + word_prefix[hb] : 0;
     while (m) {
         int b = __ffsll((unsigned long long)m) - 1;
         m &= m - 1;
-        if (o < out_cap) out_idx[o] = wi * 64 + b;
+        if (o < out_cap) {
+            out_idx[o] = wi * 64 + b;
+            if (packed_hint) slot_hint[o] = packed_hint[hb * 64 + (o - o_blk)];
+        }
         o++;
     }
 }
@@ -215,8 +220,9 @@
 __global__ __launch_bounds__(T) void k_mask_compact_lb(const uint64_t *mask, uint64_t n_words, uint64_t n_bits, uint32_t *word_prefix,
                                                         uint32_t *block_sums, uint64_t *out_idx, uint64_t out_cap, uint32_t *d_count,
                                                         uint32_t *zero_a, uint32_t n_a, uint32_t *zero_b, uint32_t n_b, Lookback lb,
-                                                        uint32_t n_tiles)
-{
+                                                        uint32_t n_tiles, const uint32_t *packed_hint, uint32_t *slot_hint)
+{
+    static_assert(kHintBlockWords % W == 0 && kHintBlockWords / W <= 64 && (T * W) % kHintBlockWords == 0, "a filter block's threads: one aligned group of a wave");
     const uint32_t tile = lb_tile_id(lb, n_tiles);
     if (tile == 0) {
         if (threadIdx.x < n_a) zero_a[threadIdx.x] = 0u;
@@ -238,9 +244,19 @@
     }
     uint32_t total;
     const uint32_t in_tile = block_scan_t<T>(cnt, &total);
+    constexpr int LB_HINTS = 8;
+    const uint32_t rank0 = packed_hint ? in_tile - (uint32_t)__shfl((int)in_tile, (int)((threadIdx.x & 63u) & ~(kHintBlockWords / W - 1u))) : 0u;
+    const uint32_t *my_hint = packed_hint ? packed_hint + (w0 & ~(uint64_t)(kHintBlockWords - 1)) * 64 + rank0 : nullptr;
+    uint32_t hv[LB_HINTS];
+#pragma unroll
+    for (int k = 0; k < LB_HINTS; k++) hv[k] = (packed_hint && (uint32_t)k < cnt) ? my_hint[k] : 0u;
     const uint32_t excl = lb_exclusive_prefix(lb, tile, total);
     if (tile == n_tiles - 1 && threadIdx.x == 0) *d_count = excl + total;
     uint64_t o = (uint64_t)excl + in_tile;
+    if (packed_hint) {
+#pragma unroll
+        for (int k = 0; k < LB_HINTS; k++) if ((uint32_t)k < cnt && o + k < out_cap) slot_hint[o + k] = hv[k];
+    }
 #pragma unroll
     for (int q = 0; q < W; q++) {
         const uint64_t wi = w0 + q;
@@ -257,6 +273,10 @@
             o++;
         }
     }
+    if (packed_hint) {
+        o = (uint64_t)excl + in_tile;
+        for (uint32_t k = LB_HINTS; k < cnt; k++) if (o + k < out_cap) slot_hint[o + k] = my_hint[k];
+    }
 }
 
 static constexpr uint32_t kLbElemsPerTile = 4096;
@@ -271,17 +291,19 @@
 
 hipError_t launch_compact(const uint64_t *mask, uint64_t n_words, uint64_t n_bits, uint32_t *word_prefix,
                           uint32_t *block_sums, uint64_t *out_idx, uint64_t out_cap, uint32_t *d_count, hipStream_t st,
-                          uint32_t *zero_a, uint32_t n_a, uint32_t *zero_b, uint32_t n_b, const Lookback *lb)
-{
+                          uint32_t *zero_a, uint32_t n_a, uint32_t *zero_b, uint32_t n_b, const Lookback *lb,
+                          const uint32_t *packed_hint, uint32_t *slot_hint)
+{
+    if (!packed_hint || !slot_hint) { packed_hint = nullptr; slot_hint = nullptr; }
     if (lb && n_words) {
         const uint32_t tw = lookback_tile_words(n_words);
         const uint32_t n_tiles = (uint32_t)((n_words + tw - 1) / tw);
         if (tw == 256)
             CRASS_LAUNCH((k_mask_compact_lb<256, 1>), dim3(n_tiles), dim3(256), 0, st, mask, n_words, n_bits, word_prefix, block_sums, out_idx, out_cap,
-                               d_count, zero_a, n_a, zero_b, n_b, *lb, n_tiles);
+                               d_count, zero_a, n_a, zero_b, n_b, *lb, n_tiles, packed_hint, slot_hint);
         else
             CRASS_LAUNCH((k_mask_compact_lb<1024, 4>), dim3(n_tiles), dim3(1024), 0, st, mask, n_words, n_bits, word_prefix, block_sums, out_idx, out_cap,
-                               d_count, zero_a, n_a, zero_b, n_b, *lb, n_tiles);
+                               d_count, zero_a, n_a, zero_b, n_b, *lb, n_tiles, packed_hint, slot_hint);
         return hipGetLastError();
     }
     if (n_words == 0) {
@@ -292,7 +314,7 @@
     unsigned nb = (unsigned)((n_words + 255) / 256);
     CRASS_LAUNCH(k_mask_count, dim3(nb), dim3(256), 0, st, mask, n_words, n_bits, word_prefix, block_sums);
     CRASS_LAUNCH(k_block_scan, dim3(1), dim3(1024), 0, st, block_sums, nb, d_count, zero_a, n_a, zero_b, n_b);
-    CRASS_LAUNCH(k_mask_scatter, dim3(nb), dim3(256), 0, st, mask, n_words, n_bits, word_prefix, block_sums, out_idx, out_cap);
+    CRASS_LAUNCH(k_mask_scatter, dim3(nb), dim3(256), 0, st, mask, n_words, n_bits, word_prefix, block_sums, out_idx, out_cap, packed_hint, slot_hint);
     return hipGetLastError();
 }
 
```
